# HazyResearch/flash-fft-conv

Hardware: AMD Instinct MI355X
Metric: FFT-conv fwd+bwd seq/s, B=16 H=768 L=16384 fft=32768 bf16 (higher is better)
Workload: dtype bf16; 1 GPU; FlashFFTConv(32768) B=16 H=768 L=16384 bf16, fwd+bwd incl. k->k_f and dk (BASELINE configs[1]); heads_per_rank=768, parallelism=head-shard x1 (no collective)

## Files before the change

flash-fft-conv_amd/csrc/ffc_body.h:

```cpp
#pragma once
#include <stdint.h>

#include "ffc_layout.h"
#include "ffc_plan.h"

#ifndef FFC_FN
#define FFC_FN inline __attribute__((always_inline))
#endif

namespace ffc {

struct ConvArgs {
  const void* u;
  const void* pregate;
  const void* postgate;
  void* y;
  const void* kf;
  const uint8_t* tab;
  PlanTabs t;
  int B, H, L;
  int npair;
  int nchunk, ppc;
  int conj_kf;
  int fast;
// ... 1045 lines not shown
        if (FWD && !NOTW) {
          if constexpr (CHAIN16_A) {
            i32 m = j * 4 + (w * 128 * GEO::S1 + 2 * tp + th);
            i32 k0 = hi * 4;
            if constexpr (RP) twiddle16(re, im, m * (k0 * ps.R + ps.k0), m * ps.R, -1.0f, s_fwd, GEO::N * ps.R - 1, 1.0f / (float)(GEO::N * ps.R));
            else twiddle16(re, im, m * k0, m, -1.0f, s_fwd);
          } else
#pragma unroll
          for (int half = 0; half < 2; half++) {
            const int s1 = (16 * half) / GEO::N1;
            i32 m = j * 4 + (s1 * 128 + w * 128 * GEO::S1 + 2 * tp + th);
            i32 k0 = hi * 4 + ((16 * half) % GEO::N1);
            F2 tr[4], ti[4];
            if constexpr (RP) chain8p(m * (k0 * ps.R + ps.k0), m * ps.R, -1.0f, s_fwd, tr, ti, GEO::N * ps.R - 1, 1.0f / (float)(GEO::N * ps.R));
            else chain8p(m * k0, m, -1.0f, s_fwd, tr, ti);
            apply8(re, im, half, tr, ti);
          }
        }
        if constexpr (!B::LEAN_OUTER) {
          if (th == 0) {
            re0 = re; im0 = im;
          } else {
#pragma unroll
            for (int r = 0; r < 16; r++) {
              if (!FWD && HALF && row_dead((r & 3) + 8 * (r >> 2))) continue;
              const int c = (r & 3) + 8 * (r >> 2);
              const int s1 = c / GEO::N1, rwc = c % GEO::N1;
              i32 off = colb[s1] + (rwc * (GEO::Mi * 2) + 4 * tp);
              B::lds_w32(off, B::template pack<DT>(re0[r], re[r]));
              B::lds_w32(off + GEO::PLANE, B::template pack<DT>(im0[r], im[r]));
            }
          }
        } else {
          if (th == 0) {
#pragma unroll
            for (int q = 0; q < 8; q++) {
              if (!FWD && HALF && row_dead(((2 * q) & 3) + 8 * ((2 * q) >> 2))) continue;
              s0r[q] = B::template pack<DT>(re[2 * q], re[2 * q + 1]);
              s0i[q] = B::template pack<DT>(im[2 * q], im[2 * q + 1]);
            }
          } else {
#pragma unroll
            for (int q = 0; q < 8; q++) {
              if (!FWD && HALF && row_dead(((2 * q) & 3) + 8 * ((2 * q) >> 2))) continue;
              u32 p1r = B::template pack<DT>(re[2 * q], re[2 * q + 1]), p1i = B::template pack<DT>(im[2 * q], im[2 * q + 1]);
#pragma unroll
              for (int o = 0; o < 2; o++) {
                const int r = 2 * q + o;
                const int c = (r & 3) + 8 * (r >> 2);
                const int s1 = c / GEO::N1, rwc = c % GEO::N1;
                i32 off = colb[s1] + (rwc * (GEO::Mi * 2) + 4 * tp);
                B::lds_w32(off, o ? B::merge_hi(s0r[q], p1r) : B::merge_lo(s0r[q], p1r));
                B::lds_w32(off + GEO::PLANE, o ? B::merge_hi(s0i[q], p1i) : B::merge_lo(s0i[q], p1i));
              }
            }
          }
        }
      }
    }
  }

#ifndef FFC_OUTER_QUAD
#define FFC_OUTER_QUAD 1
#endif
  template <bool FWD, bool HALF, bool RP = false, bool NOTW = false>
  static FFC_FN void outer_stage_quad(int L, Unit un, float s_fwd = 1.0f, Pass ps = Pass()) {
    const i32 lane = B::opaque(B::lane());
    const int w = un.wq;
    const i32 j = lane & 31, hi = lane >> 5;
    constexpr int ms_lim = (FWD && HALF && GEO::N1 == 32) ? 1 : 2;
    i32 colb[GEO::S1];
#pragma unroll
    for (int s = 0; s < GEO::S1; s++)
      colb[s] = e_off<GEO, i32>(hi * 4, j * 4 + (s * 128 + w * 128 * GEO::S1)) + un.eb;
    Mat F1;
    if constexpr (RP) load_mat(F1, FWD ? ps.mat_fwd : ps.mat_inv, lane);
    else lds_mat(F1, GEO::L_F1);
    U2 rawr[2][8], rawi[2][8];
#pragma unroll
    for (int ms = 0; ms < 2; ms++) {
      if (ms >= ms_lim) continue;
#pragma unroll
      for (int e = 0; e < 8; e++) {
        const int c = 16 * ms + 8 * (e >> 2) + (e & 3);
        const int s1 = c / GEO::N1, rwc = c % GEO::N1;
        i32 off = colb[s1] + rwc * (GEO::Mi * 2);
        if (FWD && HALF && row_dead(c)) { rawr[ms][e].x = B::uconst(0); rawr[ms][e].y = B::uconst(0); rawi[ms][e] = rawr[ms][e]; continue; }
        rawr[ms][e] = B::lds_r64(off); rawi[ms][e] = B::lds_r64(off + GEO::PLANE);
      }
    }
    u32 p0r[16], p0i[16];
#pragma unroll
    for (int tp = 0; tp < 2; tp++) {
      A16 re0, im0;
#pragma unroll
      for (int th = 0; th < 2; th++) {
        Op op;
#pragma unroll
        for (int ms = 0; ms < 2; ms++) {
          if (ms >= ms_lim) continue;
#pragma unroll
          for (int d = 0; d < 4; d++) {
            const u32 ar = tp ? rawr[ms][2 * d].y : rawr[ms][2 * d].x, br = tp ? rawr[ms][2 * d + 1].y : rawr[ms][2 * d + 1].x;
            const u32 ai = tp ? rawi[ms][2 * d].y : rawi[ms][2 * d].x, bi = tp ? rawi[ms][2 * d + 1].y : rawi[ms][2 * d + 1].x;
            op.r[ms][d] = th ? B::merge_hi(ar, br) : B::merge_lo(ar, br);
            op.i[ms][d] = th ? B::merge_hi(ai, bi) : B::merge_lo(ai, bi);
          }
        }
        A16 re, im;
        re = B::a16_zero(); im = B::a16_zero();
        cmm<!FWD, false>(re, im, op, F1, ms_lim);
        if (FWD && !NOTW) {
          if constexpr (CHAIN16_A) {
            i32 m = j * 4 + (w * 128 * GEO::S1 + 2 * tp + th);
            i32 k0 = hi * 4;
            if constexpr (RP) twiddle16(re, im, m * (k0 * ps.R + ps.k0), m * ps.R, -1.0f, s_fwd, GEO::N * ps.R - 1, 1.0f / (float)(GEO::N * ps.R));
            else twiddle16(re, im, m * k0, m, -1.0f, s_fwd);
          } else
#pragma unroll
          for (int half = 0; half < 2; half++) {
            const int s1 = (16 * half) / GEO::N1;
            i32 m = j * 4 + (s1 * 128 + w * 128 * GEO::S1 + 2 * tp + th);
            i32 k0 = hi * 4 + ((16 * half) % GEO::N1);
            F2 tr[4], ti[4];
            if constexpr (RP) chain8p(m * (k0 * ps.R + ps.k0), m * ps.R, -1.0f, s_fwd, tr, ti, GEO::N * ps.R - 1, 1.0f / (float)(GEO::N * ps.R));
            else chain8p(m * k0, m, -1.0f, s_fwd, tr, ti);
            apply8(re, im, half, tr, ti);
          }
        }
        if (th == 0) {
          re0 = re; im0 = im;
        } else {
#pragma unroll
          for (int r = 0; r < 16; r++) {
            if (!FWD && HALF && row_dead((r & 3) + 8 * (r >> 2))) continue;
            const u32 vr = B::template pack<DT>(re0[r], re[r]), vi = B::template pack<DT>(im0[r], im[r]);
            if (tp == 0) {
              p0r[r] = vr; p0i[r] = vi;
            } else {
              const int c = (r & 3) + 8 * (r >> 2);
              const int s1 = c / GEO::N1, rwc = c % GEO::N1;
              i32 off = colb[s1] + rwc * (GEO::Mi * 2);
              U2 wr, wi;
              wr.x = p0r[r]; wr.y = vr; wi.x = p0i[r]; wi.y = vi;
              B::lds_w64(off, wr);
              B::lds_w64(off + GEO::PLANE, wi);
            }
          }
        }
      }
    }
  }

  template <bool FWD, bool HALF, bool RP = false, bool DIN = false, bool NOTW = false>
  static FFC_FN void outer_stage(int L, Unit un, float s_fwd = 1.0f, Pass ps = Pass()) {
    if constexpr (DIN) { outer_stage_pair<FWD, HALF, RP, true, NOTW>(L, un, s_fwd, ps); return; }
    if constexpr (B::LEAN_OUTER && !(FWD && HALF && GEO::N1 == 32)) outer_stage_tile<FWD, HALF, RP, NOTW>(L, un, s_fwd, ps);
    else if constexpr (!B::LEAN_OUTER && FFC_OUTER_QUAD != 0 && HALF) outer_stage_quad<FWD, HALF, RP, NOTW>(L, un, s_fwd, ps);
    else outer_stage_pair<FWD, HALF, RP, false, NOTW>(L, un, s_fwd, ps);
  }

  struct InnerRegs { Mat F2; CT16 tw; i32 roff[2][2]; i32 woff[4]; };
  template <bool TWR = true>
  static FFC_FN void load_inner(InnerRegs& R, Unit un) {
    lds_mat(R.F2, GEO::L_F2);
    if constexpr (TWR) lds_ct16(R.tw, GEO::L_TW);
    const i32 lane = B::lane();
    const i32 c = lane & 31, hi = lane >> 5;
    const i32 i16 = lane & 15, g16 = (lane >> 4) & 1;
    const i32 n3b = (g16 * 16) % GEO::N3;
#pragma unroll
    for (int ms = 0; ms < 2; ms++)
#pragma unroll
      for (int rho = 0; rho < 2; rho++) {
        i32 U = hi * 4 + (16 * ms + 8 * rho) + (i16 >> 2);
        i32 sU = U / GEO::N2, n2 = U % GEO::N2;
        i32 row = sU * GEO::SV + ((g16 * 16) / GEO::N3);
        R.roff[ms][rho] = e_off<GEO, i32>(row, n2 * GEO::N3 + n3b + (i16 & 3) * 4) + un.eb;
      }
#pragma unroll
    for (int rq = 0; rq < 4; rq++) {
      i32 V = hi * 4 + 8 * rq;
      i32 row = (c / GEO::N2) * GEO::SV + V / GEO::N3;
      R.woff[rq] = e_off<GEO, i32>(row, (c % GEO::N2) * GEO::N3 + V % GEO::N3) + un.eb;
    }
  }

  static constexpr int IPASS_BYTES = 2 * 6144 + 2 * 8192;
  static constexpr int L_IPASS = GEO::LDS_BYTES;
  struct InnerPass { Mat Fa, Finv; CT16 tw; int tw2_off; int base; };
  static FFC_FN void load_inner_pass(InnerPass& ip, int k0) {
    const int base = L_IPASS + k0 * IPASS_BYTES;
    lds_mat(ip.Fa, base);
    lds_mat(ip.Finv, base + 6144);
    lds_ct16(ip.tw, base + 12288);
    ip.tw2_off = base + 12288 + 8192;
    ip.base = base;
  }
  static FFC_FN void load_inner_pass_lean(InnerPass& ip, int k0) {
    ip.base = L_IPASS + k0 * IPASS_BYTES;
    ip.tw2_off = ip.base + 12288 + 8192;
  }
  static FFC_FN void setup_tables_ipass(const uint8_t* tab, const PlanTabs& t, int R) {
    for (int k0 = 0; k0 < R; k0++) copy_tab(tab + t.ipass[k0], L_IPASS + k0 * IPASS_BYTES, IPASS_BYTES);
    B::barrier();
  }

  static FFC_FN void load_tile_op(int tau, Op& op, Unit un, const InnerRegs& R, int doff = 0) {
    const int trow = tau * (GEO::G * GEO::Mi * 2) + doff;
    if (B::HAS_TR) {
#pragma unroll
      for (int ms = 0; ms < 2; ms++)
#pragma unroll
        for (int rho = 0; rho < 2; rho++) {
          i32 off = R.roff[ms][rho] + trow;
          U2 vr = B::lds_r64_tr(off), vi = B::lds_r64_tr(off + GEO::PLANE);
          op.r[ms][2 * rho] = vr.x; op.r[ms][2 * rho + 1] = vr.y;
          op.i[ms][2 * rho] = vi.x; op.i[ms][2 * rho + 1] = vi.y;
        }
#pragma unroll
      for (int ms = 0; ms < 2; ms++) { B::pin(op.r[ms]); B::pin(op.i[ms]); }
    } else {
      const i32 lane = B::opaque(B::lane());
      const i32 c = lane & 31, hi = lane >> 5;
      const i32 sV = c / GEO::N3, n3 = c % GEO::N3;
#pragma unroll
      for (int ms = 0; ms < 2; ms++)
#pragma unroll
        for (int d = 0; d < 4; d++) {
          u32 wr[2], wi[2];
#pragma unroll
          for (int hf = 0; hf < 2; hf++) {
            int e = 2 * d + hf;
            i32 U = hi * 4 + (16 * ms + 8 * (e >> 2) + (e & 3));
            i32 sU = U / GEO::N2, n2 = U % GEO::N2;
            i32 row = sU * GEO::SV + sV + tau * GEO::G;
            i32 off = e_off<GEO, i32>(row, n2 * GEO::N3 + n3) + un.eb + doff;
            wr[hf] = B::lds_r16(off);
            wi[hf] = B::lds_r16(off + GEO::PLANE);
          }
          op.r[ms][d] = wr[0] | (wr[1] << 16);
          op.i[ms][d] = wi[0] | (wi[1] << 16);
        }
    }
  }

  static constexpr bool CAN_FOLD = ((FFC_FOLD_TW >= 1 && GEO::N1 == 16) || (FFC_FOLD_TW >= 2 && GEO::N1 == 32)) && GEO::N2 == 32 && GEO::N3 == 32;
  template <bool TWR = true, bool IP = false, bool FOLD = false, bool IPL = false>
  static FFC_FN void tile_fwd(int tau, const InnerRegs& R, Unit un, A16& re, A16& im, const InnerPass* ip = nullptr, const uint8_t* fold = nullptr,
                              const Mat2* fa_pre = nullptr) {
    if constexpr (FOLD) {
      const i32 lane = B::opaque(B::lane());
      Mat2 FA, FB;
      if (fa_pre) FA = *fa_pre;
      else load_mat2_issue(FA, fold + (0 * GEO::NT + tau) * 6144, lane);
      load_mat2_issue(FB, fold + (1 * GEO::NT + tau) * 6144, lane);
      Op op;
      load_tile_op(tau, op, un, R);
      re = B::a16_zero(); im = B::a16_zero();
      cmm2<true>(re, im, op, FA);
      if constexpr (TWR) cmul(re, im, R.tw);
      else cmul_lds<false>(re, im, GEO::L_TW);
      to_op(re, im, op);
      re = B::a16_zero(); im = B::a16_zero();
      cmm2<false>(re, im, op, FB);
      return;
    }
    Op op;
    load_tile_op(tau, op, un, R);
    re = B::a16_zero(); im = B::a16_zero();
    if constexpr (IP && IPL) {
      Mat Fa;
      lds_mat(Fa, ip->base);
      cmm<false, true>(re, im, op, Fa);
      cmul_lds<false>(re, im, ip->base + 12288);
    } else if constexpr (IP) {
      cmm<false, true>(re, im, op, ip->Fa);
      cmul(re, im, ip->tw);
    } else {
      cmm<false, true>(re, im, op, R.F2);
      if constexpr (TWR) {
        cmul(re, im, R.tw);
      } else {
        cmul_lds<false>(re, im, GEO::L_TW);
      }
    }
    to_op(re, im, op);
    re = B::a16_zero(); im = B::a16_zero();
    if constexpr (GEO::N3 != GEO::N2) {
      Mat F3;
      lds_mat(F3, GEO::L_F3);
      cmm<false, false>(re, im, op, F3);
    } else {
      cmm<false, false>(re, im, op, R.F2);
    }
  }
  template <bool TWR = true, bool RP = false, bool IP = false, bool FOLD = false, bool IPL = false>
  static FFC_FN void tile_inv(float s_inv, int tau, const InnerRegs& R, Unit un, A16& re, A16& im, int dbg = 0, Pass ps = Pass(),
                              const InnerPass* ip = nullptr, const uint8_t* fold = nullptr, const Mat2* g_pre = nullptr) {
    const i32 lane = B::opaque(B::lane());
    const i32 c = lane & 31, hi = lane >> 5;
    if constexpr (FOLD) {
      static_assert(!RP && !IP && CAN_FOLD, "folded outer twiddle: single-pass fft 16384 / 32768");
      Mat2 GB, GA;
      if (g_pre) { GB = g_pre[0]; GA = g_pre[1]; }
      else {
        load_mat2_issue(GB, fold + (2 * GEO::NT + tau) * 6144, lane);
        load_mat2_issue(GA, fold + (3 * GEO::NT + tau) * 6144, lane);
      }
// ... 425 lines not shown
    kf_mul<SZ>(a, kfB, reB, imB); to_op(reB, imB, opB);
    reB = B::a16_zero(); imB = B::a16_zero();
    cmm<true, true>(reB, imB, opB, R.F2);
    cmul_conj(reA, imA, R.tw); to_op(reA, imA, opA);
    reA = B::a16_zero(); imA = B::a16_zero();
    cmm<true, true>(reA, imA, opA, R.F2);
    cmul_conj(reB, imB, R.tw); to_op(reB, imB, opB);
    reB = B::a16_zero(); imB = B::a16_zero();
    cmm<true, true>(reB, imB, opB, R.F2);
    oi_twiddle<RP>(a.s_inv, tauA, reA, imA, ps);
    tile_store(tauA, R, reA, imA);
    oi_twiddle<RP>(a.s_inv, tauB, reB, imB, ps);
    tile_store(tauB, R, reB, imB);
  }

  template <bool SZ>
  static FFC_FN void inner_tile2x_fold(const ConvArgs& a, int h, int tau, const InnerRegs& R, Unit un, uint8_t* zsA, uint8_t* zsB) {
    static_assert(CAN_FOLD && GEO::UPW >= 2, "folded outer twiddle, two units per workgroup");
    constexpr int DB = GEO::EBYTES;
    const i32 lane = B::opaque(B::lane());
    const uint8_t* fold = a.tab + a.t.fold;
    Mat2 FA, FB, GB, GA;
    load_mat2_issue(FA, fold + (0 * GEO::NT + tau) * 6144, lane);
    KfRegs kf;
    load_kf(a, h, tau, kf);
    Op opA, opB;
    load_tile_op(tau, opA, un, R);
    load_tile_op(tau, opB, un, R, DB);
    load_mat2_issue(FB, fold + (1 * GEO::NT + tau) * 6144, lane);
    A16 reA, imA, reB, imB;
    reA = B::a16_zero(); imA = B::a16_zero();
    cmm2<true>(reA, imA, opA, FA);
    reB = B::a16_zero(); imB = B::a16_zero();
    cmm2<true>(reB, imB, opB, FA);
    load_mat2_issue(GB, fold + (2 * GEO::NT + tau) * 6144, lane);
    cmul(reA, imA, R.tw); to_op(reA, imA, opA);
    reA = B::a16_zero(); imA = B::a16_zero();
    cmm2<false>(reA, imA, opA, FB);
    cmul(reB, imB, R.tw); to_op(reB, imB, opB);
    reB = B::a16_zero(); imB = B::a16_zero();
    cmm2<false>(reB, imB, opB, FB);
    load_mat2_issue(GA, fold + (3 * GEO::NT + tau) * 6144, lane);
    if constexpr (SZ) { z_store(zsA, tau, reA, imA, Z_STREAM); z_store(zsB, tau, reB, imB, Z_STREAM); }
    {
      CT16 k;
#pragma unroll
      for (int rq = 0; rq < 4; rq++) {
        u32 wv[4] = {kf.v[rq].x, kf.v[rq].y, kf.v[rq].z, kf.v[rq].w};
#pragma unroll
        for (int q = 0; q < 4; q++) {
          k.re[4 * rq + q] = B::template unpack_lo<DT>(wv[q]);
          k.im[4 * rq + q] = B::template unpack_hi<DT>(wv[q]);
        }
      }
      if constexpr (!SZ) k.im = B::a16_scale(k.im, a.conj_kf ? -1.0f : 1.0f);
      cmul(reA, imA, k); to_op(reA, imA, opA);
      reA = B::a16_zero(); imA = B::a16_zero();
      cmm2<true>(reA, imA, opA, GB);
      cmul(reB, imB, k); to_op(reB, imB, opB);
      reB = B::a16_zero(); imB = B::a16_zero();
      cmm2<true>(reB, imB, opB, GB);
    }
    cmul_conj(reA, imA, R.tw); to_op(reA, imA, opA);
    reA = B::a16_zero(); imA = B::a16_zero();
    cmm2<true>(reA, imA, opA, GA);
    cmul_conj(reB, imB, R.tw); to_op(reB, imB, opB);
    reB = B::a16_zero(); imB = B::a16_zero();
    cmm2<true>(reB, imB, opB, GA);
    tile_store(tau, R, reA, imA);
    tile_store(tau, R, reB, imB, DB);
  }
  template <bool SZ = false>
  static FFC_FN void inner_tile2x(const ConvArgs& a, int h, int tau, const InnerRegs& R, Unit un, uint8_t* zsA = nullptr, uint8_t* zsB = nullptr) {
    static_assert(GEO::N3 == GEO::N2 && GEO::OUTER && GEO::UPW >= 2, "inner_tile2x: two units per workgroup");
    constexpr int DB = GEO::EBYTES;
    KfRegs kf;
    load_kf(a, h, tau, kf);
    Op opA, opB;
    load_tile_op(tau, opA, un, R);
    load_tile_op(tau, opB, un, R, DB);
    A16 reA, imA, reB, imB;
    reA = B::a16_zero(); imA = B::a16_zero();
    cmm<false, true>(reA, imA, opA, R.F2);
    reB = B::a16_zero(); imB = B::a16_zero();
    cmm<false, true>(reB, imB, opB, R.F2);
    cmul(reA, imA, R.tw); to_op(reA, imA, opA);
    reA = B::a16_zero(); imA = B::a16_zero();
    cmm<false, false>(reA, imA, opA, R.F2);
    cmul(reB, imB, R.tw); to_op(reB, imB, opB);
    reB = B::a16_zero(); imB = B::a16_zero();
    cmm<false, false>(reB, imB, opB, R.F2);
    if constexpr (SZ) { z_store(zsA, tau, reA, imA, Z_STREAM); z_store(zsB, tau, reB, imB, Z_STREAM); }
    {
      CT16 k;
#pragma unroll
      for (int rq = 0; rq < 4; rq++) {
        u32 wv[4] = {kf.v[rq].x, kf.v[rq].y, kf.v[rq].z, kf.v[rq].w};
#pragma unroll
        for (int q = 0; q < 4; q++) {
          k.re[4 * rq + q] = B::template unpack_lo<DT>(wv[q]);
          k.im[4 * rq + q] = B::template unpack_hi<DT>(wv[q]);
        }
      }
      if constexpr (!SZ) k.im = B::a16_scale(k.im, a.conj_kf ? -1.0f : 1.0f);
      cmul(reA, imA, k); to_op(reA, imA, opA);
      reA = B::a16_zero(); imA = B::a16_zero();
      cmm<true, true>(reA, imA, opA, R.F2);
      cmul(reB, imB, k); to_op(reB, imB, opB);
      reB = B::a16_zero(); imB = B::a16_zero();
      cmm<true, true>(reB, imB, opB, R.F2);
    }
    cmul_conj(reA, imA, R.tw); to_op(reA, imA, opA);
    reA = B::a16_zero(); imA = B::a16_zero();
    cmm<true, true>(reA, imA, opA, R.F2);
    cmul_conj(reB, imB, R.tw); to_op(reB, imB, opB);
    reB = B::a16_zero(); imB = B::a16_zero();
    cmm<true, true>(reB, imB, opB, R.F2);
    {
      const i32 lane = B::opaque(B::lane());
      const i32 c = lane & 31, hi = lane >> 5;
      const i32 sUl = c / GEO::N2, mlane = (c % GEO::N2) * GEO::N3;
      if constexpr (GEO::N3 == 32) {
        i32 k1 = sUl * GEO::SV + tau * GEO::G;
        F2 tr[4], ti[4];
        f32 c8, s8;
        chain8p(B::mul24(mlane + hi * 4, k1), k1, 1.0f, a.s_inv, tr, ti, GEO::N - 1, 1.0f / (float)GEO::N, &c8, &s8);
        apply8(reA, imA, 0, tr, ti);
        apply8(reB, imB, 0, tr, ti);
        const f32 c16 = c8 * c8 - s8 * s8, s16 = (c8 + c8) * s8;
#pragma unroll
        for (int i = 0; i < 4; i++) B::cmulp(tr[i], ti[i], c16, s16, tr[i], ti[i]);
        apply8(reA, imA, 1, tr, ti);
        apply8(reB, imB, 1, tr, ti);
      } else
#pragma unroll
      for (int half = 0; half < 2; half++) {
        const int sV = (16 * half) / GEO::N3;
        i32 k1 = sUl * GEO::SV + (sV + tau * GEO::G);
        i32 n30 = hi * 4 + ((16 * half) % GEO::N3);
        F2 tr[4], ti[4];
        chain8p(B::mul24(mlane + n30, k1), k1, 1.0f, a.s_inv, tr, ti);
        apply8(reA, imA, half, tr, ti);
        apply8(reB, imB, half, tr, ti);
      }
    }
    tile_store(tau, R, reA, imA);
    tile_store(tau, R, reB, imB, DB);
  }

  static FFC_FN void unit_barrier() {
    if constexpr (GEO::NW > 1) B::barrier();
    else B::lds_fence();
  }
  template <bool HALF, bool PROF = false, bool RP = false, bool SZ = false, bool SP = false>
  static FFC_FN void outer_jobs(const ConvArgs& a, int h, int p0, int p1, int u, Unit un, int wg_linear = 0) {
    constexpr int NC = HALF ? NCH / 2 : NCH;
    constexpr bool PREFETCH = HALF && !RP;
    constexpr bool FOLDF = CAN_FOLD && !RP && !SP && !PROF && !B::LEAN_OUTER;
    constexpr bool CROSS = !SP && !RP && !PROF && !B::LEAN_OUTER && GEO::N3 == GEO::N2 && GEO::NW > 1 && GEO::UPW >= 2;
    const int npass = RP ? a.R : 1;
    const int iters = ((p1 - p0 + GEO::UPW - 1) / GEO::UPW) * npass;
    RowRegsT<NC> X;
    if constexpr (PREFETCH) { if (p0 + u < p1) rows_load<NC>(a, h, p0 + u, un, X); }
    unsigned long long acc[8] = {0, 0, 0, 0, 0, 0, 0, 0}, t0 = 0, t1 = 0;
#define FFC_TICK(k) if (PROF) { t1 = B::clock(); acc[k] += t1 - t0; t0 = t1; }
    const bool second = B::wave() >= 4;
#define FFC_PRIO(x) if constexpr (GEO::NW > 1) B::template setprio<x>();
#pragma unroll 1
    for (int it = 0; it < iters; it++) {
      const int p = p0 + (RP ? it / npass : it) * GEO::UPW + u;
      const Pass ps = RP ? make_pass(a, it % npass) : Pass();
      const int hk = RP ? h * ps.R + ps.k0 : h;
      const bool act = p < p1;
      if (PROF) t0 = B::clock();
      FFC_PRIO(1)
      if (act) {
        if constexpr (RP) {
          rows_in_rp<NC>(a, h, p, un, ps);
        } else {
          if constexpr (!PREFETCH) rows_load<NC>(a, h, p, un, X);
          rows_store<NC>(a, h, p, un, X);
        }
        B::lds_fence();
        FFC_TICK(0)
        FFC_PRIO(0)
        outer_stage<true, HALF, RP, false, FOLDF>(a.L, un, a.s_fwd, ps);
        FFC_TICK(1)
      }
      unit_barrier();
      FFC_TICK(2)
      if constexpr (CROSS) {
        const int ug = u >> 1, wl = (u & 1) * GEO::NW + un.wq;
        const int pA = p0 + it * GEO::UPW + 2 * ug;
        if (pA < p1) {
          Unit ua;
          ua.eb = 2 * ug * GEO::EBYTES; ua.wq = wl;
          InnerRegs R;
          load_inner(R, ua);
          uint8_t* zA = SZ ? z_slot(a.zsave, h, a.npair, pA) : nullptr;
          if (pA + 1 < p1) {
#pragma unroll 1
            for (int tt = 0; tt < 2; tt++) {
              if (tt == 0) { FFC_PRIO(3) } else if (second) { FFC_PRIO(2) } else { FFC_PRIO(1) }
              if constexpr (FOLDF) inner_tile2x_fold<SZ>(a, hk, wl * 2 + tt, R, ua, zA, zA + (int64_t)GEO::N * 4);
              else inner_tile2x<SZ>(a, hk, wl * 2 + tt, R, ua, zA, zA + (int64_t)GEO::N * 4);
            }
          } else {
            inner_tile2<false, SZ, FOLDF, HALF>(a, hk, wl * 2, R, ua, Pass(), zA);
          }
        }
      } else if (act) {
        InnerRegs R;
        load_inner(R, un);
        if constexpr (SP) {
          Mat Fs;
          lds_mat_sp(Fs);
#pragma unroll 1
          for (int tt = 0; tt < GEO::TPW; tt += 2) inner_tile2_sp(a, hk, un.wq * GEO::TPW + tt, R, Fs, un);
        } else if constexpr (GEO::N3 == GEO::N2) {
#pragma unroll 1
          for (int tt = 0; tt < GEO::TPW; tt += 2) {
            if (tt == 0) { FFC_PRIO(3) } else if (second) { FFC_PRIO(2) } else { FFC_PRIO(1) }
            inner_tile2<RP, SZ, FOLDF, HALF>(a, hk, un.wq * GEO::TPW + tt, R, un, ps,
                                SZ ? (RP ? z_slot_rp(a.zsave, h, a.npair, p, ps.R, ps.k0) : z_slot(a.zsave, h, a.npair, p)) : nullptr);
          }
        } else {
          KfRegs kf0;
          load_kf(a, h, un.wq * GEO::TPW, kf0);
#pragma unroll 1
          for (int tt = 0; tt < GEO::TPW; tt++) {
            KfRegs kfn;
            if (tt + 1 < GEO::TPW) load_kf(a, h, un.wq * GEO::TPW + tt + 1, kfn);
            inner_tile(a, un.wq * GEO::TPW + tt, R, un, kf0);
            kf0 = kfn;
          }
        }
      }
      FFC_TICK(3)
      unit_barrier();
      FFC_TICK(4)
      FFC_PRIO(3)
      if constexpr (PREFETCH) { if (it + 1 < iters && p + GEO::UPW < p1) rows_load<NC>(a, h, p + GEO::UPW, un, X); }
      if (act) {
        outer_stage<false, HALF, RP>(a.L, un, 1.0f, ps);
        B::lds_fence();
        FFC_TICK(5)
        FFC_PRIO(2)
        if constexpr (SZ) {
          if (a.yraw) {
            ConvArgs ar = a;
            ar.y = a.yraw; ar.postgate = nullptr; ar.addend = nullptr; ar.sby = (int64_t)a.H * a.L;
            if constexpr (RP) rows_out_rp<NC, false>(ar, h, p, un, ps);
            else rows_out<NC, false>(ar, h, p, un);
          }
        }
        if constexpr (RP) rows_out_rp<NC>(a, h, p, un, ps);
        else rows_out<NC>(a, h, p, un);
        FFC_TICK(6)
      }
    }
#undef FFC_TICK
#undef FFC_PRIO
    if (PROF && a.prof) {
      const i32 lane = B::lane();
      unsigned long long* dst = a.prof + ((long long)wg_linear * GEO::WGW + B::wave()) * 8;
#pragma unroll
      for (int k = 0; k < 8; k++) B::g_w64(dst, lane * 0 + k, B::u2_from64(acc[k]), lane < 1);
    }
  }

  template <bool HALF = false, bool SZ = false, bool SP = false>
  static FFC_FN void conv(const ConvArgs& a, int h, int chunk) {
    setup_tables(a.tab, a.t);
    conv_job<HALF, false, SZ, SP>(a, h, chunk);
  }
  template <bool HALF = false, bool RP = false, bool SZ = false, bool SP = false>
  static FFC_FN void conv_job(const ConvArgs& a, int h, int chunk) {
    const int wv = B::wave();
    Unit un;
    un.wq = wv % GEO::NW;
    const int u = wv / GEO::NW;
    un.eb = u * GEO::EBYTES;
    const int p0 = chunk * a.ppc;
    int p1 = p0 + a.ppc;
    if (p1 > a.npair) p1 = a.npair;
    if constexpr (GEO::OUTER) {
      outer_jobs<HALF, false, RP, SZ, SP>(a, h, p0, p1, u, un);
    } else {
      const int q0 = p0 / GEO::G, q1 = (p1 + GEO::G - 1) / GEO::G;
      const int iters = (q1 - q0 + GEO::UPW - 1) / GEO::UPW;
      InnerRegs R;
      load_inner(R, un);
      if constexpr (RP) {
        static_assert(GEO::G == 1, "inner-only multi-pass: one pair per tile");
#ifndef FFC_IP_MERGE
#define FFC_IP_MERGE 1
#endif
        if (FFC_IP_MERGE != 0 && a.fast && a.L <= GEO::N && !a.aux_in) {
          const i32 lane = B::opaque(B::lane());
#pragma unroll 1
          for (int it = 0; it < iters; it++) {
            const int q = q0 + it * GEO::UPW + u;
            if (q >= q1) continue;
            RowRegs X, Y;
            rows_load<NCH>(a, h, q, un, X);
            if (a.pregate) {
              RowRegs G;
#pragma unroll
              for (int ii = 0; ii < NCH; ii++) {
                i32 idx = lane + ii * 64;
                i32 m = (idx % CPR) * 8;
#pragma unroll
                for (int pl = 0; pl < 2; pl++) {
                  i32 b = (idx / CPR + q * GEO::G) * 2 + pl;
                  G.v[ii][pl] = gload8_rows((const uint16_t*)a.pregate, b, h, a, a.sbg, m, 1, b < a.B);
                }
              }
#pragma unroll
              for (int ii = 0; ii < NCH; ii++)
#pragma unroll
                for (int pl = 0; pl < 2; pl++) X.v[ii][pl] = mul4(X.v[ii][pl], G.v[ii][pl]);
            }
#pragma unroll 1
            for (int k0 = 0; k0 < a.R; k0++) {
              InnerPass ip;
              load_inner_pass(ip, k0);
              KfRegs kf;
              load_kf(a, h * a.R + k0, 0, kf);
#pragma unroll
              for (int ii = 0; ii < NCH; ii++) {
                i32 idx = lane + ii * 64;
                pred sw;
                i32 off = pair_off(idx / CPR, (idx % CPR) * 8, &sw) + un.eb;
#pragma unroll
                for (int pl = 0; pl < 2; pl++) {
                  const U4& v = X.v[ii][pl];
                  U4 o;
                  o.x = B::sel(sw, v.z, v.x); o.y = B::sel(sw, v.w, v.y);
                  o.z = B::sel(sw, v.x, v.z); o.w = B::sel(sw, v.y, v.w);
                  B::lds_w128(off + pl * GEO::PLANE, o, B::ptrue());
                }
              }
              B::lds_fence();
              inner_tile<true, SZ>(a, 0, R, un, kf, &ip, (SZ && a.zsave) ? z_slot_small(a.zsave, h, a.npair, q, a.R, k0) : nullptr);
              B::lds_fence();
#pragma unroll
              for (int ii = 0; ii < NCH; ii++) {
                i32 idx = lane + ii * 64;
                pred sw;
                i32 off = pair_off(idx / CPR, (idx % CPR) * 8, &sw) + un.eb;
#pragma unroll
                for (int pl = 0; pl < 2; pl++) {
                  U4 o = B::lds_r128(off + pl * GEO::PLANE);
                  U4 v;
                  v.x = B::sel(sw, o.z, o.x); v.y = B::sel(sw, o.w, o.y);
                  v.z = B::sel(sw, o.x, o.z); v.w = B::sel(sw, o.y, o.w);
                  if (k0 == 0) Y.v[ii][pl] = v;
                  else Y.v[ii][pl] = add4(Y.v[ii][pl], v, 1.0f);
                }
              }
              B::lds_fence();
            }
#pragma unroll
            for (int ii = 0; ii < NCH; ii++) {
              i32 idx = lane + ii * 64;
              i32 m = (idx % CPR) * 8;
#pragma unroll
              for (int pl = 0; pl < 2; pl++) {
                i32 b = (idx / CPR + q * GEO::G) * 2 + pl;
                U4 v = Y.v[ii][pl];
                if constexpr (SZ) {
                  if (a.yraw) gstore8_rows((uint16_t*)a.yraw, b, h, a, (int64_t)a.H * a.L, m, 1, b < a.B, v);
                }
                if constexpr (B::HAS_ADD) {
                  U4 r = gload8_rows((const uint16_t*)a.addend, b, h, a, a.sba, m, 1, b < a.B);
                  if (a.postgate) v = fma4(v, gload8_rows((const uint16_t*)a.postgate, b, h, a, a.sbp, m, 1, b < a.B), r);
                  else v = sum4(v, r);
                } else {
                  if (a.postgate) v = mul4(v, gload8_rows((const uint16_t*)a.postgate, b, h, a, a.sbp, m, 1, b < a.B));
                }
                gstore8_rows((uint16_t*)a.y, b, h, a, a.sby, m, 1, b < a.B, v);
              }
            }
          }
          return;
        }
#pragma unroll 1
        for (int it = 0; it < iters * a.R; it++) {
          const int q = q0 + (it / a.R) * GEO::UPW + u;
          const int k0 = it % a.R;
          if (q < q1) {
            Pass ps; ps.k0 = k0; ps.R = a.R;
            InnerPass ip;
            load_inner_pass(ip, k0);
            KfRegs kf;
            load_kf(a, h * a.R + k0, 0, kf);
            rows_in_rp<NCH>(a, h, q, un, ps);
            B::lds_fence();
            inner_tile<true, SZ>(a, 0, R, un, kf, &ip, (SZ && a.zsave) ? z_slot_small(a.zsave, h, a.npair, q, a.R, k0) : nullptr);
            B::lds_fence();
            if constexpr (SZ) {
              if (a.yraw) {
                ConvArgs ar = a;
                ar.y = a.yraw; ar.postgate = nullptr; ar.addend = nullptr; ar.sby = (int64_t)a.H * a.L;
                rows_out_rp<NCH, false>(ar, h, q, un, ps);
              }
            }
            rows_out_rp<NCH>(a, h, q, un, ps);
            B::lds_fence();
          }
        }
        return;
      }
#pragma unroll 1
      for (int it = 0; it < iters; it++) {
        const int q = q0 + it * GEO::UPW + u;
        const bool act = q < q1;
        if (act) {
          KfRegs kf;
          load_kf(a, h, 0, kf);
          rows_in(a, h, q, un);
          B::lds_fence();
          inner_tile<false, SZ>(a, 0, R, un, kf, nullptr, (SZ && a.zsave) ? z_slot_small(a.zsave, h, a.npair, q, 1, 0) : nullptr);
          B::lds_fence();
          if constexpr (SZ) {
            if (a.yraw) {
              ConvArgs ar = a;
              ar.y = a.yraw; ar.postgate = nullptr; ar.addend = nullptr; ar.sby = (int64_t)a.H * a.L;
              rows_out<NCH, false>(ar, h, q, un);
            }
          }
          rows_out(a, h, q, un);
        }
      }
    }
  }
};

}
```

flash-fft-conv_amd/csrc/ffc_bwd_launch.h:

```cpp
#pragma once
#ifndef FFC_GATE_BATCH
#define FFC_GATE_BATCH 1
#define FFC_GATE_BATCH_OUT 2
#endif
#include "ffc_dev.h"
using namespace ffc;

template <class GEO, int DT, bool HALF, int ZM>
__global__ __launch_bounds__(GEO::WGW * 64, 2) __attribute__((amdgpu_num_vgpr(128))) void bwd_kernel(DkfArgs d) {
  if constexpr (GEO::NW == 1) {
    const int total = ((d.c.H + 7) & ~7) * d.c.nchunk;
    for (int id = blockIdx.x; id < total; id += gridDim.x) {
      int h, chunk;
      if (map_id(id, d.c.H, d.c.nchunk, &h, &chunk)) Modes<DevBO, GEO, DT>::template bwd<HALF, false, true, ZM>(d, h, chunk, blockIdx.x);
    }
  } else {
    int h, chunk;
    if (!map_block(d.c.H, d.c.nchunk, &h, &chunk)) return;
    stagger_start(d.c.flags);
    Modes<DevBO, GEO, DT>::template bwd<HALF, false, true, ZM>(d, h, chunk, blockIdx.x);
  }
}
template <class GEO, int DT>
__global__ __launch_bounds__(GEO::WGW * 64, 2) void bwd_kernel_small(DkfArgs d) {
  using M = Modes<DevB, GEO, DT>;
  M::BD::setup_tables(d.c.tab, d.c.t);
  if constexpr (GEO::N == 1024) { if (d.c.R > 1) M::BD::setup_tables_ipass(d.c.tab, d.c.t, d.c.R); }
  const int total = ((d.c.H + 7) & ~7) * d.c.nchunk;
  for (int id = blockIdx.x; id < total; id += gridDim.x) {
    int h, chunk;
    if (map_id(id, d.c.H, d.c.nchunk, &h, &chunk)) M::template bwd<false, false, false>(d, h, chunk, id);
  }
}
template <class GEO, int DT, bool HALF, int ZM, bool FASTK>
__global__ __launch_bounds__(GEO::WGW * 64, 2) __attribute__((amdgpu_num_vgpr(128))) void bwd_rp_kernel(DkfArgs d) {
  using BK = typename std::conditional<FASTK, DevBOF, DevBO>::type;
  int h, chunk;
  if (!map_block(d.c.H, d.c.nchunk, &h, &chunk)) return;
  Modes<BK, GEO, DT>::BD::setup_tables(d.c.tab, d.c.t);
  const int wv = DevBO::wave(), wg = blockIdx.x;
#pragma unroll 1
  for (int k0 = 0; k0 < d.c.R; k0++) Modes<BK, GEO, DT>::template bwd<HALF, true, true, ZM>(d, h, chunk, wg, k0, wv);
}

template <int ZM>
struct BwdLaunchZ {
template <class GEO, int DT>
struct T {
  static int run(const DkfArgs& d, hipStream_t st) {
    static_assert(Body<DevB, GEO, DT>::IPASS_BYTES == IPASS_BYTES, "ffc_route.h");
    const BwdRoute r = bwd_route<GEO>(d, false);
    if (r.err) return ffc_fail(r.err);
    constexpr int T_ = GEO::WGW * 64;
    if constexpr (!GEO::OUTER && ZM != 0) {
      return ffc_fail("single-tile sizes are launched by the recomputing unit (run-time spectrum switch)");
    } else if constexpr (!GEO::OUTER) {
      return ffc_launch(bwd_kernel_small<GEO, DT>, "bwd_kernel", r.grid, T_, r.lds_max, r.lds, st, d);
    } else {
      return pick([&](auto mp, auto half, auto fastk) -> int {
        constexpr bool MP = decltype(mp)::value, HALF = decltype(half)::value, FASTK = decltype(fastk)::value;
        if constexpr (MP && GEO::N == 32768)
          return ffc_launch(bwd_rp_kernel<GEO, DT, HALF, ZM, FASTK>, "bwd_rp_kernel", r.grid, T_, r.lds_max, r.lds, st, d);
        else if constexpr (!MP && !FASTK)
          return ffc_launch(bwd_kernel<GEO, DT, HALF, ZM>, "bwd_kernel", r.grid, T_, r.lds_max, r.lds, st, d);
        else
          return ffc_fail("internal: the backward route names a kernel that does not exist");
      }, r.multi_pass, r.half, r.fastk);
    }
  }
};
};
```

flash-fft-conv_amd/csrc/ffc_conv_launch.h:

```cpp
#pragma once
#include "ffc_dev.h"

template <class FAM>
struct ConvLaunch {
template <class GEO, int DT>
struct T {
  static int run(const ffc::ConvArgs& a, hipStream_t st) {
    using namespace ffc;
    static_assert(Body<DevB, GEO, DT>::IPASS_BYTES == IPASS_BYTES, "ffc_route.h");
    const FwdRoute r = fwd_route<GEO>(a);
    if (r.err) return ffc_fail(r.err);
    return pick([&](auto mp, auto half, auto sz, auto sp) -> int {
      constexpr bool MP = decltype(mp)::value, HALF = decltype(half)::value, SZ = decltype(sz)::value, SP = decltype(sp)::value;
      if constexpr (fwd_kernel_exists<GEO>(FAM::HAS_ADD, MP, HALF, SZ, SP))
        return ffc_launch(FAM::template kernel<GEO, DT, MP, HALF, SZ, SP>(), FAM::what(MP, SZ, SP, GEO::OUTER), r.grid, GEO::WGW * 64, r.lds_max, r.lds, st, a);
      else
        return ffc_fail("internal: the forward route names a kernel that does not exist");
    }, r.multi_pass, r.half, r.sz, r.sp);
  }
};
};
```

flash-fft-conv_amd/csrc/ffc_dev.h:

```cpp
#pragma once
#include <hip/hip_runtime.h>
#include <stdint.h>
#include <stdlib.h>
#include <string.h>

#include <string>
#include <type_traits>

#define FFC_FN __device__ __forceinline__
#include "../../include/flashfftconv_hip.h"
#include "ffc_body.h"
#include "ffc_modes.h"
#include "ffc_big.h"
#include "ffc_route.h"

namespace ffc {

typedef __bf16 bf16x8 __attribute__((ext_vector_type(8)));
typedef _Float16 f16x8 __attribute__((ext_vector_type(8)));
typedef __bf16 bf16x2 __attribute__((ext_vector_type(2)));
typedef _Float16 f16x2 __attribute__((ext_vector_type(2)));
typedef float f32x2 __attribute__((ext_vector_type(2)));
typedef float f32x16 __attribute__((ext_vector_type(16)));
typedef short s16x4 __attribute__((ext_vector_type(4)));
typedef uint32_t u32x4v __attribute__((ext_vector_type(4)));

extern __shared__ __attribute__((aligned(16))) uint8_t ffc_smem[];

struct DevB {
  using f32 = float;
  using i32 = int;
  using u32 = uint32_t;
  using pred = bool;
  struct U2 { u32 x, y; };
  struct U4 { u32 x, y, z, w; };
  static constexpr bool LEAN_OUTER = false;
  static constexpr bool FAST_ONLY = false;
  static constexpr bool HAS_ADD = false;
  using A16 = f32x16;
  using W4 = u32x4v;
  static constexpr bool HAS_TR = true;
  template <bool CONJ> static FFC_FN void cmul16(A16& re, A16& im, const A16& tr, const A16& ti) {
    const A16 a = re, b = im;
    if (!CONJ) { re = a * tr - b * ti; im = a * ti + b * tr; }
    else { re = a * tr + b * ti; im = b * tr - a * ti; }
  }
  using F2 = f32x2;
  static FFC_FN F2 f2(f32 a, f32 b) { F2 v = {a, b}; return v; }
  static FFC_FN f32 f2_lo(F2 v) { return v.x; }
  static FFC_FN f32 f2_hi(F2 v) { return v.y; }
  static FFC_FN void cmulp(F2 xr, F2 xi, f32 wr, f32 wi, F2& yr, F2& yi) {
    yr = xr * wr - xi * wi;
    yi = xr * wi + xi * wr;
  }
  template <bool CONJ>
  static FFC_FN void cmul2v(A16& re, A16& im, int r0, F2 tr, F2 ti) {
    const F2 a = {re[r0], re[r0 + 1]}, b = {im[r0], im[r0 + 1]};
    F2 x, y;
    if (!CONJ) { x = a * tr - b * ti; y = a * ti + b * tr; }
    else { x = a * tr + b * ti; y = b * tr - a * ti; }
    re[r0] = x.x; re[r0 + 1] = x.y; im[r0] = y.x; im[r0 + 1] = y.y;
  }
  static FFC_FN void cmac2_conj(F2& wr, F2& wi, const A16& a, const A16& b, int r0, F2 zr, F2 zi) {
    const F2 a2 = {a[r0], a[r0 + 1]}, b2 = {b[r0], b[r0 + 1]};
    wr = wr + (a2 * zr + b2 * zi);
    wi = wi + (b2 * zr - a2 * zi);
  }
#define FFC_A8(b) "a" #b "0", "a" #b "1", "a" #b "2", "a" #b "3", "a" #b "4", "a" #b "5", "a" #b "6", "a" #b "7", "a" #b "8", "a" #b "9"
  static FFC_FN void agpr_reserve() {
    asm volatile("; a0..a127 hold the dk_f partial sums"
                 ::: "a0", "a1", "a2", "a3", "a4", "a5", "a6", "a7", "a8", "a9", FFC_A8(1), FFC_A8(2), FFC_A8(3), FFC_A8(4),
                     FFC_A8(5), FFC_A8(6), FFC_A8(7), FFC_A8(8), FFC_A8(9), FFC_A8(10), FFC_A8(11), "a120", "a121", "a122",
                     "a123", "a124", "a125", "a126", "a127");
  }
#undef FFC_A8
  template <int I> static FFC_FN f32 agpr_get() {
    f32 x;
    asm volatile("v_accvgpr_read_b32 %0, a%c1" : "=v"(x) : "n"(I));
    return x;
  }
  template <int I> static FFC_FN void agpr_set(f32 x) { asm volatile("v_accvgpr_write_b32 a%c0, %1" ::"n"(I), "v"(x)); }
  static FFC_FN void pin(W4& x) { asm("" : "+v"(x)); }
  static FFC_FN void pin4(U4& x) { asm volatile("" : "+v"(x.x), "+v"(x.y), "+v"(x.z), "+v"(x.w)); }
  static FFC_FN void sched_fence() { __builtin_amdgcn_sched_barrier(0); }
  template <bool CONJ>
  static FFC_FN void cmul2(A16& re, A16& im, int r0, f32 tr0, f32 tr1, f32 ti0, f32 ti1) {
    cmul2v<CONJ>(re, im, r0, f2(tr0, tr1), f2(ti0, ti1));
  }
  static FFC_FN A16 a16_scale(const A16& a, float s) { return a * s; }
  static FFC_FN A16 a16_zero() { A16 z = {0.f, 0.f, 0.f, 0.f, 0.f, 0.f, 0.f, 0.f, 0.f, 0.f, 0.f, 0.f, 0.f, 0.f, 0.f, 0.f}; return z; }
  static FFC_FN W4 w4(u32 a, u32 b, u32 c, u32 e) { W4 v = {a, b, c, e}; return v; }

  static FFC_FN i32 lane() { return (int)(threadIdx.x & 63); }
  static FFC_FN int wave() { return __builtin_amdgcn_readfirstlane((int)(threadIdx.x >> 6)); }
  static FFC_FN void barrier() { __syncthreads(); }
  static FFC_FN f32 fconst(float c) { return c; }
  static FFC_FN pred ptrue() { return true; }
  static FFC_FN pred pfalse() { return false; }
  static FFC_FN f32 as_f32(u32 a) { return __builtin_bit_cast(float, a); }
  static FFC_FN u32 as_u32(f32 a) { return __builtin_bit_cast(uint32_t, a); }

  static FFC_FN U2 lds_r64(i32 off) { uint2 v = *(const uint2*)(ffc_smem + off); return U2{v.x, v.y}; }
  static FFC_FN void lds_w64(i32 off, U2 v) { *(uint2*)(ffc_smem + off) = make_uint2(v.x, v.y); }
  static FFC_FN void lds_w32(i32 off, u32 v) { *(uint32_t*)(ffc_smem + off) = v; }
  static FFC_FN void lds_w128(i32 off, U4 v, pred p) {
    if (p) *(uint4*)(ffc_smem + off) = make_uint4(v.x, v.y, v.z, v.w);
  }
  static FFC_FN U4 lds_r128(i32 off) { uint4 v = *(const uint4*)(ffc_smem + off); return U4{v.x, v.y, v.z, v.w}; }
  static FFC_FN void lds_w16(i32 off, u32 v) { *(uint16_t*)(ffc_smem + off) = (uint16_t)v; }
  static FFC_FN u32 lds_r32(i32 off) { return *(const uint32_t*)(ffc_smem + off); }
  static FFC_FN u32 lds_r16(i32 off) { return *(const uint16_t*)(ffc_smem + off); }
  static FFC_FN U2 lds_r64_tr(i32 off) {
    s16x4 t = __builtin_amdgcn_ds_read_tr16_b64_v4i16((__attribute__((address_space(3))) s16x4*)(ffc_smem + off));
    uint2 v = __builtin_bit_cast(uint2, t);
    return U2{v.x, v.y};
  }
  static FFC_FN void lds_fence() { __builtin_amdgcn_fence(__ATOMIC_ACQ_REL, "wavefront"); }
  template <bool NT>
  static FFC_FN void g2lds32(const void* base, i32 dw, int lds_off) {
    const __attribute__((address_space(1))) void* g = (const __attribute__((address_space(1))) void*)((const uint32_t*)base + dw);
    __attribute__((address_space(3))) void* l = (__attribute__((address_space(3))) void*)(ffc_smem + lds_off);
    if constexpr (NT) __builtin_amdgcn_global_load_lds(g, l, 4, 0, 2);
    else __builtin_amdgcn_global_load_lds(g, l, 4, 0, 0);
  }
  template <bool NT>
  static FFC_FN void g2lds128(const void* base, i32 o16, int lds_off) {
    const __attribute__((address_space(1))) void* g = (const __attribute__((address_space(1))) void*)((const uint4*)base + o16);
    __attribute__((address_space(3))) void* l = (__attribute__((address_space(3))) void*)(ffc_smem + lds_off);
    if constexpr (NT) __builtin_amdgcn_global_load_lds(g, l, 16, 0, 2);
    else __builtin_amdgcn_global_load_lds(g, l, 16, 0, 0);
  }
  static FFC_FN void vm_wait0() { __builtin_amdgcn_s_waitcnt(0x0F70); }
  static FFC_FN void lds_w32p(i32 off, u32 v, pred p) { if (p) *(uint32_t*)(ffc_smem + off) = v; }
  static FFC_FN pred pnot(pred p) { return !p; }
  static FFC_FN u32 uconst(uint32_t c) { return c; }
  static FFC_FN i32 mul24(i32 a, i32 b) { return __mul24(a, b); }
  static FFC_FN unsigned long long clock() { return __builtin_amdgcn_s_memtime(); }
  template <int P> static FFC_FN void setprio() { __builtin_amdgcn_s_setprio(P); }
  static FFC_FN U2 u2_from64(unsigned long long v) { return U2{(u32)v, (u32)(v >> 32)}; }
  static FFC_FN void settle(f32& a, f32& b) { asm volatile("s_nop 4" : "+v"(a), "+v"(b)); }
  static FFC_FN f32 i2f(i32 a) { return (float)a; }
  static FFC_FN f32 cos_rev(f32 x) { return __builtin_amdgcn_cosf(x); }
  static FFC_FN f32 sin_rev(f32 x) { return __builtin_amdgcn_sinf(x); }
  static FFC_FN i32 opaque(i32 x) { asm volatile("" : "+v"(x)); return x; }
  static FFC_FN u32 sel(pred p, u32 a, u32 b) { return p ? a : b; }
  static FFC_FN u32 merge_lo(u32 a, u32 b) { return __builtin_amdgcn_perm(b, a, 0x05040100u); }
  static FFC_FN u32 merge_hi(u32 a, u32 b) { return __builtin_amdgcn_perm(b, a, 0x07060302u); }
  static FFC_FN i32 imin(i32 a, int b) { return a < b ? a : b; }
  static FFC_FN u32 g_r16(const void* base, i32 e, pred p) {
    uint16_t v = 0;
    if (p) v = ((const uint16_t*)base)[e];
    return v;
  }
  static FFC_FN void g_w16(void* base, i32 e, u32 v, pred p) {
    if (p) ((uint16_t*)base)[e] = (uint16_t)v;
  }
  static FFC_FN u32 g_r32(const void* base, i32 e, pred p) {
    uint32_t v = 0;
    if (p) v = ((const uint32_t*)base)[e];
    return v;
  }
  static FFC_FN void g_w32(void* base, i32 e, u32 v, pred p) {
    if (p) ((uint32_t*)base)[e] = v;
  }
  static FFC_FN U2 g_r64(const void* base, i32 o8, pred p) {
    uint2 v = make_uint2(0, 0);
    if (p) v = ((const uint2*)base)[o8];
    return U2{v.x, v.y};
  }
  static FFC_FN void g_w64(void* base, i32 o8, U2 v, pred p) {
    if (p) ((uint2*)base)[o8] = make_uint2(v.x, v.y);
  }
  static FFC_FN U4 g_r128(const void* base, i32 o16) {
    uint4 v = ((const uint4*)base)[o16];
    return U4{v.x, v.y, v.z, v.w};
  }
  static FFC_FN U4 g_r128_nt(const void* base, i32 o16) {
    u32x4v v = __builtin_nontemporal_load(((const u32x4v*)base) + o16);
    return U4{v.x, v.y, v.z, v.w};
  }
  static FFC_FN void g_w128_nt(void* base, i32 o16, U4 v, pred p) {
    if (p) { u32x4v t = {v.x, v.y, v.z, v.w}; __builtin_nontemporal_store(t, ((u32x4v*)base) + o16); }
  }
  static FFC_FN U4 g_r128p(const void* base, i32 o16, pred p) {
    uint4 v = make_uint4(0, 0, 0, 0);
    if (p) v = ((const uint4*)base)[o16];
    return U4{v.x, v.y, v.z, v.w};
  }
  static FFC_FN void g_w128(void* base, i32 o16, U4 v, pred p) {
    if (p) ((uint4*)base)[o16] = make_uint4(v.x, v.y, v.z, v.w);
  }
  template <int DT>
  static FFC_FN void mfma(A16& acc, const W4& a, const W4& b) {
    if (DT == DT_BF16)
      acc = __builtin_amdgcn_mfma_f32_32x32x16_bf16(__builtin_bit_cast(bf16x8, a), __builtin_bit_cast(bf16x8, b), acc, 0, 0, 0);
    else
      acc = __builtin_amdgcn_mfma_f32_32x32x16_f16(__builtin_bit_cast(f16x8, a), __builtin_bit_cast(f16x8, b), acc, 0, 0, 0);
  }
  template <int DT>
  static FFC_FN u32 pack(f32 lo, f32 hi) {
    f32x2 v = {lo, hi};
    if (DT == DT_BF16) return __builtin_bit_cast(uint32_t, __builtin_convertvector(v, bf16x2));
    return __builtin_bit_cast(uint32_t, __builtin_convertvector(v, f16x2));
  }
  static FFC_FN u32 pk_mul_f16(u32 a, u32 b) {
    return __builtin_bit_cast(uint32_t, __builtin_bit_cast(f16x2, a) * __builtin_bit_cast(f16x2, b));
  }
  template <int DT>
  static FFC_FN f32 unpack_lo(u32 a) {
    if (DT == DT_BF16) return __builtin_bit_cast(float, a << 16);
    return (float)__builtin_bit_cast(_Float16, (uint16_t)(a & 0xffffu));
  }
  template <int DT>
  static FFC_FN f32 unpack_hi(u32 a) {
    if (DT == DT_BF16) return __builtin_bit_cast(float, a & 0xffff0000u);
    return (float)__builtin_bit_cast(_Float16, (uint16_t)(a >> 16));
  }
};

__device__ __forceinline__ bool map_id(int id, int H, int nchunk, int* h, int* chunk) {
  int xcd = id & 7, s = id >> 3;
  *h = xcd + 8 * (s / nchunk);
  *chunk = s % nchunk;
  return *h < H;
}
__device__ __forceinline__ void stagger_start(int flags) {
  const int s = (flags >> 4) & 15;
  if (s == 0) return;
  const int n = ((blockIdx.x >> 3) & 7) * s;
  for (int i = 0; i < n; i++) __builtin_amdgcn_s_sleep(8);
}
__device__ __forceinline__ bool map_block(int H, int nchunk, int* h, int* chunk) {
  int id = blockIdx.x;
  int xcd = id & 7, s = id >> 3;
  *h = xcd + 8 * (s / nchunk);
  *chunk = s % nchunk;
  return *h < H;
}

struct DevBA : DevB {
  static constexpr bool HAS_ADD = true;
};

struct DevBO : DevB {
  static constexpr bool LEAN_OUTER = true;
  static FFC_FN i32 lane() {
    int x = (int)__builtin_amdgcn_mbcnt_hi(~0u, __builtin_amdgcn_mbcnt_lo(~0u, 0u));
    asm volatile("" : "+v"(x));
    return x;
  }
};

struct DevBOF : DevBO {
  static constexpr bool FAST_ONLY = true;
};

}

struct ffc_plan {
  ffc::HostPlan hp;
  ffc::HostPlan hp_bf;
  uint8_t* d_blob = nullptr;
  uint8_t* d_blob_bf = nullptr;
  int32_t* d_freq = nullptr;
  int num_cu = 256;
  int env_flags = 0;
  int env_stream = -1;
  int env_persist = -1;
  int env_wg_mult = 0;
};
static inline int ffc_persist(const ffc_plan* p) {
  if (p->env_persist == -1) return p->num_cu & ~7;
  return p->env_persist > 0 ? (p->env_persist & ~7) : 1 << 30;
}

extern "C" void ffc_set_error_(const char* m);
static inline int ffc_fail(const std::string& m) { ffc_set_error_(m.c_str()); return 1; }
#define HIPCHK(x)                                                                     \
  do {                                                                                \
    hipError_t e_ = (x);                                                              \
    if (e_ != hipSuccess) return ffc_fail(std::string(#x) + ": " + hipGetErrorString(e_)); \
  } while (0)

int ffc_set_lds_once(const void* kernel, int bytes);
namespace ffc { struct DkfArgs; }
int ffc_conv_res_launch(int N, int dtype, const ffc::ConvArgs& a, hipStream_t st);
int ffc_bwdz_launch(int N, int dtype, const ffc::DkfArgs& d, hipStream_t st);
template <class K>
static int ffc_set_lds(K kernel, int bytes) { return ffc_set_lds_once((const void*)kernel, bytes); }

template <class K, class A>
static int ffc_launch(K kernel, const char* what, dim3 grid, dim3 block, int lds_max, int lds, hipStream_t st, const A& args) {
  if (int rc = ffc_set_lds(kernel, lds_max)) return rc;
  hipLaunchKernelGGL(kernel, grid, block, lds, st, args);
  const hipError_t e = hipGetLastError();
  return e == hipSuccess ? 0 : ffc_fail(std::string(what) + " launch: " + hipGetErrorString(e));
}

template <template <class, int> class FN, class... A>
static int ffc_dispatch(int N, int dtype, A&&... args) {
  int rc = 0;
  const bool found = ffc::with_geo(N, [&](auto geo) {
    using GEO = decltype(geo);
    rc = dtype == ffc::DT_BF16 ? FN<GEO, ffc::DT_BF16>::run(args...) : FN<GEO, ffc::DT_F16>::run(args...);
  });
  return found ? rc : ffc_fail("unsupported fft size");
}

static inline void ffc_choose_chunks(const ffc_plan* p, int H, int npair, int* nchunk, int* ppc, bool fwd_only = false) {
  const bool outer = p->hp.N1 > 1;
  int upw = 8 / p->hp.NW;
  int pairs_per_iter = outer ? upw : upw * p->hp.G;
  int wg_per_cu = outer ? 1 : 2;
  int iters_total = (npair + pairs_per_iter - 1) / pairs_per_iter;
  int ipc;
  const int e = p->env_wg_mult;
  if (e > 0 || !fwd_only) {
    int mult = e > 0 ? e : 2;
    int target = p->num_cu * wg_per_cu * mult;
    int nc = (target + H - 1) / H;
    if (nc > iters_total) nc = iters_total;
    if (nc < 1) nc = 1;
    ipc = (iters_total + nc - 1) / nc;
  } else {
    const long slots = (long)p->num_cu * wg_per_cu;
    long best = -1;
    ipc = iters_total;
    for (int c = 1; c <= iters_total; c++) {
      long nch = (iters_total + c - 1) / c;
      long rounds = ((long)H * nch + slots - 1) / slots;
      long cost = rounds * (10L * c + 6);
      if (best < 0 || cost <= best) { best = cost; ipc = c; }
    }
  }
  *ppc = ipc * pairs_per_iter;
  *nchunk = (npair + *ppc - 1) / *ppc;
}

static inline void* ffc_zscratch(const ffc_plan* p, void* ws, int H, int nchunk) {
  return (uint8_t*)ws + (int64_t)nchunk * H * p->hp.R * p->hp.NT * 2048 * 4;
}
```

flash-fft-conv_amd/csrc/ffc_k_conv.hip:

```cpp
#include "ffc_conv_launch.h"
using namespace ffc;

static constexpr int SMALL_WAVES = 2;
template <class GEO, int DT, bool HALF, bool SZ = false, bool SP = false>
__global__ __launch_bounds__(GEO::WGW * 64, GEO::OUTER ? 2 : SMALL_WAVES) void conv_kernel(ConvArgs a) {
  using BD = Body<DevB, GEO, DT>;
  if constexpr (GEO::OUTER && GEO::NW == 1) {
    BD::setup_tables(a.tab, a.t);
    const int total = ((a.H + 7) & ~7) * a.nchunk;
    for (int id = blockIdx.x; id < total; id += gridDim.x) {
      int h, chunk;
      if (map_id(id, a.H, a.nchunk, &h, &chunk)) BD::template conv_job<HALF, false, SZ>(a, h, chunk);
    }
  } else if constexpr (!GEO::OUTER) {
    BD::setup_tables(a.tab, a.t);
    const int total = ((a.H + 7) & ~7) * a.nchunk;
    for (int id = blockIdx.x; id < total; id += gridDim.x) {
      int h, chunk;
      if (map_id(id, a.H, a.nchunk, &h, &chunk)) BD::template conv_job<HALF, false, SZ>(a, h, chunk);
    }
  } else {
    int h, chunk;
    if (!map_block(a.H, a.nchunk, &h, &chunk)) return;
    stagger_start(a.flags);
    if constexpr (GEO::NW > 1 && !SP) {
      BD::setup_tables(a.tab, a.t);
      if (a.kfuse_k || a.kfuse_x) Modes<DevB, GEO, DT>::kfft_head(a, h);
      BD::template conv_job<HALF, false, SZ, SP>(a, h, chunk);
    } else {
      BD::template conv<HALF, SZ, SP>(a, h, chunk);
    }
  }
}

template <class GEO, int DT, bool HALF, bool SZ = false>
__global__ __launch_bounds__(GEO::WGW * 64, 2) void conv_rp_kernel(ConvArgs a) {
  using BD = Body<DevB, GEO, DT>;
  if constexpr (!GEO::OUTER) {
    BD::setup_tables(a.tab, a.t);
    BD::setup_tables_ipass(a.tab, a.t, a.R);
    const int total = ((a.H + 7) & ~7) * a.nchunk;
    for (int id = blockIdx.x; id < total; id += gridDim.x) {
      int h, chunk;
      if (map_id(id, a.H, a.nchunk, &h, &chunk)) BD::template conv_job<HALF, true, SZ>(a, h, chunk);
    }
  } else {
    int h, chunk;
    if (!map_block(a.H, a.nchunk, &h, &chunk)) return;
    BD::setup_tables(a.tab, a.t);
    BD::template conv_job<HALF, true, SZ>(a, h, chunk);
  }
}

struct ConvKernels {
  static constexpr bool HAS_ADD = false;
  template <class GEO, int DT, bool MP, bool HALF, bool SZ, bool SP>
  static constexpr auto kernel() {
    if constexpr (MP) return conv_rp_kernel<GEO, DT, HALF, SZ>;
    else return conv_kernel<GEO, DT, HALF, SZ, SP>;
  }
  static const char* what(bool mp, bool sz, bool sp, bool outer) {
    if (mp) return sz && outer ? "conv_rp_kernel (spectrum-saving)" : "conv_rp_kernel";
    if (sz) return outer ? "conv_kernel (spectrum-saving)" : "conv_kernel (spectrum-saving, single tile)";
    return sp ? "conv_kernel (frequency-sparse)" : "conv_kernel";
  }
};
template __global__ void conv_kernel<Geo<1, 16, 16>, DT_BF16, true>(ConvArgs);
template __global__ void conv_kernel<Geo<1, 16, 16>, DT_F16, true>(ConvArgs);
template __global__ void conv_kernel<Geo<1, 16, 32>, DT_BF16, true>(ConvArgs);
template __global__ void conv_kernel<Geo<1, 16, 32>, DT_F16, true>(ConvArgs);
template __global__ void conv_kernel<Geo<1, 32, 32>, DT_BF16, true>(ConvArgs);
template __global__ void conv_kernel<Geo<1, 32, 32>, DT_F16, true>(ConvArgs);

static inline bool ffc_stride_ok(int64_t* sb, int64_t B, int64_t H, int64_t L) {
  if (*sb == 0) *sb = H * L;
  return *sb >= H * L && (B - 1) * *sb + H * L < ((int64_t)1 << 31);
}

extern "C" int64_t ffc_spectrum_bytes(const ffc_plan* p, int64_t B, int64_t H) {
  if (!p || B <= 0 || H <= 0) return 0;
  if (p->hp.N1 <= 1) {
    const int64_t G = (32 / p->hp.N2) * (32 / p->hp.N3);
    return H * (((B + 1) / 2 + G - 1) / G) * p->hp.R * 4096;
  }
  return ((B + 1) / 2) * H * (int64_t)p->hp.N * 4;
}

struct FwdCall {
  const void *u, *kf, *pregate, *postgate;
  void* y;
  int64_t B, H, L;
  void* stream;
  int conj_kf;
  int64_t sb_u, sb_pre, sb_post, sb_y;
  void *zsave, *yraw;
  int sparse;
  const void* addend; int64_t sb_add;
  const float* kfuse_k; int64_t kfuse_Lk;
  const void* kfuse_x; float kfuse_xscale;
};
static FwdCall fwd_call(const void* u, const void* kf, const void* pregate, const void* postgate, void* y, int64_t B, int64_t H, int64_t L,
                        void* stream) {
  FwdCall c{};
  c.u = u; c.kf = kf; c.pregate = pregate; c.postgate = postgate; c.y = y; c.B = B; c.H = H; c.L = L; c.stream = stream;
  return c;
}
static bool kfft_in_launch(const ffc_plan* p, int64_t B, int64_t H) {
  int nchunk = 0, ppc = 0;
  if (B > 0 && H > 0) ffc_choose_chunks(p, (int)H, (int)((B + 1) / 2), &nchunk, &ppc, true);
  return fwd_takes_kfft(p->hp, nchunk, 0, p->env_flags);
}

static int conv_fwd_impl(const ffc_plan* p, const FwdCall& c) {
  const void *u = c.u, *kf = c.kf, *pregate = c.pregate, *postgate = c.postgate, *addend = c.addend;
  void *y = c.y, *zsave = c.zsave;
  const int64_t B = c.B, H = c.H, L = c.L;
  const int sparse = c.sparse;
  int64_t sb_u = c.sb_u, sb_pre = c.sb_pre, sb_post = c.sb_post, sb_y = c.sb_y, sb_add = c.sb_add;
  if (!p || !u || !kf || !y) return ffc_fail("null arg");
  if (B <= 0 || H <= 0) return ffc_fail("empty batch/heads");
  if (L <= 0 || L > p->hp.N) return ffc_fail("L must be in (0, fft_size]");
  if ((uintptr_t)kf & 15) return ffc_fail("k_f must be 16-byte aligned");
  if (!ffc_stride_ok(&sb_u, B, H, L) || !ffc_stride_ok(&sb_pre, B, H, L) || !ffc_stride_ok(&sb_post, B, H, L) ||
      !ffc_stride_ok(&sb_y, B, H, L) || !ffc_stride_ok(&sb_add, B, H, L))
    return ffc_fail("tensor too large (>= 2^31 elements) or batch stride smaller than H*L");
  ConvArgs a{};
  a.u = u; a.pregate = pregate; a.postgate = postgate; a.y = y; a.kf = kf;
  a.tab = p->d_blob; a.t = p->hp.tabs;
  a.B = (int)B; a.H = (int)H; a.L = (int)L; a.npair = (int)((B + 1) / 2);
  a.sbu = sb_u; a.sbg = sb_pre; a.sbp = sb_post; a.sby = sb_y;
  a.addend = addend; a.sba = sb_add;
  a.conj_kf = c.conj_kf;
  a.zsave = zsave; a.yraw = (zsave || p->hp.N1 <= 1) ? c.yraw : nullptr;
  a.sparse = sparse;
  if (sparse && (sparse < 0 || sparse > 4 || zsave || p->hp.R > 1 || p->hp.N2 != 32 || p->hp.N3 != 32 || p->hp.N1 <= 1))
    return ffc_fail("frequency-sparse forward: fft 16384 / 32768, 1 <= rows <= 4, no spectrum buffer");
  if (zsave && (ffc_spectrum_bytes(p, B, H) == 0 || ((uintptr_t)zsave & 15))) return ffc_fail("spectrum buffer: unsupported plan or misaligned");
  a.s_inv = (float)p->hp.s_inv; a.s_fwd = (float)p->hp.s_fwd;
  a.flags = p->env_flags;
  a.fast = (L % 8 == 0) && !(((uintptr_t)u | (uintptr_t)y | (uintptr_t)pregate | (uintptr_t)postgate | (uintptr_t)addend) & 15) &&
           !((sb_u | sb_pre | sb_post | sb_y | sb_add) & 7);
  ffc_choose_chunks(p, a.H, a.npair, &a.nchunk, &a.ppc, true);
  a.persist = ffc_persist(p);
  a.R = p->hp.R;
  if (c.kfuse_k) {
    a.kfuse_k = c.kfuse_k; a.kfuse_Lk = (int)c.kfuse_Lk;
    a.kfuse_scale = (float)(p->hp.s_k / p->hp.s_fwd) / (p->hp.dtype == DT_F16 ? 256.f : 1.f);
    a.kfuse_fast = (c.kfuse_Lk % 4 == 0) && !((uintptr_t)c.kfuse_k & 15);
  }
  if (c.kfuse_x) { a.kfuse_x = c.kfuse_x; a.kfuse_scale = c.kfuse_xscale; a.kfuse_Lk = p->hp.N; a.kfuse_fast = 1; }
  a.stream = p->env_stream >= 0 ? p->env_stream : (p->hp.R > 1 ? 0 : 1);
  if (addend) return ffc_conv_res_launch(p->hp.N, p->hp.dtype, a, (hipStream_t)c.stream);
  return ffc_dispatch<ConvLaunch<ConvKernels>::T>(p->hp.N, p->hp.dtype, a, (hipStream_t)c.stream);
}

extern "C" int ffc_conv_fwd_strided(const ffc_plan* p, const void* u, const void* kf, const void* pregate, const void* postgate,
                                    void* y, int64_t B, int64_t H, int64_t L, int conj_kf, int64_t sb_u, int64_t sb_pre,
                                    int64_t sb_post, int64_t sb_y, void* stream) {
  FwdCall c = fwd_call(u, kf, pregate, postgate, y, B, H, L, stream);
  c.conj_kf = conj_kf; c.sb_u = sb_u; c.sb_pre = sb_pre; c.sb_post = sb_post; c.sb_y = sb_y;
  return conv_fwd_impl(p, c);
}
extern "C" int ffc_conv_fwd_z(const ffc_plan* p, const void* u, const void* kf, const void* pregate, const void* postgate, void* y,
                              void* zsave, void* y_raw, int64_t B, int64_t H, int64_t L, int64_t sb_u, int64_t sb_pre, int64_t sb_post,
                              int64_t sb_y, void* stream) {
  if (!zsave && !(y_raw && p && p->hp.N1 <= 1)) return ffc_fail("null spectrum buffer (y_raw alone: single-tile sizes, fft <= 2048)");
  if (y_raw && ((uintptr_t)y_raw & 15)) return ffc_fail("y_raw must be 16-byte aligned");
  FwdCall c = fwd_call(u, kf, pregate, postgate, y, B, H, L, stream);
  c.zsave = zsave; c.yraw = y_raw; c.sb_u = sb_u; c.sb_pre = sb_pre; c.sb_post = sb_post; c.sb_y = sb_y;
  return conv_fwd_impl(p, c);
}

extern "C" int ffc_conv_fwd_res(const ffc_plan* p, const void* u, const void* kf, const void* pregate, const void* postgate,
                                const void* addend, void* y, void* zsave, void* y_raw, int64_t B, int64_t H, int64_t L, int conj_kf,
                                int64_t sb_u, int64_t sb_pre, int64_t sb_post, int64_t sb_add, int64_t sb_y, void* stream) {
  if (!p) return ffc_fail("null arg");
  if (y_raw && !zsave && p->hp.N1 > 1) return ffc_fail("y_raw without a spectrum buffer: single-tile sizes only (fft <= 2048)");
  if (y_raw && ((uintptr_t)y_raw & 15)) return ffc_fail("y_raw must be 16-byte aligned");
  if ((zsave || y_raw) && conj_kf) return ffc_fail("spectrum buffer / y_raw: forward pass only (conj_kf = 0)");
  if (addend && y && B > 0 && H > 0 && L > 0) {
    const int64_t sa = sb_add ? sb_add : H * L, sy = sb_y ? sb_y : H * L;
    const uintptr_t a0 = (uintptr_t)addend, a1 = a0 + (uintptr_t)(((B - 1) * sa + H * L) * 2);
    const uintptr_t y0 = (uintptr_t)y, y1 = y0 + (uintptr_t)(((B - 1) * sy + H * L) * 2);
    if (a0 < y1 && y0 < a1) return ffc_fail("addend overlaps y");
  }
  FwdCall c = fwd_call(u, kf, pregate, postgate, y, B, H, L, stream);
  c.conj_kf = conj_kf; c.zsave = zsave; c.yraw = y_raw; c.addend = addend;
  c.sb_u = sb_u; c.sb_pre = sb_pre; c.sb_post = sb_post; c.sb_y = sb_y; c.sb_add = sb_add;
  return conv_fwd_impl(p, c);
}

extern "C" int ffc_conv_fwd_sparse(const ffc_plan* p, const void* u, const void* kf, const void* pregate, const void* postgate,
                                   void* y, int64_t B, int64_t H, int64_t L, int conj_kf, int rows, void* stream) {
  if (rows < 1) return ffc_fail("frequency-sparse forward: rows must be >= 1");
  FwdCall c = fwd_call(u, kf, pregate, postgate, y, B, H, L, stream);
  c.conj_kf = conj_kf; c.sparse = rows;
  return conv_fwd_impl(p, c);
}

extern "C" int ffc_conv_fwd(const ffc_plan* p, const void* u, const void* kf, const void* pregate, const void* postgate, void* y,
                            int64_t B, int64_t H, int64_t L, int conj_kf, void* stream) {
  return ffc_conv_fwd_strided(p, u, kf, pregate, postgate, y, B, H, L, conj_kf, 0, 0, 0, 0, stream);
}

template <class GEO, int DT>
__global__ __launch_bounds__(GEO::WGW * 64, 2) void conv_prof_kernel(ConvArgs a) {
  int h, chunk;
  if (!map_block(a.H, a.nchunk, &h, &chunk)) return;
  using BD = Body<DevB, GEO, DT>;
  BD::setup_tables(a.tab, a.t);
  const int wv = DevB::wave();
  typename BD::Unit un;
  un.wq = wv % GEO::NW;
  const int u = wv / GEO::NW;
  un.eb = u * GEO::EBYTES;
  const int p0 = chunk * a.ppc;
  int p1 = p0 + a.ppc;
  if (p1 > a.npair) p1 = a.npair;
  if (16 * GEO::Mi >= a.L) BD::template outer_jobs<true, true>(a, h, p0, p1, u, un, blockIdx.x);
  else BD::template outer_jobs<false, true>(a, h, p0, p1, u, un, blockIdx.x);
}

extern "C" int ffc_conv_fwd_prof(const ffc_plan* p, const void* u, const void* kf, void* y, int64_t B, int64_t H, int64_t L,
                                 unsigned long long* prof, int* grid_out, void* stream) {
  if (!p || p->hp.N != 32768 || p->hp.dtype != DT_BF16) return ffc_fail("prof build: N=32768 bf16 only");
  using GEO = Geo<32, 32, 32>;
  ConvArgs a{};
  a.u = u; a.y = y; a.kf = kf; a.tab = p->d_blob; a.t = p->hp.tabs;
  a.B = (int)B; a.H = (int)H; a.L = (int)L; a.npair = (int)((B + 1) / 2); a.s_inv = (float)p->hp.s_inv; a.s_fwd = (float)p->hp.s_fwd;
  a.fast = (L % 8 == 0);
  a.sbu = a.sbg = a.sbp = a.sby = H * L;
  a.flags = p->env_flags;
  a.prof = prof;
  ffc_choose_chunks(p, a.H, a.npair, &a.nchunk, &a.ppc);
  const int grid = fwd_route<GEO>(a).grid;
  if (grid_out) *grid_out = grid;
  return ffc_launch(conv_prof_kernel<GEO, DT_BF16>, "conv_prof_kernel", grid, GEO::WGW * 64, GEO::LDS_BYTES, GEO::LDS_BYTES, (hipStream_t)stream, a);
}

extern "C" int ffc_conv_fwd_k(const ffc_plan* p, const float* k, int64_t Lk, void* kf_out, const void* u, const void* pregate,
                              const void* postgate, void* y, void* zsave, void* y_raw, int64_t B, int64_t H, int64_t L, void* stream) {
  if (!p || !k || !kf_out) return ffc_fail("null arg");
  if (y_raw && ((uintptr_t)y_raw & 15)) return ffc_fail("y_raw must be 16-byte aligned");
  const bool fuse = kfft_in_launch(p, B, H) && Lk > 0 && Lk <= p->hp.N && H * Lk < ((int64_t)1 << 31);
  if (!fuse) {
    int rc = ffc_kernel_fft(p, k, H, Lk, kf_out, stream);
    if (rc) return rc;
  }
  FwdCall c = fwd_call(u, kf_out, pregate, postgate, y, B, H, L, stream);
  c.zsave = zsave; c.yraw = y_raw;
  if (fuse) { c.kfuse_k = k; c.kfuse_Lk = Lk; }
  return conv_fwd_impl(p, c);
}

extern "C" int ffc_conv_fwd_kx(const ffc_plan* p, const void* xpair, float scale, void* kf_out, const void* u, void* y, void* zsave,
                               int64_t B, int64_t H, int64_t L, void* stream) {
  if (!p || !xpair || !kf_out) return ffc_fail("null arg");
  const bool fuse = kfft_in_launch(p, B, H) && !((uintptr_t)xpair & 15);
  if (!fuse) {
    int rc = ffc_kernel_fft_c(p, xpair, H, kf_out, scale, stream);
    if (rc) return rc;
  }
  FwdCall c = fwd_call(u, kf_out, nullptr, nullptr, y, B, H, L, stream);
  c.zsave = zsave;
  if (fuse) { c.kfuse_x = xpair; c.kfuse_xscale = scale; }
  return conv_fwd_impl(p, c);
}
```

flash-fft-conv_amd/csrc/ffc_modes.h:

```cpp
#pragma once
#include "ffc_body.h"

namespace ffc {

struct KfArgs {
  const float* k;
  void* kf;
  const uint8_t* tab;
  PlanTabs t;
  int H, Lk;
  float scale;
  float s_fwd;
  float prescale;
  const void* xpair;
  int fast;
  int R;
};

struct DkfArgs {
  ConvArgs c;
  const void* dout;
  float* ws;
  int64_t sbd, sbdu, sbdpre, sbdpost;
  void* du;
// ... 688 lines not shown
    ConvArgs av = a;
    ConvArgs ad = a;
    ad.u = d.dout; ad.pregate = a.postgate; ad.sbu = d.sbd; ad.sbg = a.sbp;
    float* slab = RP ? d.ws + (((int64_t)chunk * a.H + h) * a.R + k0) * (GEO::NT * 2048)
                     : d.ws + ((int64_t)chunk * a.H + h) * (GEO::NT * 2048);
    InnerRegs R;
    if constexpr (GEO::OUTER) {
      const int iters = (p1 - p0 + GEO::UPW - 1) / GEO::UPW;
      uint8_t* zs = (uint8_t*)d.zscratch + ((int64_t)(wg_linear * GEO::UPW + u)) * (GEO::N * 4);
      WAcc W;
      w_acc_zero(W);
#pragma unroll 1
      for (int it = 0; it < iters; it++) {
        const int p = p0 + it * GEO::UPW + u;
        const bool act = p < p1;
        if (act) {
          if constexpr (RP) BD::template rows_in_rp<NCX>(av, h, p, un, ps);
          else BD::template rows_in<NCX>(av, h, p, un);
          B::lds_fence();
          BD::template outer_stage<true, HALF, RP>(a.L, un, a.s_fwd, ps);
        }
        BD::unit_barrier();
        if (act) {
          BD::template load_inner<false>(R, un);
#pragma unroll 1
          for (int tt = 0; tt < GEO::TPW; tt++) {
            A16 re, im;
            BD::template tile_fwd<false>(un.wq * GEO::TPW + tt, R, un, re, im);
            z_store(zs, un.wq * GEO::TPW + tt, re, im, (a.flags & 4) != 0);
          }
        }
        BD::unit_barrier();
        if (act) {
          if constexpr (RP) BD::template rows_in_rp<NCX>(ad, h, p, un, ps);
          else BD::template rows_in<NCX>(ad, h, p, un);
          B::lds_fence();
          BD::template outer_stage<true, HALF, RP>(a.L, un, a.s_fwd, ps);
        }
        BD::unit_barrier();
        if (act) {
          BD::template load_inner<false>(R, un);
          bwd_tiles<false, RP>(a, h, un, R, zs, slab, it == 0, W, ps);
        } else if (it == 0) {
#pragma unroll 1
          for (int tt = GEO::TPW; tt < GEO::TPW; tt++) w_zero(slab, un.wq * GEO::TPW + tt);
        }
        BD::unit_barrier();
      }
      w_acc_finish(slab, u, un, W);
    } else if (a.R > 1) {
      if constexpr (GEO::N == 1024) {
        BD::setup_tables_ipass(a.tab, a.t, a.R);
        const int q0 = p0, q1 = p1;
        const int iters = (q1 - q0 + GEO::UPW - 1) / GEO::UPW;
        BD::template load_inner<false>(R, un);
#pragma unroll 1
        for (int k0 = 0; k0 < a.R; k0++) {
          Pass ps; ps.k0 = k0; ps.R = a.R;
          InnerPass ip;
          BD::load_inner_pass_lean(ip, k0);
          A16 wre = B::a16_zero(), wim = B::a16_zero();
#pragma unroll 1
          for (int it = 0; it < iters; it++) {
            const int q = q0 + it * GEO::UPW + u;
            if (q < q1) {
              ZReg zv;
              A16 re, im;
              BD::template rows_in_rp<BD::NCH>(av, h, q, un, ps);
              B::lds_fence();
              BD::template tile_fwd<true, true, false, true>(0, R, un, re, im, &ip);
              z_pack(re, im, zv);
              B::lds_fence();
              BD::template rows_in_rp<BD::NCH>(ad, h, q, un, ps);
              B::lds_fence();
              BD::template tile_fwd<true, true, false, true>(0, R, un, re, im, &ip);
              w_add(wre, wim, zv, re, im);
              B::lds_fence();
            }
          }
          reduce_store_w(d.ws + (((int64_t)chunk * a.H + h) * a.R + k0) * 2048, u, wre, wim);
        }
      }
    } else {
      const int q0 = p0 / GEO::G, q1 = (p1 + GEO::G - 1) / GEO::G;
      const int iters = (q1 - q0 + GEO::UPW - 1) / GEO::UPW;
      BD::load_inner(R, un);
      A16 wre, wim;
      wre = B::a16_zero(); wim = B::a16_zero();
#pragma unroll 1
      for (int it = 0; it < iters; it++) {
        const int q = q0 + it * GEO::UPW + u;
        if (q < q1) {
          ZReg zv;
          A16 re, im;
          BD::rows_in(av, h, q, un);
          B::lds_fence();
          BD::tile_fwd(0, R, un, re, im);
          z_pack(re, im, zv);
          B::lds_fence();
          BD::rows_in(ad, h, q, un);
          B::lds_fence();
          BD::tile_fwd(0, R, un, re, im);
#pragma unroll
          for (int r = 0; r < 16; r++) {
            u32 pr = zv.r[r >> 1], pi = zv.i[r >> 1];
            f32 ur = (r & 1) ? B::template unpack_hi<DT>(pr) : B::template unpack_lo<DT>(pr);
            f32 ui = (r & 1) ? B::template unpack_hi<DT>(pi) : B::template unpack_lo<DT>(pi);
            wre[r] = wre[r] + (re[r] * ur + im[r] * ui);
            wim[r] = wim[r] + (im[r] * ur - re[r] * ui);
          }
          B::lds_fence();
        }
      }
      reduce_store_w(slab, u, wre, wim);
    }
  }
  static FFC_FN void z_unpack(const typename BD::KfRegs& z, A16& re, A16& im) {
#pragma unroll
    for (int rq = 0; rq < 4; rq++) {
      u32 wv[4] = {z.v[rq].x, z.v[rq].y, z.v[rq].z, z.v[rq].w};
#pragma unroll
      for (int q = 0; q < 4; q++) {
        re[4 * rq + q] = B::template unpack_lo<DT>(wv[q]);
        im[4 * rq + q] = B::template unpack_hi<DT>(wv[q]);
      }
    }
  }
  static FFC_FN void kf_plain_mul(const typename BD::KfRegs& kf, A16& re, A16& im) {
    typename BD::CT16 k;
#pragma unroll
    for (int rq = 0; rq < 4; rq++) {
      u32 wv[4] = {kf.v[rq].x, kf.v[rq].y, kf.v[rq].z, kf.v[rq].w};
#pragma unroll
      for (int q = 0; q < 4; q++) {
        k.re[4 * rq + q] = B::template unpack_lo<DT>(wv[q]);
        k.im[4 * rq + q] = B::template unpack_hi<DT>(wv[q]);
      }
    }
    BD::cmul(re, im, k);
  }
  static FFC_FN void kf_conj_mul(const typename BD::KfRegs& kf, A16& re, A16& im) {
    typename BD::CT16 k;
#pragma unroll
    for (int rq = 0; rq < 4; rq++) {
      u32 wv[4] = {kf.v[rq].x, kf.v[rq].y, kf.v[rq].z, kf.v[rq].w};
#pragma unroll
      for (int q = 0; q < 4; q++) {
        k.re[4 * rq + q] = B::template unpack_lo<DT>(wv[q]);
        k.im[4 * rq + q] = B::template unpack_hi<DT>(wv[q]);
      }
    }
    BD::cmul_conj(re, im, k);
  }
  template <bool HALF = false, bool RP = false, bool SETUP = true, int ZM = -1>
  static FFC_FN void bwd(const DkfArgs& d, int h, int chunk, int wg_linear, int k0 = 0, int wv_in = 0) {
    const ConvArgs& a = d.c;
    const Pass ps = RP ? make_pass(a.tab, a.t, a.R, k0) : Pass();
    const int hk = RP ? h * a.R + k0 : h;
    constexpr int NCX = HALF ? BD::NCH / 2 : BD::NCH;
    if constexpr (!RP && SETUP) BD::setup_tables(a.tab, a.t);
    const int wv = RP ? wv_in : B::wave();
    Unit un;
    un.wq = wv % GEO::NW;
    const int u = wv / GEO::NW;
    un.eb = u * GEO::EBYTES;
    const int p0 = chunk * a.ppc;
    int p1 = p0 + a.ppc;
    if (p1 > a.npair) p1 = a.npair;
    ConvArgs av = a;
    ConvArgs ad = a;
    ad.u = d.dout; ad.pregate = a.postgate; ad.sbu = d.sbd; ad.sbg = a.sbp;
    ConvArgs ao = a;
    ao.y = d.du; ao.postgate = a.pregate; ao.sby = d.sbdu; ao.sbp = a.sbg;
    ConvArgs ap = a;
    ap.y = d.dpre; ap.postgate = a.u; ap.sby = d.sbdpre; ap.sbp = a.sbu;
    ConvArgs aq = a;
    aq.y = d.dpost; aq.postgate = d.dout; aq.sby = d.sbdpost; aq.sbp = d.sbd;
    const bool dpost_tf = d.dpost != nullptr && d.yraw == nullptr;
    if constexpr (!(RP && GEO::OUTER)) {
      if (d.dpost && d.yraw) { ad.aux_in = d.yraw; ad.aux_out = d.dpost; ad.sbai = (int64_t)a.H * a.L; ad.sbao = d.sbdpost; }
    }
    float* slab = RP ? d.ws + (((int64_t)chunk * a.H + h) * a.R + k0) * (GEO::NT * 2048)
                     : d.ws + ((int64_t)chunk * a.H + h) * (GEO::NT * 2048);
    InnerRegs R;
    if constexpr (GEO::OUTER) {
      const int iters = (p1 - p0 + GEO::UPW - 1) / GEO::UPW;
      uint8_t* zs = (uint8_t*)d.zscratch + ((int64_t)(wg_linear * GEO::UPW + u)) * (GEO::N * 4);
      WAcc W;
      w_acc_zero(W);
      const bool have_z = ZM < 0 ? d.zin != nullptr : ZM == 1;
      constexpr bool FOLDZ = BD::CAN_FOLD && GEO::N1 == 32 && ZM == 1 && !RP;
      constexpr bool DMA_OK = BD::HAS_DMA && HALF && !RP && ZM != 0;
      const bool dma = DMA_OK && have_z && a.fast && !ad.pregate && !ad.aux_in && !dpost_tf && !(a.flags & 8);
      if constexpr (DMA_OK) { if (dma && p0 + u < p1) BD::rows_dma(ad, h, p0 + u, un); }
      const bool second = wv >= 4;
#define FFC_BPRIO(x) if constexpr (GEO::NW > 1) B::template setprio<x>();
#pragma unroll 1
      for (int it = 0; it < iters; it++) {
        const int p = p0 + it * GEO::UPW + u;
        const bool act = p < p1;
        FFC_BPRIO(1)
        const void* zp = !have_z ? (const void*)zs
                         : RP ? (const void*)BD::z_slot_rp(const_cast<void*>(d.zin), h, a.npair, act ? p : p0, a.R, k0)
                              : (const void*)BD::z_slot(const_cast<void*>(d.zin), h, a.npair, act ? p : p0);
        if (have_z) {
          if (dpost_tf) {
            BD::unit_barrier();
            if (act) {
              BD::template load_inner<false>(R, un);
#pragma unroll 1
              for (int tt = 0; tt < GEO::TPW; tt++) {
                const int tau = un.wq * GEO::TPW + tt;
                typename BD::KfRegs zv, kf;
                z_load(zp, tau, zv, BD::Z_STREAM);
                BD::load_kf(a, hk, tau, kf);
                A16 re, im;
                z_unpack(zv, re, im);
                kf_plain_mul(kf, re, im);
                BD::template tile_inv<false, RP>(a.s_inv, tau, R, un, re, im, 0, ps);
              }
            }
            BD::unit_barrier();
            if (act) {
              BD::template outer_stage<false, HALF, RP>(a.L, un, 1.0f, ps);
              B::lds_fence();
              if constexpr (RP) BD::template rows_out_rp<NCX>(aq, h, p, un, ps);
              else BD::template rows_out<NCX>(aq, h, p, un);
            }
          }
          if (act) {
            bool done = false;
            if constexpr (DMA_OK) {
              if (dma) {
                BD::rows_dma_finish(ad, p, un);
                FFC_BPRIO(0)
                BD::template outer_stage<true, HALF, RP, true, FOLDZ>(a.L, un, a.s_fwd, ps);
                done = true;
              }
            }
            if (!done) {
              if constexpr (RP) BD::template rows_in_rp<NCX>(ad, h, p, un, ps);
              else BD::template rows_in<NCX>(ad, h, p, un);
              B::lds_fence();
              FFC_BPRIO(0)
              BD::template outer_stage<true, HALF, RP, false, FOLDZ>(a.L, un, a.s_fwd, ps);
            }
          }
        } else {
          if (act) {
            if constexpr (RP) BD::template rows_in_rp<NCX>(av, h, p, un, ps);
            else BD::template rows_in<NCX>(av, h, p, un);
            B::lds_fence();
            FFC_BPRIO(0)
            BD::template outer_stage<true, HALF, RP>(a.L, un, a.s_fwd, ps);
          }
          BD::unit_barrier();
          FFC_BPRIO(3)
          if (act) {
            BD::template load_inner<false>(R, un);
#pragma unroll 1
            for (int tt = 0; tt < GEO::TPW; tt++) {
              const int tau = un.wq * GEO::TPW + tt;
              A16 re, im;
              BD::template tile_fwd<false>(tau, R, un, re, im);
              z_store(zs, tau, re, im, (a.flags & 4) != 0);
              if (dpost_tf) {
                typename BD::KfRegs kf;
                BD::load_kf(a, hk, tau, kf);
                kf_plain_mul(kf, re, im);
                BD::template tile_inv<false, RP>(a.s_inv, tau, R, un, re, im, 0, ps);
              }
            }
          }
          BD::unit_barrier();
          FFC_BPRIO(1)
          if (dpost_tf) {
            if (act) {
              BD::template outer_stage<false, HALF, RP>(a.L, un, 1.0f, ps);
              B::lds_fence();
              if constexpr (RP) BD::template rows_out_rp<NCX>(aq, h, p, un, ps);
              else BD::template rows_out<NCX>(aq, h, p, un);
            }
          }
          if (act) {
            if constexpr (RP) BD::template rows_in_rp<NCX>(ad, h, p, un, ps);
            else BD::template rows_in<NCX>(ad, h, p, un);
            B::lds_fence();
            FFC_BPRIO(0)
            BD::template outer_stage<true, HALF, RP>(a.L, un, a.s_fwd, ps);
          }
        }
        BD::unit_barrier();
        FFC_BPRIO(3)
        if (act) {
          BD::template load_inner<false>(R, un);
          bwd_tiles<true, RP, ZM == 1>(a, hk, un, R, zp, slab, it == 0, W, ps, have_z && BD::Z_STREAM, second);
        } else if (it == 0) {
#pragma unroll 1
          for (int tt = GEO::TPW; tt < GEO::TPW; tt++) w_zero(slab, un.wq * GEO::TPW + tt);
        }
        BD::unit_barrier();
        FFC_BPRIO(3)
        if (act) {
          BD::template outer_stage<false, HALF, RP>(a.L, un, 1.0f, ps);
          B::lds_fence();
          if constexpr (DMA_OK) { if (dma && p + GEO::UPW < p1) BD::rows_dma(ad, h, p + GEO::UPW, un); }
          FFC_BPRIO(2)
          if constexpr (RP) {
            BD::template rows_out_rp<NCX>(ao, h, p, un, ps);
            if (d.dpre) BD::template rows_out_rp<NCX>(ap, h, p, un, ps);
          } else {
            BD::template rows_out<NCX>(ao, h, p, un);
            if (d.dpre) BD::template rows_out<NCX>(ap, h, p, un);
          }
        }
      }
#undef FFC_BPRIO
      if constexpr (!RP && GEO::NW > 1) {
        if (d.dk_out || d.dk_pair) {
          using MB = Modes<B, GEO, DT_BF16>;
          if constexpr (DT != DT_BF16) {
            B::barrier();
            MB::BD::setup_tables(d.tab_bf, d.t_bf);
          }
          if constexpr (GEO::UPW == 1) MB::dk_tail(d, h, un.wq);
          else MB::dk_tail_multi(d, h, u, un.wq);
          return;
        }
      }
      if constexpr (RP && GEO::NW > 1 && GEO::UPW == 1 && DT == DT_BF16) {
        if (d.dk_out) { dk_tail_rp(d, h, un.wq, ps); return; }
      }
      w_acc_finish(slab, u, un, W);
    } else if (a.R > 1) {
      if constexpr (GEO::N == 1024) {
        if constexpr (SETUP) BD::setup_tables_ipass(a.tab, a.t, a.R);
        const int q0 = p0, q1 = p1;
        const int iters = (q1 - q0 + GEO::UPW - 1) / GEO::UPW;
        BD::template load_inner<false>(R, un);
#pragma unroll 1
        for (int k0 = 0; k0 < a.R; k0++) {
          Pass ps; ps.k0 = k0; ps.R = a.R;
          InnerPass ip;
          BD::load_inner_pass_lean(ip, k0);
          A16 wre = B::a16_zero(), wim = B::a16_zero();
#pragma unroll 1
          for (int it = 0; it < iters; it++) {
            const int q = q0 + it * GEO::UPW + u;
            if (q < q1) {
              ZReg zv;
              A16 re, im;
              typename BD::KfRegs kf;
              BD::load_kf(a, h * a.R + k0, 0, kf);
              typename BD::KfRegs zk;
              if (d.zin) {
                z_load(BD::z_slot_small(const_cast<void*>(d.zin), h, a.npair, q, a.R, k0), 0, zk, BD::Z_STREAM);
              } else {
                BD::template rows_in_rp<BD::NCH>(av, h, q, un, ps);
                B::lds_fence();
                BD::template tile_fwd<true, true, false, true>(0, R, un, re, im, &ip);
                z_pack(re, im, zv);
                B::lds_fence();
              }
              if (ad.aux_in && k0 == 0) BD::template rows_aux_rp<BD::NCH>(ad, h, q, un);
              BD::template rows_in_rp<BD::NCH>(ad, h, q, un, ps);
              B::lds_fence();
              BD::template tile_fwd<true, true, false, true>(0, R, un, re, im, &ip);
              if (d.zin) w_add_k(wre, wim, zk, re, im);
              else w_add(wre, wim, zv, re, im);
              kf_conj_mul(kf, re, im);
              B::lds_fence();
              BD::template tile_inv<true, false, true, false, true>(a.s_inv, 0, R, un, re, im, 0, Pass(), &ip);
              B::lds_fence();
              BD::template rows_out_rp<BD::NCH>(ao, h, q, un, ps);
              if (d.dpre) BD::template rows_out_rp<BD::NCH>(ap, h, q, un, ps);
              B::lds_fence();
            }
          }
          reduce_store_w(d.ws + (((int64_t)chunk * a.H + h) * a.R + k0) * 2048, u, wre, wim);
        }
      }
    } else {
      const int q0 = p0 / GEO::G, q1 = (p1 + GEO::G - 1) / GEO::G;
      const int iters = (q1 - q0 + GEO::UPW - 1) / GEO::UPW;
      BD::load_inner(R, un);
      A16 wre = B::a16_zero(), wim = B::a16_zero();
#pragma unroll 1
      for (int it = 0; it < iters; it++) {
        const int q = q0 + it * GEO::UPW + u;
        if (q < q1) {
          ZReg zv;
          A16 re, im;
          typename BD::KfRegs kf;
          BD::load_kf(a, h, 0, kf);
          typename BD::KfRegs zk;
          if (d.zin) {
            z_load(BD::z_slot_small(const_cast<void*>(d.zin), h, a.npair, q, 1, 0), 0, zk, BD::Z_STREAM);
          } else {
            BD::rows_in(av, h, q, un);
            B::lds_fence();
            BD::tile_fwd(0, R, un, re, im);
            z_pack(re, im, zv);
            B::lds_fence();
          }
          BD::rows_in(ad, h, q, un);
          B::lds_fence();
          BD::tile_fwd(0, R, un, re, im);
          if (d.zin) w_add_k(wre, wim, zk, re, im);
          else w_add(wre, wim, zv, re, im);
          kf_conj_mul(kf, re, im);
          B::lds_fence();
          BD::tile_inv(a.s_inv, 0, R, un, re, im);
          B::lds_fence();
          BD::rows_out(ao, h, q, un);
          if (d.dpre) BD::rows_out(ap, h, q, un);
          B::lds_fence();
        }
      }
      reduce_store_w(slab, u, wre, wim);
    }
  }

  static FFC_FN void w_add(A16& wre, A16& wim, const ZReg& zv, const A16& re, const A16& im) {
#pragma unroll
    for (int r = 0; r < 16; r++) {
      u32 pr = zv.r[r >> 1], pi = zv.i[r >> 1];
      f32 ur = (r & 1) ? B::template unpack_hi<DT>(pr) : B::template unpack_lo<DT>(pr);
      f32 ui = (r & 1) ? B::template unpack_hi<DT>(pi) : B::template unpack_lo<DT>(pi);
      wre[r] = wre[r] + (re[r] * ur + im[r] * ui);
      wim[r] = wim[r] + (im[r] * ur - re[r] * ui);
    }
  }
  static FFC_FN void w_add_k(A16& wre, A16& wim, const typename BD::KfRegs& z, const A16& re, const A16& im) {
#pragma unroll
    for (int rq = 0; rq < 4; rq++) {
      u32 wv[4] = {z.v[rq].x, z.v[rq].y, z.v[rq].z, z.v[rq].w};
#pragma unroll
      for (int q = 0; q < 4; q++) {
        const int r = 4 * rq + q;
        f32 ur = B::template unpack_lo<DT>(wv[q]), ui = B::template unpack_hi<DT>(wv[q]);
        wre[r] = wre[r] + (re[r] * ur + im[r] * ui);
        wim[r] = wim[r] + (im[r] * ur - re[r] * ui);
      }
    }
  }
  static FFC_FN void reduce_store_w(float* slab, int u, const A16& wre, const A16& wim) {
    static_assert(!GEO::OUTER, "single-tile geometries");
    if constexpr (GEO::UPW == 1) {
      store_w(slab, wre, wim);
    } else {
      static_assert(GEO::UPW == 8 && GEO::UPW * GEO::EBYTES >= 8 * 4096, "one wave per unit, 4 KB of exchange buffer each");
      const i32 lane = B::opaque(B::lane());
      f32 sr[2], si[2];
#pragma unroll
      for (int plane = 0; plane < 2; plane++) {
        B::barrier();
#pragma unroll
// ... 246 lines not shown
```

flash-fft-conv_amd/csrc/ffc_route.h:

```cpp
#pragma once
#include <stdint.h>
#include <type_traits>
#include "ffc_body.h"
#include "ffc_modes.h"
#include "ffc_big.h"

namespace ffc {

template <class F>
inline int pick(F&& f) { return f(); }
template <class F, class... Bs>
inline int pick(F&& f, bool b, Bs... bs) {
  return b ? pick([&](auto... r) { return f(std::true_type{}, r...); }, bs...)
           : pick([&](auto... r) { return f(std::false_type{}, r...); }, bs...);
}
template <class F>
inline int level_dispatch(int n0, bool f16, bool fwd, F&& f) {
  return pick([&](auto n32, auto h, auto fw) -> int {
    return f(std::integral_constant<int, decltype(n32)::value ? 32 : 16>{}, std::integral_constant<int, decltype(h)::value ? DT_F16 : DT_BF16>{}, fw);
  }, n0 == 32, f16, fwd);
}

template <class F>
inline bool with_geo(int N, F&& f) {
  switch (N) {
    case 256: f(Geo<1, 16, 16>{}); return true;
    case 512: f(Geo<1, 16, 32>{}); return true;
    case 1024: case 2048: f(Geo<1, 32, 32>{}); return true;
    case 4096: f(Geo<16, 16, 16>{}); return true;
    case 8192: f(Geo<32, 16, 16>{}); return true;
    case 16384: f(Geo<16, 32, 32>{}); return true;
    case 32768: case 65536: case 131072: f(Geo<32, 32, 32>{}); return true;
  }
  return false;
}

static constexpr int IPASS_BYTES = 2 * 6144 + 2 * 8192;
static constexpr const char* NO_MULTI_PASS = "multi-pass plan on a geometry without multi-pass kernels";

inline int cap_two_per_cu(int grid, int persist) {
  const int cap = (persist > 0 && persist < (1 << 29)) ? 2 * persist : (1 << 30);
  return grid > cap ? cap : grid;
}

struct FwdRoute {
  bool multi_pass;
  bool half;
  bool sz;
  bool sp;
  int grid, lds_max, lds;
  const char* err;
};
template <class GEO>
inline FwdRoute fwd_route(const ConvArgs& a) {
  FwdRoute r{};
  r.grid = ((a.H + 7) & ~7) * a.nchunk;
  r.lds_max = r.lds = GEO::LDS_BYTES;
  if (a.R > 1) {
    r.multi_pass = true;
    if (GEO::N == 32768) {
      r.half = 16 * GEO::Mi >= a.L;
      r.sz = a.zsave != nullptr;
    } else if (GEO::N == 1024) {
      r.sz = a.zsave || a.yraw;
      r.grid = cap_two_per_cu(r.grid, a.persist);
      r.lds_max = GEO::LDS_BYTES + 2 * IPASS_BYTES;
      r.lds = GEO::LDS_BYTES + a.R * IPASS_BYTES;
    } else {
      r.err = NO_MULTI_PASS;
    }
    return r;
  }
  if (GEO::OUTER && GEO::NW == 1 && r.grid > a.persist) r.grid = a.persist;
  if (!GEO::OUTER && a.persist > 0 && a.persist < (1 << 29) && r.grid > 2 * a.persist) r.grid = 2 * a.persist;
  r.half = GEO::OUTER && (GEO::N1 / 2) * GEO::Mi >= a.L;
  if (a.sparse) {
    if (GEO::HAS_SP) r.sp = true;
    else r.err = "frequency-sparse kernel: fft 16384 / 32768 only";
    return r;
  }
  r.sz = a.zsave || (!GEO::OUTER && a.yraw);
  return r;
}
template <class GEO>
constexpr bool fwd_kernel_exists(bool add, bool multi_pass, bool half, bool sz, bool sp) {
  if (multi_pass) return !sp && (GEO::N == 32768 || (GEO::N == 1024 && !half));
  if (sp) return GEO::HAS_SP && !add && !sz;
  return GEO::OUTER || !half;
}

struct BwdRoute {
  bool multi_pass;
  bool half;
  bool fastk;
  bool small;
  int grid, lds_max, lds;
  const char* err;
};
template <class GEO>
inline BwdRoute bwd_route(const DkfArgs& d, bool dkf) {
  const ConvArgs& c = d.c;
  BwdRoute r{};
  r.grid = ((c.H + 7) & ~7) * c.nchunk;
  r.lds_max = r.lds = GEO::LDS_BYTES;
  if (c.R > 1 && GEO::OUTER) {
    if (GEO::N != 32768) { r.err = NO_MULTI_PASS; return r; }
    r.multi_pass = true;
    r.half = 16 * GEO::Mi >= c.L;
    r.fastk = !dkf && c.fast && (FFC_RP_FASTK != 0);
    return r;
  }
  if (GEO::OUTER) {
    if (GEO::NW == 1 && c.persist > 0 && r.grid > c.persist) r.grid = c.persist;
    r.half = (GEO::N1 / 2) * GEO::Mi >= c.L;
    return r;
  }
  r.small = true;
  if (c.R > 1 && GEO::N != 1024) { r.err = NO_MULTI_PASS; return r; }
  r.lds_max = GEO::LDS_BYTES + 2 * IPASS_BYTES;
  r.lds = GEO::LDS_BYTES + (c.R > 1 ? c.R * IPASS_BYTES : 0);
  if (!dkf) r.grid = cap_two_per_cu(r.grid, c.persist);
  return r;
}

inline bool fwd_takes_kfft(const HostPlan& hp, int nchunk, int sparse, int flags) {
  return nchunk == 1 && hp.N >= 8192 && hp.N <= 32768 && hp.R == 1 && !sparse && !(flags & 64);
}
enum { DK_SEPARATE = 0, DK_TAIL = 1, DK_TAIL_MULTI = 2 };
inline bool bwd_takes_dk(const HostPlan& hp, int nchunk, int flags) {
  return nchunk == 1 && hp.N >= ((flags & 128) ? 8192 : 16384) && hp.N <= 32768 && hp.R == 1 && !(flags & 32);
}
inline bool bwd_takes_dk_multi(const HostPlan& hp, int nchunk, int flags) {
  return nchunk == 1 && hp.R > 1 && hp.N1 > 1 && hp.dtype == DT_BF16 && !(flags & 32);
}
inline int bwd_dk_form(const HostPlan& hp, int nchunk, int flags, bool complex_rows) {
  if (bwd_takes_dk(hp, nchunk, flags)) return DK_TAIL;
  return (!complex_rows && bwd_takes_dk_multi(hp, nchunk, flags)) ? DK_TAIL_MULTI : DK_SEPARATE;
}
inline void set_dk_tail(DkfArgs* d, float* dk, void* pair, int Lk, float scale, int fast, const uint8_t* tab_bf, const PlanTabs& t_bf) {
  d->dk_out = dk; d->dk_pair = pair; d->Lk = Lk; d->dk_scale = scale; d->dk_fast = fast;
  d->tab_bf = tab_bf; d->t_bf = t_bf;
}

inline int decode_dtype(int dtype, int dir, BigArgs* a) {
  a->lf32 = (dtype & 16) ? 1 : 0;
  a->half = (dtype & 32) ? 1 : 0;
  const int e = (dtype >> 8) & 0xff;
  if (e > 30 || (e && !(a->lf32 && dir))) return -1;
  a->lpre = (float)(1u << e);
  return dtype & 15;
}
inline const char* set_long_side(BigArgs* a, int dir, int64_t Hin, int64_t Llong, int64_t pitch_in, int64_t pitch_out, int64_t pitch_gate) {
  const int64_t hl = Hin * Llong;
  if ((dir ? pitch_out : pitch_in) != 0) return "outer pass: the short side (pair-plane tensor) is contiguous, its pitch must be 0";
  int64_t pl = dir ? pitch_in : pitch_out, pg = a->gate ? pitch_gate : 0;
  if (!pl) pl = hl;
  if (!pg) pg = hl;
  if (pl < hl || pg < hl) return "outer pass: a batch pitch is smaller than Hin * Llong";
  if (a->lf32 && pl != hl) return "outer pass: the fp32 long side is contiguous";
  a->pin = dir ? pl : 0; a->pout = dir ? 0 : pl; a->pgate = pg;
  a->strided = (pl != hl || pg != hl) ? 1 : 0;
  a->fast = (Llong % 8 == 0) && !(((uintptr_t)a->in | (uintptr_t)a->out | (uintptr_t)a->gate) & 15) && !((pl | pg) & 7);
  return nullptr;
}
inline bool half_rows_ok(const BigArgs& a, int64_t Bv, int64_t npair) { return !a.half || (Bv == 1 && npair == 1); }
inline const char* set_level(BigArgs* a, int dir, int64_t Bv, int64_t npair, int64_t Hin, int64_t Mi, int64_t Llong, float scale,
                             int64_t pitch_in, int64_t pitch_out, int64_t pitch_gate) {
  a->Bp_valid = (int)Bv; a->npair = (int)npair; a->Hin = (int)Hin; a->Mi = (int)Mi; a->Llong = (int)Llong; a->scale = scale;
  return set_long_side(a, dir, Hin, Llong, pitch_in, pitch_out, pitch_gate);
}
inline bool level_pipe(const BigArgs& a, bool fwd, bool opt_in) {
  return opt_in && a.R == 1 && a.fast && !a.lf32 && !a.half && !a.strided && !(fwd && a.gate);
}
inline bool level_wide(const BigArgs& a) { return a.Llong > 32 * a.Mi; }
inline const char* level_wide_check(const BigArgs& a) {
  if (a.strided) return "outer pass (R passes), wide form: contiguous long side only";
  if (a.lf32 || a.half) return "outer pass (R passes), long side beyond the first 32 rows: 16-bit rows and all short-side rows only";
  if (GeoBig<32>::WGW % a.R) return "outer pass (R passes), wide form: R must divide the workgroup's waves";
  return nullptr;
}
inline int level_wide_cols(int R) { return 128 * (GeoBig<32>::WGW / R); }
inline int64_t level_blocks(const BigArgs& a, int cols) { return (int64_t)a.npair * a.Hin * (a.Mi / cols); }

}
```

flash-fft-conv_amd/csrc/ffc_sim.cpp:

```cpp
#include <math.h>
#include <pthread.h>
#include <stdint.h>
#include <stdlib.h>
#include <string.h>

#include <atomic>
#include <thread>
#include <vector>

#define FFC_FN inline __attribute__((always_inline))
#include "ffc_body.h"
#include "ffc_modes.h"
#include "ffc_big.h"
#include "ffc_route.h"

namespace ffc {

template <class T>
struct Vec {
  T v[64];
  Vec() {}
  Vec(T s) { for (int i = 0; i < 64; i++) v[i] = s; }
};
#define VOP(op)                                                                           \
  template <class T> inline Vec<T> operator op(const Vec<T>& a, const Vec<T>& b) {        \
    Vec<T> r; for (int i = 0; i < 64; i++) r.v[i] = a.v[i] op b.v[i]; return r; }         \
  template <class T> inline Vec<T> operator op(const Vec<T>& a, T b) {                    \
    Vec<T> r; for (int i = 0; i < 64; i++) r.v[i] = a.v[i] op b; return r; }              \
  template <class T> inline Vec<T> operator op(T a, const Vec<T>& b) {                    \
    Vec<T> r; for (int i = 0; i < 64; i++) r.v[i] = a op b.v[i]; return r; }
VOP(+) VOP(-) VOP(*) VOP(/) VOP(%) VOP(&) VOP(|) VOP(^)
#undef VOP
template <class T> inline Vec<T> operator<<(const Vec<T>& a, int s) { Vec<T> r; for (int i = 0; i < 64; i++) r.v[i] = a.v[i] << s; return r; }
template <class T> inline Vec<T> operator>>(const Vec<T>& a, int s) { Vec<T> r; for (int i = 0; i < 64; i++) r.v[i] = a.v[i] >> s; return r; }
inline Vec<uint32_t> operator&(const Vec<uint32_t>& a, unsigned b) { Vec<uint32_t> r; for (int i = 0; i < 64; i++) r.v[i] = a.v[i] & b; return r; }
inline Vec<int> operator*(const Vec<int>& a, long b) { return a * (int)b; }
inline Vec<bool> operator<(const Vec<int>& a, int b) { Vec<bool> r; for (int i = 0; i < 64; i++) r.v[i] = a.v[i] < b; return r; }
inline Vec<bool> operator<(const Vec<int>& a, const Vec<int>& b) { Vec<bool> r; for (int i = 0; i < 64; i++) r.v[i] = a.v[i] < b.v[i]; return r; }
inline Vec<bool> operator>=(const Vec<int>& a, int b) { Vec<bool> r; for (int i = 0; i < 64; i++) r.v[i] = a.v[i] >= b; return r; }
inline Vec<bool> operator&&(const Vec<bool>& a, const Vec<bool>& b) { Vec<bool> r; for (int i = 0; i < 64; i++) r.v[i] = a.v[i] && b.v[i]; return r; }
inline Vec<bool> operator&&(const Vec<bool>& a, bool b) { Vec<bool> r; for (int i = 0; i < 64; i++) r.v[i] = a.v[i] && b; return r; }

struct WgCtx {
  std::vector<uint8_t> lds;
  pthread_barrier_t bar;
  int nwaves;
};
static thread_local WgCtx* g_wg = nullptr;
static thread_local int g_wave = 0;
static thread_local Vec<float> g_agpr[128];
static std::atomic<long> g_dma_count{0};

static inline float dt_to_f32(int DT, uint16_t h) { return DT == DT_BF16 ? bf16_to_f32(h) : f16_to_f32(h); }
static inline uint16_t f32_to_dt(int DT, float f) { return DT == DT_BF16 ? f32_to_bf16(f) : f32_to_f16(f); }

struct SimB {
  static constexpr bool LEAN_OUTER = false;
  static constexpr bool FAST_ONLY = false;
  static constexpr bool HAS_ADD = false;
  using f32 = Vec<float>;
  using i32 = Vec<int>;
  using u32 = Vec<uint32_t>;
  using pred = Vec<bool>;
  struct U2 { u32 x, y; };
  struct U4 { u32 x, y, z, w; };
  struct A16 { f32 v[16]; f32& operator[](int i) { return v[i]; } const f32& operator[](int i) const { return v[i]; } };
  struct W4 { u32 v[4]; u32& operator[](int i) { return v[i]; } const u32& operator[](int i) const { return v[i]; } };
  template <bool CONJ> static void cmul16(A16& re, A16& im, const A16& tr, const A16& ti) {
    for (int r = 0; r < 16; r++) {
      f32 a = re[r], b = im[r];
      if (!CONJ) { re[r] = a * tr[r] - b * ti[r]; im[r] = a * ti[r] + b * tr[r]; }
      else { re[r] = a * tr[r] + b * ti[r]; im[r] = b * tr[r] - a * ti[r]; }
    }
  }
  struct F2 { f32 x, y; };
  static F2 f2(const f32& a, const f32& b) { F2 v; v.x = a; v.y = b; return v; }
  static f32 f2_lo(const F2& v) { return v.x; }
  static f32 f2_hi(const F2& v) { return v.y; }
  static void cmulp(const F2& xr, const F2& xi, const f32& wr, const f32& wi, F2& yr, F2& yi) {
    F2 r, i;
    r.x = xr.x * wr - xi.x * wi; r.y = xr.y * wr - xi.y * wi;
    i.x = xr.x * wi + xi.x * wr; i.y = xr.y * wi + xi.y * wr;
    yr = r; yi = i;
  }
  template <bool CONJ>
  static void cmul2v(A16& re, A16& im, int r0, const F2& tr, const F2& ti) { cmul2<CONJ>(re, im, r0, tr.x, tr.y, ti.x, ti.y); }
  static void cmac2_conj(F2& wr, F2& wi, const A16& a, const A16& b, int r0, const F2& zr, const F2& zi) {
    wr.x = wr.x + (a[r0] * zr.x + b[r0] * zi.x);
    wr.y = wr.y + (a[r0 + 1] * zr.y + b[r0 + 1] * zi.y);
    wi.x = wi.x + (b[r0] * zr.x - a[r0] * zi.x);
    wi.y = wi.y + (b[r0 + 1] * zr.y - a[r0 + 1] * zi.y);
  }
  static void agpr_reserve() {}
  template <int I> static f32 agpr_get() { return g_agpr[I]; }
  template <int I> static void agpr_set(const f32& x) { g_agpr[I] = x; }
  static void pin(W4&) {}
  static void pin4(U4&) {}
  static void sched_fence() {}
  template <bool CONJ>
  static void cmul2(A16& re, A16& im, int r0, const f32& tr0, const f32& tr1, const f32& ti0, const f32& ti1) {
    const f32* tr[2] = {&tr0, &tr1}; const f32* ti[2] = {&ti0, &ti1};
    for (int q = 0; q < 2; q++) {
      f32 a = re[r0 + q], b = im[r0 + q];
      if (!CONJ) { re[r0 + q] = a * *tr[q] - b * *ti[q]; im[r0 + q] = a * *ti[q] + b * *tr[q]; }
      else { re[r0 + q] = a * *tr[q] + b * *ti[q]; im[r0 + q] = b * *tr[q] - a * *ti[q]; }
    }
  }
  static A16 a16_scale(const A16& a, float s) { A16 r; for (int i = 0; i < 16; i++) r[i] = a[i] * f32(s); return r; }
  static A16 a16_zero() { A16 z; for (int i = 0; i < 16; i++) z.v[i] = f32(0.f); return z; }
  static W4 w4(const u32& a, const u32& b, const u32& c, const u32& e) { W4 v; v.v[0] = a; v.v[1] = b; v.v[2] = c; v.v[3] = e; return v; }
  static bool HAS_TR;

  static i32 lane() { i32 r; for (int i = 0; i < 64; i++) r.v[i] = i; return r; }
  static int wave() { return g_wave; }
  static void barrier() { if (g_wg->nwaves > 1) pthread_barrier_wait(&g_wg->bar); }
  static f32 fconst(float c) { return f32(c); }
  static pred ptrue() { return pred(true); }
  static pred pfalse() { return pred(false); }
  static f32 as_f32(const u32& a) { f32 r; for (int i = 0; i < 64; i++) memcpy(&r.v[i], &a.v[i], 4); return r; }
  static u32 as_u32(const f32& a) { u32 r; for (int i = 0; i < 64; i++) memcpy(&r.v[i], &a.v[i], 4); return r; }

  static uint8_t* L() { return g_wg->lds.data(); }
  static void chk(int off, int n) { if (off < 0 || off + n > (int)g_wg->lds.size() || (off & (n - 1))) abort(); }
  static U2 lds_r64(const i32& off) {
    U2 r;
    for (int i = 0; i < 64; i++) { chk(off.v[i], 8); memcpy(&r.x.v[i], L() + off.v[i], 4); memcpy(&r.y.v[i], L() + off.v[i] + 4, 4); }
    return r;
  }
  static void lds_w64(const i32& off, const U2& v) {
    for (int i = 0; i < 64; i++) { chk(off.v[i], 8); memcpy(L() + off.v[i], &v.x.v[i], 4); memcpy(L() + off.v[i] + 4, &v.y.v[i], 4); }
  }
  static void lds_w32(const i32& off, const u32& v) {
    for (int i = 0; i < 64; i++) { chk(off.v[i], 4); memcpy(L() + off.v[i], &v.v[i], 4); }
  }
  static void lds_w128(const i32& off, const U4& v, const pred& p) {
    for (int i = 0; i < 64; i++)
      if (p.v[i]) {
        chk(off.v[i], 16);
        memcpy(L() + off.v[i], &v.x.v[i], 4); memcpy(L() + off.v[i] + 4, &v.y.v[i], 4);
        memcpy(L() + off.v[i] + 8, &v.z.v[i], 4); memcpy(L() + off.v[i] + 12, &v.w.v[i], 4);
      }
  }
  static U4 lds_r128(const i32& off) {
    U4 r;
    for (int i = 0; i < 64; i++) {
      chk(off.v[i], 16);
      memcpy(&r.x.v[i], L() + off.v[i], 4); memcpy(&r.y.v[i], L() + off.v[i] + 4, 4);
      memcpy(&r.z.v[i], L() + off.v[i] + 8, 4); memcpy(&r.w.v[i], L() + off.v[i] + 12, 4);
    }
    return r;
  }
  static void lds_w16(const i32& off, const u32& v) {
    for (int i = 0; i < 64; i++) { chk(off.v[i], 2); uint16_t h = (uint16_t)v.v[i]; memcpy(L() + off.v[i], &h, 2); }
  }
  static u32 lds_r32(const i32& off) {
    u32 r;
    for (int i = 0; i < 64; i++) { chk(off.v[i], 4); memcpy(&r.v[i], L() + off.v[i], 4); }
    return r;
  }
  static u32 lds_r16(const i32& off) {
    u32 r;
    for (int i = 0; i < 64; i++) { chk(off.v[i], 2); uint16_t h; memcpy(&h, L() + off.v[i], 2); r.v[i] = h; }
    return r;
  }
  static U2 lds_r64_tr(const i32& off) {
    U2 r;
    for (int g = 0; g < 4; g++) {
      uint16_t M[16][4];
      for (int i = 0; i < 16; i++) { chk(off.v[g * 16 + i], 8); memcpy(M[i], L() + off.v[g * 16 + i], 8); }
      for (int i = 0; i < 16; i++) {
        uint16_t e[4];
        for (int j = 0; j < 4; j++) e[j] = M[4 * j + (i >> 2)][i & 3];
        r.x.v[g * 16 + i] = e[0] | ((uint32_t)e[1] << 16);
        r.y.v[g * 16 + i] = e[2] | ((uint32_t)e[3] << 16);
      }
    }
    return r;
  }
  static void lds_fence() {}
  template <bool NT>
  static void g2lds32(const void* base, const i32& dw, int lds_off) {
    g_dma_count++;
    for (int i = 0; i < 64; i++) { chk(lds_off + 4 * i, 4); memcpy(L() + lds_off + 4 * i, (const uint32_t*)base + dw.v[i], 4); }
  }
  template <bool NT>
  static void g2lds128(const void* base, const i32& o16, int lds_off) {
    g_dma_count++;
    for (int i = 0; i < 64; i++) { chk(lds_off + 16 * i, 16); memcpy(L() + lds_off + 16 * i, (const uint8_t*)base + 16 * (int64_t)o16.v[i], 16); }
  }
  static void vm_wait0() {}
  static void lds_w32p(const i32& off, const u32& v, const pred& p) {
    for (int i = 0; i < 64; i++) if (p.v[i]) { chk(off.v[i], 4); memcpy(L() + off.v[i], &v.v[i], 4); }
  }
  static pred pnot(const pred& p) { pred r; for (int i = 0; i < 64; i++) r.v[i] = !p.v[i]; return r; }
  static i32 mul24(const i32& a, const i32& b) { return a * b; }
  static unsigned long long clock() { return 0; }
  template <int P> static void setprio() {}
  static U2 u2_from64(unsigned long long v) { U2 r; r.x = u32((uint32_t)v); r.y = u32((uint32_t)(v >> 32)); return r; }
  static void settle(f32&, f32&) {}
  static f32 i2f(const i32& a) { f32 r; for (int i = 0; i < 64; i++) r.v[i] = (float)a.v[i]; return r; }
  static f32 cos_rev(const f32& a) { f32 r; for (int i = 0; i < 64; i++) r.v[i] = (float)cos(6.283185307179586 * (double)a.v[i]); return r; }
  static f32 sin_rev(const f32& a) { f32 r; for (int i = 0; i < 64; i++) r.v[i] = (float)sin(6.283185307179586 * (double)a.v[i]); return r; }
  static i32 opaque(const i32& x) { return x; }
  static u32 uconst(uint32_t c) { return u32(c); }
  static i32 imin(const i32& a, int b) { i32 r; for (int i = 0; i < 64; i++) r.v[i] = a.v[i] < b ? a.v[i] : b; return r; }
  static u32 merge_lo(const u32& a, const u32& b) { u32 r; for (int i = 0; i < 64; i++) r.v[i] = (a.v[i] & 0xffffu) | (b.v[i] << 16); return r; }
  static u32 merge_hi(const u32& a, const u32& b) { u32 r; for (int i = 0; i < 64; i++) r.v[i] = (a.v[i] >> 16) | (b.v[i] & 0xffff0000u); return r; }
  static u32 sel(const pred& p, const u32& a, const u32& b) { u32 r; for (int i = 0; i < 64; i++) r.v[i] = p.v[i] ? a.v[i] : b.v[i]; return r; }
  static u32 g_r16(const void* base, const i32& e, const pred& p) {
    u32 r;
    for (int i = 0; i < 64; i++) { uint16_t h = 0; if (p.v[i]) memcpy(&h, (const uint8_t*)base + (int64_t)e.v[i] * 2, 2); r.v[i] = h; }
    return r;
  }
  static void g_w16(void* base, const i32& e, const u32& v, const pred& p) {
    for (int i = 0; i < 64; i++) if (p.v[i]) { uint16_t h = (uint16_t)v.v[i]; memcpy((uint8_t*)base + (int64_t)e.v[i] * 2, &h, 2); }
  }
  static u32 g_r32(const void* base, const i32& e, const pred& p) {
    u32 r;
    for (int i = 0; i < 64; i++) { uint32_t h = 0; if (p.v[i]) memcpy(&h, (const uint8_t*)base + (int64_t)e.v[i] * 4, 4); r.v[i] = h; }
    return r;
  }
  static void g_w32(void* base, const i32& e, const u32& v, const pred& p) {
    for (int i = 0; i < 64; i++) if (p.v[i]) memcpy((uint8_t*)base + (int64_t)e.v[i] * 4, &v.v[i], 4);
  }
  static U2 g_r64(const void* base, const i32& o8, const pred& p) {
    U2 r;
    for (int i = 0; i < 64; i++) {
      if (p.v[i]) { const uint8_t* q = (const uint8_t*)base + (int64_t)o8.v[i] * 8; memcpy(&r.x.v[i], q, 4); memcpy(&r.y.v[i], q + 4, 4); }
      else { r.x.v[i] = 0; r.y.v[i] = 0; }
    }
    return r;
  }
  static void g_w64(void* base, const i32& o8, const U2& v, const pred& p) {
    for (int i = 0; i < 64; i++)
      if (p.v[i]) { uint8_t* q = (uint8_t*)base + (int64_t)o8.v[i] * 8; memcpy(q, &v.x.v[i], 4); memcpy(q + 4, &v.y.v[i], 4); }
  }
  static U4 g_r128(const void* base, const i32& o16) {
    U4 r;
    for (int i = 0; i < 64; i++) {
      const uint8_t* q = (const uint8_t*)base + (int64_t)o16.v[i] * 16;
      memcpy(&r.x.v[i], q, 4); memcpy(&r.y.v[i], q + 4, 4); memcpy(&r.z.v[i], q + 8, 4); memcpy(&r.w.v[i], q + 12, 4);
    }
    return r;
  }
  static U4 g_r128_nt(const void* base, const i32& o16) { return g_r128(base, o16); }
  static U4 g_r128p(const void* base, const i32& o16, const pred& p) {
    U4 r;
    for (int i = 0; i < 64; i++) {
      if (p.v[i]) {
        const uint8_t* q = (const uint8_t*)base + (int64_t)o16.v[i] * 16;
        memcpy(&r.x.v[i], q, 4); memcpy(&r.y.v[i], q + 4, 4); memcpy(&r.z.v[i], q + 8, 4); memcpy(&r.w.v[i], q + 12, 4);
      } else { r.x.v[i] = r.y.v[i] = r.z.v[i] = r.w.v[i] = 0; }
    }
    return r;
  }
  static void g_w128(void* base, const i32& o16, const U4& v, const pred& p) {
    for (int i = 0; i < 64; i++)
      if (p.v[i]) {
        uint8_t* q = (uint8_t*)base + (int64_t)o16.v[i] * 16;
        memcpy(q, &v.x.v[i], 4); memcpy(q + 4, &v.y.v[i], 4); memcpy(q + 8, &v.z.v[i], 4); memcpy(q + 12, &v.w.v[i], 4);
      }
  }
  static void g_w128_nt(void* base, const i32& o16, const U4& v, const pred& p) { g_w128(base, o16, v, p); }
  template <int DT>
  static void mfma(A16& acc, const W4& a, const W4& b) {
    float A[32][16], Bm[16][32];
    for (int l = 0; l < 64; l++)
      for (int e = 0; e < 8; e++) {
        uint16_t ha = (uint16_t)(a[e >> 1].v[l] >> (16 * (e & 1)));
        uint16_t hb = (uint16_t)(b[e >> 1].v[l] >> (16 * (e & 1)));
        A[l & 31][8 * (l >> 5) + e] = dt_to_f32(DT, ha);
        Bm[8 * (l >> 5) + e][l & 31] = dt_to_f32(DT, hb);
      }
    for (int l = 0; l < 64; l++)
      for (int r = 0; r < 16; r++) {
        int i = acc_row(r, l >> 5), j = l & 31;
        float s = 0;
        for (int k = 0; k < 16; k++) s += A[i][k] * Bm[k][j];
        acc[r].v[l] += s;
      }
  }
  template <int DT> static u32 pack(const f32& lo, const f32& hi) {
    u32 r;
    for (int i = 0; i < 64; i++) r.v[i] = f32_to_dt(DT, lo.v[i]) | ((uint32_t)f32_to_dt(DT, hi.v[i]) << 16);
    return r;
  }
  static u32 pk_mul_f16(const u32& a, const u32& b) {
    u32 r;
    for (int i = 0; i < 64; i++) {
      float lo = f16_to_f32((uint16_t)a.v[i]) * f16_to_f32((uint16_t)b.v[i]);
      float hi = f16_to_f32((uint16_t)(a.v[i] >> 16)) * f16_to_f32((uint16_t)(b.v[i] >> 16));
      r.v[i] = f32_to_f16(lo) | ((uint32_t)f32_to_f16(hi) << 16);
    }
    return r;
  }
  template <int DT> static f32 unpack_lo(const u32& a) { f32 r; for (int i = 0; i < 64; i++) r.v[i] = dt_to_f32(DT, (uint16_t)a.v[i]); return r; }
  template <int DT> static f32 unpack_hi(const u32& a) { f32 r; for (int i = 0; i < 64; i++) r.v[i] = dt_to_f32(DT, (uint16_t)(a.v[i] >> 16)); return r; }
};
bool SimB::HAS_TR = true;
struct SimBO : SimB { static constexpr bool LEAN_OUTER = true; };
struct SimBA : SimB { static constexpr bool HAS_ADD = true; };
struct SimBOF : SimBO { static constexpr bool FAST_ONLY = true; };
static bool g_force_slow = false;

template <class F>
static void run_wg(int nwaves, int lds_bytes, F fn) {
  WgCtx ctx;
  ctx.lds.assign(lds_bytes, 0xCD);
  ctx.nwaves = nwaves;
  pthread_barrier_init(&ctx.bar, nullptr, nwaves);
  std::vector<std::thread> th;
  for (int w = 0; w < nwaves; w++)
    th.emplace_back([&, w]() { g_wg = &ctx; g_wave = w; fn(); });
  for (auto& t : th) t.join();
  pthread_barrier_destroy(&ctx.bar);
}

static constexpr int NO_KERNEL = -8;
template <class GEO> constexpr int sim_lds() { return GEO::LDS_BYTES + (GEO::OUTER ? 0 : 4 * IPASS_BYTES); }
template <class F>
static int sim_jobs(int H, int nchunk, int lds, F job) {
  for (int h = 0; h < H; h++)
    for (int c = 0; c < nchunk; c++) run_wg(8, lds, [&]() { job(h, c); });
  return 0;
}

template <class GEO, int DT, class SB = SimB>
static int sim_conv_t(const ConvArgs& a) {
  using BD = Body<SB, GEO, DT>;
  static_assert(BD::IPASS_BYTES == IPASS_BYTES && GEO::WGW == 8, "ffc_route.h");
  const FwdRoute r = fwd_route<GEO>(a);
  if (r.err) return NO_KERNEL;
  return pick([&](auto mp, auto half, auto sz, auto sp) -> int {
    constexpr bool MP = decltype(mp)::value, HALF = decltype(half)::value, SZ = decltype(sz)::value, SP = decltype(sp)::value;
    if constexpr (!fwd_kernel_exists<GEO>(SB::HAS_ADD, MP, HALF, SZ, SP)) {
      return NO_KERNEL;
    } else if constexpr (MP) {
      return sim_jobs(a.H, a.nchunk, r.lds, [&](int h, int c) {
        BD::setup_tables(a.tab, a.t);
        if constexpr (!GEO::OUTER) BD::setup_tables_ipass(a.tab, a.t, a.R);
        BD::template conv_job<HALF, true, SZ>(a, h, c);
      });
    } else {
      return sim_jobs(a.H, a.nchunk, r.lds, [&](int h, int c) {
        if constexpr (GEO::OUTER && GEO::NW > 1 && !SP && !SB::HAS_ADD) {
          if (a.kfuse_k || a.kfuse_x) {
            BD::setup_tables(a.tab, a.t);
            Modes<SB, GEO, DT>::kfft_head(a, h);
            BD::template conv_job<HALF, false, SZ>(a, h, c);
            return;
          }
        }
        BD::template conv<HALF, SZ, SP>(a, h, c);
      });
    }
  }, r.multi_pass, r.half, r.sz, r.sp);
}

template <template <class, int> class FN, class... A>
static int dispatch(int N, int dtype, A&&... args) {
  int rc = 0;
  const bool found = with_geo(N, [&](auto geo) {
    using GEO = decltype(geo);
    rc = dtype == DT_BF16 ? FN<GEO, DT_BF16>::run(args...) : FN<GEO, DT_F16>::run(args...);
  });
  return found ? rc : -1;
}
template <class GEO, int DT> struct ConvRun { static int run(const ConvArgs& a) { return sim_conv_t<GEO, DT>(a); } };
template <class GEO, int DT> struct ConvResRun { static int run(const ConvArgs& a) { return sim_conv_t<GEO, DT, SimBA>(a); } };
template <class GEO, int DT> struct KfRun {
  static int run(const KfArgs& a) {
    const int nunits = GEO::OUTER ? a.H : (a.H + GEO::G - 1) / GEO::G;
    for (int wg = 0; wg < (nunits + GEO::UPW - 1) / GEO::UPW; wg++)
      run_wg(GEO::WGW, sim_lds<GEO>(), [&]() { Modes<SimB, GEO, DT>::kfft(a, wg); });
    return 0;
  }
};
template <class GEO, int DT, bool DKF>
static int sim_bwd_t(const DkfArgs& d) {
  using MO = Modes<SimBO, GEO, DT>;
  const BwdRoute r = bwd_route<GEO>(d, DKF);
  if (r.err) return NO_KERNEL;
  const int H = d.c.H, nchunk = d.c.nchunk, lds = sim_lds<GEO>();
  return pick([&](auto mp, auto half, auto fastk, auto zm) -> int {
    constexpr bool MP = decltype(mp)::value, HALF = decltype(half)::value, FASTK = decltype(fastk)::value, ZM = decltype(zm)::value;
    if constexpr (!GEO::OUTER) {
      if constexpr (MP || HALF || FASTK || ZM) return NO_KERNEL;
      else if constexpr (DKF) return sim_jobs(H, nchunk, lds, [&](int h, int c) { MO::dkf(d, h, c, h * nchunk + c); });
      else return sim_jobs(H, nchunk, lds, [&](int h, int c) { MO::bwd(d, h, c, h * nchunk + c); });
    } else if constexpr (MP) {
      if constexpr (GEO::N != 32768 || (DKF && (FASTK || ZM))) {
        return NO_KERNEL;
      } else {
        using MK = Modes<typename std::conditional<FASTK, SimBOF, SimBO>::type, GEO, DT>;
        return sim_jobs(H, nchunk, lds, [&](int h, int c) {
          MK::BD::setup_tables(d.c.tab, d.c.t);
          for (int k0 = 0; k0 < d.c.R; k0++) {
            if constexpr (DKF) MK::template dkf<HALF, true>(d, h, c, h * nchunk + c, k0, SimBO::wave());
            else MK::template bwd<HALF, true>(d, h, c, h * nchunk + c, k0, SimBO::wave());
          }
        });
      }
    } else if constexpr (FASTK || (DKF && ZM)) {
      return NO_KERNEL;
    } else if constexpr (DKF) {
      return sim_jobs(H, nchunk, lds, [&](int h, int c) { MO::template dkf<HALF>(d, h, c, h * nchunk + c); });
    } else if constexpr (ZM) {
      return sim_jobs(H, nchunk, lds, [&](int h, int c) { MO::template bwd<HALF, false, true, 1>(d, h, c, h * nchunk + c); });
    } else {
      return sim_jobs(H, nchunk, lds, [&](int h, int c) { MO::template bwd<HALF>(d, h, c, h * nchunk + c); });
    }
  }, r.multi_pass, r.half, r.fastk, !DKF && GEO::OUTER && !r.multi_pass && d.zin != nullptr);
}
template <class GEO, int DT> struct DkfRun { static int run(const DkfArgs& d) { return sim_bwd_t<GEO, DT, true>(d); } };
template <class GEO, int DT> struct BwdRun { static int run(const DkfArgs& d) { return sim_bwd_t<GEO, DT, false>(d); } };
template <class GEO, int DT> struct DkRun {
  static int run(const DkArgs& a) {
    const int nunits = GEO::OUTER ? a.H : (a.H + GEO::G - 1) / GEO::G;
    for (int wg = 0; wg < (nunits + GEO::UPW - 1) / GEO::UPW; wg++)
      run_wg(GEO::WGW, sim_lds<GEO>(), [&]() { Modes<SimB, GEO, DT>::dkifft(a, wg); });
    return 0;
  }
};
template <class GEO, int DT> struct UpwGet { static int run(int* out) { *out = GEO::UPW; return 0; } };

}

using namespace ffc;

extern "C" {

void ffcsim_set_tr(int on) { SimB::HAS_TR = on != 0; }
void ffcsim_force_slow_io(int on) { g_force_slow = on != 0; }

int ffcsim_selftest_primitives(const uint32_t* in, uint32_t* out) {
  run_wg(1, 1024, [&]() {
    using Bk = SimB;
    Bk::W4 a, b;
    for (int i = 0; i < 4; i++) for (int l = 0; l < 64; l++) { a[i].v[l] = in[l * 8 + i]; b[i].v[l] = in[l * 8 + 4 + i]; }
    Bk::A16 acc = Bk::a16_zero(), acc2 = Bk::a16_zero();
    Bk::mfma<DT_BF16>(acc, a, b);
    Bk::mfma<DT_F16>(acc2, a, b);
    Bk::i32 lane = Bk::lane();
    Bk::U2 w; w.x = a[0]; w.y = a[1];
    Bk::lds_w64(lane * 8, w);
    Bk::U2 t = Bk::lds_r64_tr(((lane * 5 + 3) & 63) * 8);
    Bk::u32 p0 = Bk::pack<DT_BF16>(acc[0], acc[1]), p1 = Bk::pack<DT_F16>(acc[0], acc[1]);
    Bk::f32 u0 = Bk::unpack_lo<DT_F16>(a[2]), u1 = Bk::unpack_hi<DT_F16>(a[2]);
    Bk::f32 u2 = Bk::unpack_lo<DT_BF16>(a[2]), u3 = Bk::unpack_hi<DT_BF16>(a[2]);
    for (int l = 0; l < 64; l++) {
      for (int i = 0; i < 16; i++) { memcpy(&out[l * 40 + i], &acc[i].v[l], 4); memcpy(&out[l * 40 + 16 + i], &acc2[i].v[l], 4); }
      out[l * 40 + 32] = t.x.v[l]; out[l * 40 + 33] = t.y.v[l];
      out[l * 40 + 34] = p0.v[l]; out[l * 40 + 35] = p1.v[l];
      memcpy(&out[l * 40 + 36], &u0.v[l], 4); memcpy(&out[l * 40 + 37], &u1.v[l], 4);
      memcpy(&out[l * 40 + 38], &u2.v[l], 4); memcpy(&out[l * 40 + 39], &u3.v[l], 4);
    }
  });
  return 0;
}

int ffcsim_plan_info(int N, int dtype, int* nt, double* s_fwd, double* s_k, int32_t* kf_freq ) {
  HostPlan p;
  if (!build_plan(N, dtype, &p)) return -1;
  *nt = p.NT * p.R; *s_fwd = p.s_fwd; *s_k = p.s_k;
  if (kf_freq) memcpy(kf_freq, p.kf_freq.data(), p.kf_freq.size() * 4);
  return 0;
}

static int g_sparse_rows = 0;
void ffcsim_set_sparse(int rows) { g_sparse_rows = rows; }
static void* g_z = nullptr; static void* g_yraw = nullptr; static int g_flags = 0;
void ffcsim_set_z(void* z, void* yraw, int flags) { g_z = z; g_yraw = yraw; g_flags = flags; }
long ffcsim_dma_count() { return g_dma_count.exchange(0); }
static float* g_dk_out = nullptr; static int g_dk_lk = 0;
void ffcsim_set_fused_dk(float* dk, int Lk) { g_dk_out = dk; g_dk_lk = Lk; }
static const float* g_kfuse_k = nullptr; static int g_kfuse_lk = 0;
void ffcsim_set_fused_k(const float* k, int Lk) { g_kfuse_k = k; g_kfuse_lk = Lk; }
static const void* g_kfuse_x = nullptr; static float g_kfuse_xscale = 1.f;
void ffcsim_set_fused_kx(const void* xpair, float scale) { g_kfuse_x = xpair; g_kfuse_xscale = scale; }
static void* g_dk_pair = nullptr; static float g_dk_pair_scale = 1.f;
void ffcsim_set_fused_dkpair(void* outpair, float scale) { g_dk_pair = outpair; g_dk_pair_scale = scale; }
static int g_big_pipe = 0;
void ffcsim_set_big_pipe(int on) { g_big_pipe = on; }
int ffcsim_conv_fwd(int N, int dtype, const void* u, const void* kf, const void* pregate, const void* postgate,
                    void* y, int B, int H, int L, int conj_kf) {
  HostPlan p;
  if (!build_plan(N, dtype, &p)) return -1;
  if (L > N || L <= 0) return -2;
  ConvArgs a{};
  a.u = u; a.pregate = pregate; a.postgate = postgate; a.y = y; a.kf = kf;
  a.tab = p.blob.data(); a.t = p.tabs;
  a.B = B; a.H = H; a.L = L; a.npair = (B + 1) / 2;
  a.sbu = a.sbg = a.sbp = a.sby = (int64_t)H * L;
  a.nchunk = 1; a.ppc = a.npair; a.conj_kf = conj_kf; a.s_inv = (float)p.s_inv; a.s_fwd = (float)p.s_fwd;
  a.fast = (L % 8 == 0) && !g_force_slow;
  a.R = p.R;
  a.sparse = g_sparse_rows;
  if (p.N1 > 1 && p.R == 1) { a.zsave = g_z; a.yraw = g_z ? g_yraw : nullptr; }
  if (p.N1 <= 1) { a.zsave = g_z; a.yraw = g_yraw; }
  const bool kfuse = fwd_takes_kfft(p, a.nchunk, a.sparse, 0);
  if (g_kfuse_x && kfuse) {
    a.kfuse_x = g_kfuse_x; a.kfuse_scale = g_kfuse_xscale; a.kfuse_Lk = N; a.kfuse_fast = 1;
  }
  if (g_kfuse_k && kfuse) {
    a.kfuse_k = g_kfuse_k; a.kfuse_Lk = g_kfuse_lk; a.kfuse_scale = (float)(p.s_k / p.s_fwd) / (dtype == DT_F16 ? 256.f : 1.f); a.kfuse_fast = (g_kfuse_lk % 4 == 0) && !g_force_slow;
  }
  return dispatch<ConvRun>(N, dtype, a);
}

int ffcsim_conv_fwd_res(int N, int dtype, const void* u, const void* kf, const void* pregate, const void* postgate, const void* addend,
                        void* y, void* zsave, void* y_raw, int B, int H, int L, int conj_kf, int64_t sb_u, int64_t sb_pre, int64_t sb_post,
                        int64_t sb_add, int64_t sb_y) {
  HostPlan p;
  if (!build_plan(N, dtype, &p)) return -1;
  if (L > N || L <= 0 || B <= 0 || H <= 0) return -2;
  if (y_raw && !zsave && p.N1 > 1) return -3;
  const int64_t hl = (int64_t)H * L;
  if (!sb_u) sb_u = hl; if (!sb_pre) sb_pre = hl; if (!sb_post) sb_post = hl; if (!sb_add) sb_add = hl; if (!sb_y) sb_y = hl;
  if (sb_u < hl || sb_pre < hl || sb_post < hl || sb_add < hl || sb_y < hl) return -2;
  if (addend) {
    const uintptr_t a0 = (uintptr_t)addend, a1 = a0 + (uintptr_t)(((B - 1) * sb_add + hl) * 2);
    const uintptr_t y0 = (uintptr_t)y, y1 = y0 + (uintptr_t)(((B - 1) * sb_y + hl) * 2);
    if (a0 < y1 && y0 < a1) return -4;
  }
  ConvArgs a{};
  a.u = u; a.pregate = pregate; a.postgate = postgate; a.y = y; a.kf = kf; a.addend = addend;
  a.tab = p.blob.data(); a.t = p.tabs;
  a.B = B; a.H = H; a.L = L; a.npair = (B + 1) / 2;
  a.sbu = sb_u; a.sbg = sb_pre; a.sbp = sb_post; a.sby = sb_y; a.sba = sb_add;
  a.nchunk = 1; a.ppc = a.npair; a.conj_kf = conj_kf; a.s_inv = (float)p.s_inv; a.s_fwd = (float)p.s_fwd;
  a.fast = (L % 8 == 0) && !((sb_u | sb_pre | sb_post | sb_y | sb_add) & 7) && !g_force_slow;
  a.R = p.R;
  a.zsave = zsave; a.yraw = y_raw;
  if (!addend) return dispatch<ConvRun>(N, dtype, a);
  return dispatch<ConvResRun>(N, dtype, a);
}



static int sim_level_args(BigArgs* a, int* dtype, int fwd, const void* in, void* out, const void* gate, int Bp_valid, int npair, int Hin, int Mi,
                          int Llong, float scale, int64_t pitch_in, int64_t pitch_out, int64_t pitch_gate) {
  *dtype = decode_dtype(*dtype, fwd, a);
  if (*dtype < 0) return -1;
  if (!half_rows_ok(*a, Bp_valid, npair)) return -4;
  if (Llong <= 0) return -5;
  if (pitch_in || pitch_out || (gate && pitch_gate)) { a->in = in; a->out = out; a->gate = gate; }
  const bool bad = set_level(a, fwd, Bp_valid, npair, Hin, Mi, Llong, scale, pitch_in, pitch_out, pitch_gate) != nullptr;
  a->in = in; a->out = out; a->gate = gate;
  if (bad) return -7;
  if (g_force_slow) a->fast = 0;
  return 0;
}
int ffcsim_big_outer_r_strided(int N0, int R, int c, int dtype, int fwd, const void* in, void* out, const void* gate, int Bp_valid, int npair,
                               int Hin, int Mi, int Llong, float scale, int64_t pitch_in, int64_t pitch_out, int64_t pitch_gate) {
  HostPlan p;
  if (R > 1 && N0 != 32) return -3;
  BigArgs a{};
  a.R = R; a.c = c;
  const int rc = sim_level_args(&a, &dtype, fwd, in, out, gate, Bp_valid, npair, Hin, Mi, Llong, scale, pitch_in, pitch_out, pitch_gate);
  if (!build_plan(R > 1 ? 32768 * R : (N0 == 16 ? 16384 : 32768), dtype, &p)) return -1;
  if (rc) return rc;
  a.fmat = p.blob.data() + (R > 1 ? p.tabs.matk[c][fwd ? 0 : 1] : p.tabs.mat[0]);
  if (Mi % (N0 == 16 ? GeoBig<16>::Mi : GeoBig<32>::Mi)) return -2;
  const bool pipe = level_pipe(a, fwd != 0, g_big_pipe != 0);
  return level_dispatch(N0, dtype == DT_F16, fwd != 0, [&](auto n0, auto dt, auto fw) -> int {
    constexpr int NN = decltype(n0)::value, DD = decltype(dt)::value;
    constexpr bool FF = decltype(fw)::value;
    const int nblk = (int)level_blocks(a, GeoBig<NN>::Mi), npw = pipe ? (nblk < 3 ? nblk : 3) : nblk;
    for (int wg = 0; wg < npw; wg++)
      run_wg(GeoBig<NN>::WGW + (pipe ? 1 : 0), pipe ? BigBody<SimB, NN, DD>::PIPE_LDS : GeoBig<NN>::LDS_BYTES, [&]() {
        if (pipe) BigBody<SimB, NN, DD>::template run_pipe<FF>(a, wg, npw);
        else if (a.strided) BigBody<SimB, NN, DD, true>::template run<FF>(a, wg);
        else BigBody<SimB, NN, DD>::template run<FF>(a, wg);
      });
    return 0;
  });
}
int ffcsim_big_outer_r(int N0, int R, int c, int dtype, int fwd, const void* in, void* out, const void* gate, int Bp_valid, int npair,
                       int Hin, int Mi, int Llong, float scale) {
  return ffcsim_big_outer_r_strided(N0, R, c, dtype, fwd, in, out, gate, Bp_valid, npair, Hin, Mi, Llong, scale, 0, 0, 0);
}
int ffcsim_big_outer(int N0, int dtype, int fwd, const void* in, void* out, const void* gate, int Bp_valid, int npair,
                     int Hin, int Mi, int Llong, float scale) {
  return ffcsim_big_outer_r(N0, 1, 0, dtype, fwd, in, out, gate, Bp_valid, npair, Hin, Mi, Llong, scale);
}
int ffcsim_big_outer_strided(int N0, int dtype, int fwd, const void* in, void* out, const void* gate, int Bp_valid, int npair,
                             int Hin, int Mi, int Llong, float scale, int64_t pitch_in, int64_t pitch_out, int64_t pitch_gate) {
  return ffcsim_big_outer_r_strided(N0, 1, 0, dtype, fwd, in, out, gate, Bp_valid, npair, Hin, Mi, Llong, scale, pitch_in, pitch_out, pitch_gate);
}

int ffcsim_big_outer_all_strided(int R, int dtype, int fwd, const void* in, void* out, const void* gate, int Bp_valid, int npair,
                                 int Hin, int Mi, int Llong, float scale, int64_t pitch_in, int64_t pitch_out, int64_t pitch_gate) {
  HostPlan p;
  BigArgs a{};
  a.R = R; a.c = 0;
  const int rc = sim_level_args(&a, &dtype, fwd, in, out, gate, Bp_valid, npair, Hin, Mi, Llong, scale, pitch_in, pitch_out, pitch_gate);
  if (R < 2 || R > 4 || !build_plan(32768 * R, dtype, &p)) return -1;
  if (rc) return rc;
  for (int c = 0; c < R; c++) a.fmats[c] = p.blob.data() + p.tabs.matk[c][fwd ? 0 : 1];
  a.fmat = a.fmats[0];
  if (Mi % GeoBig<32>::Mi) return -2;
  if (Llong > R * 32 * Mi) return -5;
  if (level_wide(a)) {
    BigArgs w = a;
    w.strided = 0;
    if (level_wide_check(w)) return -6;
    if (pitch_in || pitch_out || pitch_gate) return -7;
    a.wide = 1;
  }
  return level_dispatch(32, dtype == DT_F16, fwd != 0, [&](auto n0, auto dt, auto fw) -> int {
    constexpr int DD = decltype(dt)::value;
    constexpr bool FF = decltype(fw)::value;
    if constexpr (decltype(n0)::value != 32) return -3;
    const int nblk = (int)level_blocks(a, a.wide ? level_wide_cols(a.R) : GeoBig<32>::Mi);
    for (int wg = 0; wg < nblk; wg++)
      run_wg(GeoBig<32>::WGW, GeoBig<32>::LDS_BYTES, [&]() {
        if (a.wide) BigBody<SimB, 32, DD>::template run_wide<FF>(a, wg);
        else if (a.strided) BigBody<SimB, 32, DD, true>::template run_all<FF>(a, wg);
        else BigBody<SimB, 32, DD>::template run_all<FF>(a, wg);
      });
    return 0;
  });
}
int ffcsim_big_outer_all(int R, int dtype, int fwd, const void* in, void* out, const void* gate, int Bp_valid, int npair,
                         int Hin, int Mi, int Llong, float scale) {
  return ffcsim_big_outer_all_strided(R, dtype, fwd, in, out, gate, Bp_valid, npair, Hin, Mi, Llong, scale, 0, 0, 0);
}

int ffcsim_upw(int N) { int u = 0; dispatch<UpwGet>(N, 0, &u); return u; }

int ffcsim_launch_route(int N, int dtype, int B, int H, int L, int nchunk, int persist, int flags, int* out) {
  HostPlan p;
  if (!build_plan(N, dtype, &p)) return -1;
  static char buf[16];
  DkfArgs d{};
  ConvArgs& a = d.c;
  a.B = B; a.H = H; a.L = L; a.npair = (B + 1) / 2; a.nchunk = nchunk; a.persist = persist; a.R = p.R;
  a.zsave = (flags & (1 << 16)) ? buf : nullptr; a.yraw = (flags & (1 << 17)) ? buf : nullptr;
  a.sparse = (flags & (1 << 18)) ? 2 : 0; a.fast = (flags & (1 << 19)) ? 1 : 0;
  with_geo(N, [&](auto geo) {
    using GEO = decltype(geo);
    const FwdRoute f = fwd_route<GEO>(a);
    const int fo[8] = {f.multi_pass, f.half, f.sz, f.sp, f.grid, f.lds_max, f.lds, f.err != nullptr};
    memcpy(out, fo, sizeof fo);
    for (int dkf = 0; dkf < 2; dkf++) {
      const BwdRoute b = bwd_route<GEO>(d, dkf != 0);
      const int bo[8] = {b.multi_pass, b.half, b.fastk, b.small, b.grid, b.lds_max, b.lds, b.err != nullptr};
      memcpy(out + 8 + 8 * dkf, bo, sizeof bo);
    }
  });
  out[24] = fwd_takes_kfft(p, nchunk, a.sparse, flags & 0xffff);
  out[25] = bwd_dk_form(p, nchunk, flags & 0xffff, false);
  out[26] = bwd_dk_form(p, nchunk, flags & 0xffff, true);
  return 0;
}

int ffcsim_kernel_fft_c(int N, int dtype, const void* xpair, int H, void* kf, float scale) {
  HostPlan p;
  if (!build_plan(N, dtype, &p)) return -1;
  KfArgs a{};
  a.xpair = xpair; a.kf = kf; a.tab = p.blob.data(); a.t = p.tabs; a.H = H; a.Lk = N; a.scale = scale; a.prescale = 1.f; a.s_fwd = (float)p.s_fwd; a.fast = 1;
  a.R = p.R;
  return dispatch<KfRun>(N, dtype, a);
}

int ffcsim_kernel_fft(int N, int dtype, const float* k, int H, int Lk, void* kf) {
  HostPlan p;
  if (!build_plan(N, dtype, &p)) return -1;
  KfArgs a{};
  a.k = k; a.kf = kf; a.tab = p.blob.data(); a.t = p.tabs; a.H = H; a.Lk = Lk;
  a.s_fwd = (float)p.s_fwd;
  a.prescale = dtype == DT_F16 ? 256.f : 1.f;
  a.scale = (float)(p.s_k / p.s_fwd) / a.prescale; a.fast = (Lk % 4 == 0) && !g_force_slow;
  a.R = p.R;
  return dispatch<KfRun>(N, dtype, a);
}

int ffcsim_conv_bwd_dkf(int N, int dtype, const void* dout, const void* u, const void* pregate, const void* postgate,
                        float* ws, int B, int H, int L, int nchunk) {
  HostPlan p;
  if (!build_plan(N, dtype, &p)) return -1;
  DkfArgs d{};
  ConvArgs& a = d.c;
  a.u = u; a.pregate = pregate; a.postgate = postgate; a.tab = p.blob.data(); a.t = p.tabs;
  a.B = B; a.H = H; a.L = L; a.npair = (B + 1) / 2; a.s_fwd = (float)p.s_fwd;
  a.sbu = a.sbg = a.sbp = a.sby = (int64_t)H * L; d.sbd = d.sbdu = d.sbdpre = d.sbdpost = (int64_t)H * L;
  int upw = ffcsim_upw(N);
  int per_iter = p.N1 > 1 ? upw : upw * p.G;
  int iters_total = (a.npair + per_iter - 1) / per_iter;
  if (nchunk > iters_total) nchunk = iters_total;
  int ipc = (iters_total + nchunk - 1) / nchunk;
  a.ppc = ipc * per_iter; a.nchunk = (a.npair + a.ppc - 1) / a.ppc;
  a.fast = (L % 8 == 0) && !g_force_slow;
  a.R = p.R;
  d.dout = dout; d.ws = ws;
  std::vector<uint8_t> zs((size_t)H * a.nchunk * upw * N * 4 + 16);
  d.zscratch = zs.data();
  int rc = dispatch<DkfRun>(N, dtype, d);
  return rc < 0 ? rc : a.nchunk;
}

int ffcsim_conv_bwd(int N, int dtype, const void* dout, const void* u, const void* kf, const void* pregate, const void* postgate,
                    void* du, void* dpre, void* dpost, float* ws, int B, int H, int L, int nchunk) {
  HostPlan p;
  if (!build_plan(N, dtype, &p)) return -1;
  DkfArgs d{};
  ConvArgs& a = d.c;
  a.u = u; a.kf = kf; a.pregate = pregate; a.postgate = postgate; a.tab = p.blob.data(); a.t = p.tabs;
  a.B = B; a.H = H; a.L = L; a.npair = (B + 1) / 2; a.s_inv = (float)p.s_inv; a.s_fwd = (float)p.s_fwd;
  a.sbu = a.sbg = a.sbp = a.sby = (int64_t)H * L; d.sbd = d.sbdu = d.sbdpre = d.sbdpost = (int64_t)H * L;
  int upw = ffcsim_upw(N);
  int per_iter = p.N1 > 1 ? upw : upw * p.G;
  int iters_total = (a.npair + per_iter - 1) / per_iter;
  if (nchunk > iters_total) nchunk = iters_total;
  int ipc = (iters_total + nchunk - 1) / nchunk;
  a.ppc = ipc * per_iter; a.nchunk = (a.npair + a.ppc - 1) / a.ppc;
  a.fast = (L % 8 == 0) && !g_force_slow;
  a.R = p.R;
  d.dout = dout; d.ws = ws; d.du = du; d.dpre = dpre; d.dpost = (p.N1 > 1 || g_yraw) ? dpost : nullptr;
  if (p.N1 > 1 && p.R == 1 && g_z) { d.zin = g_z; d.yraw = g_yraw; a.flags = g_flags; a.stream = 1; }
  if (p.N1 <= 1) { d.zin = g_z; d.yraw = dpost ? g_yraw : nullptr; }
  HostPlan pbf;
  if (g_dk_pair && bwd_dk_form(p, a.nchunk, 128, true) != DK_SEPARATE) {
    if (!build_plan(N, DT_BF16, &pbf)) return -1;
    set_dk_tail(&d, nullptr, g_dk_pair, N, g_dk_pair_scale, 1, pbf.blob.data(), pbf.tabs);
  } else if (g_dk_out && bwd_dk_form(p, a.nchunk, 128, false) != DK_SEPARATE) {
    if (!build_plan(N, DT_BF16, &pbf)) return -1;
    set_dk_tail(&d, g_dk_out, nullptr, g_dk_lk, (float)(1.0 / p.s_fwd), (g_dk_lk % 4 == 0) && !g_force_slow, pbf.blob.data(), pbf.tabs);
  }
  std::vector<uint8_t> zs((size_t)H * a.nchunk * upw * N * 4 + 16);
  d.zscratch = zs.data();
  int rc = dispatch<BwdRun>(N, dtype, d);
  return rc < 0 ? rc : a.nchunk;
}

int ffcsim_kernel_ifft_grad_c(int N, const float* ws, int nslab, int H, void* outpair, float scale) {
  HostPlan p;
  if (!build_plan(N, DT_BF16, &p)) return -1;
  DkArgs a{};
  a.ws = ws; a.outpair = outpair; a.tab = p.blob.data(); a.t = p.tabs; a.H = H; a.Lk = N; a.nslab = nslab; a.scale = scale; a.s_inv = (float)p.s_inv; a.fast = 1;
  a.R = p.R;
  return dispatch<DkRun>(N, DT_BF16, a);
}

int ffcsim_kernel_ifft_grad(int N, int dtype, const float* ws, int nslab, int H, int Lk, float* dk) {
  HostPlan p;
  (void)dtype;
  dtype = DT_BF16;
  if (!build_plan(N, dtype, &p)) return -1;
  DkArgs a{};
  a.ws = ws; a.dk = dk; a.tab = p.blob.data(); a.t = p.tabs; a.H = H; a.Lk = Lk; a.nslab = nslab;
  a.scale = (float)(1.0 / p.s_fwd); a.s_inv = (float)p.s_inv;
  a.fast = (Lk % 4 == 0) && !g_force_slow;
  a.R = p.R;
  return dispatch<DkRun>(N, dtype, a);
}

}
```

Before: 10.58 million seq/s.

## Use half-height 16x16 MFMA inverse outer stage with direct global store for fft 32768

Adds a specialised inverse outer FFT stage for the 32x32x32 geometry that computes only the half of the output rows needed when L <= N/2. It uses 16x16x32 MFMA tiles with a register-pinned DFT matrix. A new direct-store route writes the result straight from registers to global memory, with optional nontemporal stores, and skips the LDS round trip and the separate rows_out pass. It is wired into the forward and backward kernel launch routes. The cost is more kernel variants and register pressure, and the route-selection logic (r.gs) is only partly shown.

```diff
diff --git a/flash-fft-conv_amd/csrc/ffc_body.h b/flash-fft-conv_amd/csrc/ffc_body.h
--- a/flash-fft-conv_amd/csrc/ffc_body.h
+++ b/flash-fft-conv_amd/csrc/ffc_body.h
@@ -1221,9 +1221,98 @@
     }
   }
 
+  static constexpr bool HALF_C = GEO::N1 == 32 && GEO::N2 == 32 && GEO::N3 == 32;
+  using A4 = typename B::A4;
+  struct NoMid { FFC_FN void operator()() const {} };
+  template <bool GS, class MID>
+  static FFC_FN void outer_inv_half_cols(int hc, Unit un, const W4& Cr, const W4& Ci, const W4& Cn, const ConvArgs* a, int h, int pq, MID mid) {
+    const i32 lane = B::opaque(B::lane());
+    const i32 c = lane & 15, g = lane >> 4;
+    const i32 m0 = c * 4 + (hc * 64 + un.wq * 128);
+    const i32 colr = e_off<GEO, i32>((g >> 1) * 16 + (g & 1) * 4, m0) + un.eb;
+    U2 rawr[8], rawi[8];
+#pragma unroll
+    for (int e = 0; e < 8; e++) {
+      i32 off = colr + kslot_row(0, 0, e) * (GEO::Mi * 2);
+      rawr[e] = B::lds_r64(off); rawi[e] = B::lds_r64(off + GEO::PLANE);
+    }
+    A4 re[4], im[4];
+#pragma unroll
+    for (int t = 0; t < 4; t++) {
+      W4 dr, di;
+#pragma unroll
+      for (int d = 0; d < 4; d++) {
+        const u32 ar = (t & 2) ? rawr[2 * d].y : rawr[2 * d].x, br = (t & 2) ? rawr[2 * d + 1].y : rawr[2 * d + 1].x;
+        const u32 ai = (t & 2) ? rawi[2 * d].y : rawi[2 * d].x, bi = (t & 2) ? rawi[2 * d + 1].y : rawi[2 * d + 1].x;
+        dr[d] = (t & 1) ? B::merge_hi(ar, br) : B::merge_lo(ar, br);
+        di[d] = (t & 1) ? B::merge_hi(ai, bi) : B::merge_lo(ai, bi);
+      }
+      re[t] = B::a4_zero(); im[t] = B::a4_zero();
+      B::template mfma16<DT>(re[t], Cr, dr);
+      B::template mfma16<DT>(im[t], Ci, dr);
+      B::template mfma16<DT>(re[t], Cn, di);
+      B::template mfma16<DT>(im[t], Cr, di);
+      if (t == 0) mid();
+    }
+    U2 wr[4], wi[4];
+#pragma unroll
+    for (int r = 0; r < 4; r++) {
+      wr[r].x = B::template pack<DT>(re[0][r], re[1][r]); wr[r].y = B::template pack<DT>(re[2][r], re[3][r]);
+      wi[r].x = B::template pack<DT>(im[0][r], im[1][r]); wi[r].y = B::template pack<DT>(im[2][r], im[3][r]);
+    }
+    if constexpr (!GS) {
+      const i32 colw = e_off<GEO, i32>(g * 4, m0) + un.eb;
+#pragma unroll
+      for (int r = 0; r < 4; r++) {
+        B::lds_w64(colw + r * (GEO::Mi * 2), wr[r]);
+        B::lds_w64(colw + (r * (GEO::Mi * 2) + GEO::PLANE), wi[r]);
+      }
+    } else {
+      const i32 n = g * (4 * GEO::Mi) + m0;
+#pragma unroll
+      for (int pl = 0; pl < 2; pl++) {
+        const int b = 2 * pq + pl;
+        const bool ok = b < a->B;
+        uint16_t* base = (uint16_t*)a->y + row_off(b, ok, a->sby, h, a->L);
+        if (a->stream) {
+#pragma unroll
+          for (int r = 0; r < 4; r++) B::g_w64_nt(base, (n + r * GEO::Mi) >> 2, pl ? wi[r] : wr[r], ((n + r * GEO::Mi) < a->L) && ok);
+        } else {
+#pragma unroll
+          for (int r = 0; r < 4; r++) B::g_w64(base, (n + r * GEO::Mi) >> 2, pl ? wi[r] : wr[r], ((n + r * GEO::Mi) < a->L) && ok);
+        }
+      }
+    }
+  }
+  template <bool GS>
+  static FFC_FN void outer_inv_half(Unit un, const ConvArgs* a = nullptr, int h = 0, int pq = 0) { outer_inv_half<GS>(un, a, h, pq, NoMid()); }
+  template <bool GS, class LAST>
+  static FFC_FN void outer_inv_half(Unit un, const ConvArgs* a, int h, int pq, LAST last) {
+    static_assert(HALF_C && GEO::S1 == 1 && GEO::NW == 8, "half-height phase C: fft 32768");
+    static_assert(!GS || !B::HAS_ADD, "the direct store has no addend");
+    const i32 lane = B::opaque(B::lane());
+    const i32 toff = ((lane & 15) + ((lane >> 4) & 1) * 32) * 16 + (lane >> 5) * 3072 + GEO::L_F1;
+    U4 v0 = B::lds_r128(toff), v1 = B::lds_r128(toff + 1024), v2 = B::lds_r128(toff + 2048);
+    W4 Cr = B::w4(v0.x, v0.y, v0.z, v0.w);
+    W4 Ci = B::w4(v2.x, v2.y, v2.z, v2.w);
+    W4 Cn = B::w4(v1.x, v1.y, v1.z, v1.w);
+    B::pin(Cr); B::pin(Ci); B::pin(Cn);
+    if constexpr (B::LEAN_OUTER) {
+#pragma unroll 1
+      for (int hc = 0; hc < 2; hc++)
+        outer_inv_half_cols<GS>(hc, un, Cr, Ci, Cn, a, h, pq, [&]() { if (hc == 1) last(); });
+    } else {
+      outer_inv_half_cols<GS>(0, un, Cr, Ci, Cn, a, h, pq, NoMid());
+      outer_inv_half_cols<GS>(1, un, Cr, Ci, Cn, a, h, pq, last);
+    }
+  }
+
   template <bool FWD, bool HALF, bool RP = false, bool DIN = false, bool NOTW = false>
-  static FFC_FN void outer_stage(int L, Unit un, float s_fwd = 1.0f, Pass ps = Pass()) {
+  static FFC_FN void outer_stage(int L, Unit un, float s_fwd = 1.0f, Pass ps = Pass(), int flags = 0) {
     if constexpr (DIN) { outer_stage_pair<FWD, HALF, RP, true, NOTW>(L, un, s_fwd, ps); return; }
+    if constexpr (!FWD && HALF && !RP && HALF_C) {
+      if (!(flags & 256)) { outer_inv_half<false>(un); return; }
+    }
     if constexpr (B::LEAN_OUTER && !(FWD && HALF && GEO::N1 == 32)) outer_stage_tile<FWD, HALF, RP, NOTW>(L, un, s_fwd, ps);
     else if constexpr (!B::LEAN_OUTER && FFC_OUTER_QUAD != 0 && HALF) outer_stage_quad<FWD, HALF, RP, NOTW>(L, un, s_fwd, ps);
     else outer_stage_pair<FWD, HALF, RP, false, NOTW>(L, un, s_fwd, ps);
@@ -1955,8 +2044,9 @@
     if constexpr (GEO::NW > 1) B::barrier();
     else B::lds_fence();
   }
-  template <bool HALF, bool PROF = false, bool RP = false, bool SZ = false, bool SP = false>
+  template <bool HALF, bool PROF = false, bool RP = false, bool SZ = false, bool SP = false, bool GS = false>
   static FFC_FN void outer_jobs(const ConvArgs& a, int h, int p0, int p1, int u, Unit un, int wg_linear = 0) {
+    static_assert(!GS || (HALF && !RP && !SP && HALF_C), "direct-store phase C: single-pass fft 32768, L <= N/2");
     constexpr int NC = HALF ? NCH / 2 : NCH;
     constexpr bool PREFETCH = HALF && !RP;
     constexpr bool FOLDF = CAN_FOLD && !RP && !SP && !PROF && !B::LEAN_OUTER;
@@ -2044,8 +2134,13 @@
       FFC_TICK(4)
       FFC_PRIO(3)
       if constexpr (PREFETCH) { if (it + 1 < iters && p + GEO::UPW < p1) rows_load<NC>(a, h, p + GEO::UPW, un, X); }
-      if (act) {
-        outer_stage<false, HALF, RP>(a.L, un, 1.0f, ps);
+      if constexpr (GS) {
+        if (act) {
+          outer_inv_half<true>(un, &a, h, p);
+          FFC_TICK(5)
+        }
+      } else if (act) {
+        outer_stage<false, HALF, RP>(a.L, un, 1.0f, ps, a.flags);
         B::lds_fence();
         FFC_TICK(5)
         FFC_PRIO(2)
@@ -2072,12 +2167,12 @@
     }
   }
 
-  template <bool HALF = false, bool SZ = false, bool SP = false>
+  template <bool HALF = false, bool SZ = false, bool SP = false, bool GS = false>
   static FFC_FN void conv(const ConvArgs& a, int h, int chunk) {
     setup_tables(a.tab, a.t);
-    conv_job<HALF, false, SZ, SP>(a, h, chunk);
-  }
-  template <bool HALF = false, bool RP = false, bool SZ = false, bool SP = false>
+    conv_job<HALF, false, SZ, SP, GS>(a, h, chunk);
+  }
+  template <bool HALF = false, bool RP = false, bool SZ = false, bool SP = false, bool GS = false>
   static FFC_FN void conv_job(const ConvArgs& a, int h, int chunk) {
     const int wv = B::wave();
     Unit un;
@@ -2088,7 +2183,7 @@
     int p1 = p0 + a.ppc;
     if (p1 > a.npair) p1 = a.npair;
     if constexpr (GEO::OUTER) {
-      outer_jobs<HALF, false, RP, SZ, SP>(a, h, p0, p1, u, un);
+      outer_jobs<HALF, false, RP, SZ, SP, GS>(a, h, p0, p1, u, un);
     } else {
       const int q0 = p0 / GEO::G, q1 = (p1 + GEO::G - 1) / GEO::G;
       const int iters = (q1 - q0 + GEO::UPW - 1) / GEO::UPW;
diff --git a/flash-fft-conv_amd/csrc/ffc_bwd_launch.h b/flash-fft-conv_amd/csrc/ffc_bwd_launch.h
--- a/flash-fft-conv_amd/csrc/ffc_bwd_launch.h
+++ b/flash-fft-conv_amd/csrc/ffc_bwd_launch.h
@@ -6,7 +6,7 @@
 #include "ffc_dev.h"
 using namespace ffc;
 
-template <class GEO, int DT, bool HALF, int ZM>
+template <class GEO, int DT, bool HALF, int ZM, bool GS = false>
 __global__ __launch_bounds__(GEO::WGW * 64, 2) __attribute__((amdgpu_num_vgpr(128))) void bwd_kernel(DkfArgs d) {
   if constexpr (GEO::NW == 1) {
     const int total = ((d.c.H + 7) & ~7) * d.c.nchunk;
@@ -18,7 +18,7 @@
     int h, chunk;
     if (!map_block(d.c.H, d.c.nchunk, &h, &chunk)) return;
     stagger_start(d.c.flags);
-    Modes<DevBO, GEO, DT>::template bwd<HALF, false, true, ZM>(d, h, chunk, blockIdx.x);
+    Modes<DevBO, GEO, DT>::template bwd<HALF, false, true, ZM, GS>(d, h, chunk, blockIdx.x);
   }
 }
 template <class GEO, int DT>
@@ -56,6 +56,11 @@
       return ffc_fail("single-tile sizes are launched by the recomputing unit (run-time spectrum switch)");
     } else if constexpr (!GEO::OUTER) {
       return ffc_launch(bwd_kernel_small<GEO, DT>, "bwd_kernel", r.grid, T_, r.lds_max, r.lds, st, d);
+    } else if (r.gs) {
+      if constexpr (GEO::N == 32768)
+        return ffc_launch(bwd_kernel<GEO, DT, true, ZM, true>, "bwd_kernel (direct store)", r.grid, T_, r.lds_max, r.lds, st, d);
+      else
+        return ffc_fail("internal: the backward route names a kernel that does not exist");
     } else {
       return pick([&](auto mp, auto half, auto fastk) -> int {
         constexpr bool MP = decltype(mp)::value, HALF = decltype(half)::value, FASTK = decltype(fastk)::value;
diff --git a/flash-fft-conv_amd/csrc/ffc_conv_launch.h b/flash-fft-conv_amd/csrc/ffc_conv_launch.h
--- a/flash-fft-conv_amd/csrc/ffc_conv_launch.h
+++ b/flash-fft-conv_amd/csrc/ffc_conv_launch.h
@@ -10,6 +10,14 @@
     static_assert(Body<DevB, GEO, DT>::IPASS_BYTES == IPASS_BYTES, "ffc_route.h");
     const FwdRoute r = fwd_route<GEO>(a);
     if (r.err) return ffc_fail(r.err);
+    if (r.gs) {
+      if constexpr (!FAM::HAS_ADD && GEO::N == 32768)
+        return pick([&](auto sz) -> int {
+          return ffc_launch(FAM::template kernel_gs<GEO, DT, decltype(sz)::value>(), FAM::what(false, decltype(sz)::value, false, true), r.grid, GEO::WGW * 64, r.lds_max, r.lds, st, a);
+        }, r.sz);
+      else
+        return ffc_fail("internal: the forward route names a kernel that does not exist");
+    }
     return pick([&](auto mp, auto half, auto sz, auto sp) -> int {
       constexpr bool MP = decltype(mp)::value, HALF = decltype(half)::value, SZ = decltype(sz)::value, SP = decltype(sp)::value;
       if constexpr (fwd_kernel_exists<GEO>(FAM::HAS_ADD, MP, HALF, SZ, SP))
diff --git a/flash-fft-conv_amd/csrc/ffc_dev.h b/flash-fft-conv_amd/csrc/ffc_dev.h
--- a/flash-fft-conv_amd/csrc/ffc_dev.h
+++ b/flash-fft-conv_amd/csrc/ffc_dev.h
@@ -24,6 +24,8 @@
 typedef float f32x16 __attribute__((ext_vector_type(16)));
 typedef short s16x4 __attribute__((ext_vector_type(4)));
 typedef uint32_t u32x4v __attribute__((ext_vector_type(4)));
+typedef uint32_t u32x2v __attribute__((ext_vector_type(2)));
+typedef float f32x4 __attribute__((ext_vector_type(4)));
 
 extern __shared__ __attribute__((aligned(16))) uint8_t ffc_smem[];
 
@@ -39,6 +41,7 @@
   static constexpr bool HAS_ADD = false;
   using A16 = f32x16;
   using W4 = u32x4v;
+  using A4 = f32x4;
   static constexpr bool HAS_TR = true;
   template <bool CONJ> static FFC_FN void cmul16(A16& re, A16& im, const A16& tr, const A16& ti) {
     const A16 a = re, b = im;
@@ -89,6 +92,7 @@
   }
   static FFC_FN A16 a16_scale(const A16& a, float s) { return a * s; }
   static FFC_FN A16 a16_zero() { A16 z = {0.f, 0.f, 0.f, 0.f, 0.f, 0.f, 0.f, 0.f, 0.f, 0.f, 0.f, 0.f, 0.f, 0.f, 0.f, 0.f}; return z; }
+  static FFC_FN A4 a4_zero() { A4 z = {0.f, 0.f, 0.f, 0.f}; return z; }
   static FFC_FN W4 w4(u32 a, u32 b, u32 c, u32 e) { W4 v = {a, b, c, e}; return v; }
 
   static FFC_FN i32 lane() { return (int)(threadIdx.x & 63); }
@@ -131,6 +135,7 @@
     else __builtin_amdgcn_global_load_lds(g, l, 16, 0, 0);
   }
   static FFC_FN void vm_wait0() { __builtin_amdgcn_s_waitcnt(0x0F70); }
+  static FFC_FN void lds_wait0() { __builtin_amdgcn_s_waitcnt(0xC07F); __builtin_amdgcn_sched_barrier(0); }
   static FFC_FN void lds_w32p(i32 off, u32 v, pred p) { if (p) *(uint32_t*)(ffc_smem + off) = v; }
   static FFC_FN pred pnot(pred p) { return !p; }
   static FFC_FN u32 uconst(uint32_t c) { return c; }
@@ -171,6 +176,9 @@
   static FFC_FN void g_w64(void* base, i32 o8, U2 v, pred p) {
     if (p) ((uint2*)base)[o8] = make_uint2(v.x, v.y);
   }
+  static FFC_FN void g_w64_nt(void* base, i32 o8, U2 v, pred p) {
+    if (p) { u32x2v t = {v.x, v.y}; __builtin_nontemporal_store(t, ((u32x2v*)base) + o8); }
+  }
   static FFC_FN U4 g_r128(const void* base, i32 o16) {
     uint4 v = ((const uint4*)base)[o16];
     return U4{v.x, v.y, v.z, v.w};
@@ -196,6 +204,13 @@
       acc = __builtin_amdgcn_mfma_f32_32x32x16_bf16(__builtin_bit_cast(bf16x8, a), __builtin_bit_cast(bf16x8, b), acc, 0, 0, 0);
     else
       acc = __builtin_amdgcn_mfma_f32_32x32x16_f16(__builtin_bit_cast(f16x8, a), __builtin_bit_cast(f16x8, b), acc, 0, 0, 0);
+  }
+  template <int DT>
+  static FFC_FN void mfma16(A4& acc, const W4& a, const W4& b) {
+    if (DT == DT_BF16)
+      acc = __builtin_amdgcn_mfma_f32_16x16x32_bf16(__builtin_bit_cast(bf16x8, a), __builtin_bit_cast(bf16x8, b), acc, 0, 0, 0);
+    else
+      acc = __builtin_amdgcn_mfma_f32_16x16x32_f16(__builtin_bit_cast(f16x8, a), __builtin_bit_cast(f16x8, b), acc, 0, 0, 0);
   }
   template <int DT>
   static FFC_FN u32 pack(f32 lo, f32 hi) {
diff --git a/flash-fft-conv_amd/csrc/ffc_k_conv.hip b/flash-fft-conv_amd/csrc/ffc_k_conv.hip
--- a/flash-fft-conv_amd/csrc/ffc_k_conv.hip
+++ b/flash-fft-conv_amd/csrc/ffc_k_conv.hip
@@ -2,7 +2,7 @@
 using namespace ffc;
 
 static constexpr int SMALL_WAVES = 2;
-template <class GEO, int DT, bool HALF, bool SZ = false, bool SP = false>
+template <class GEO, int DT, bool HALF, bool SZ = false, bool SP = false, bool GS = false>
 __global__ __launch_bounds__(GEO::WGW * 64, GEO::OUTER ? 2 : SMALL_WAVES) void conv_kernel(ConvArgs a) {
   using BD = Body<DevB, GEO, DT>;
   if constexpr (GEO::OUTER && GEO::NW == 1) {
@@ -26,9 +26,9 @@
     if constexpr (GEO::NW > 1 && !SP) {
       BD::setup_tables(a.tab, a.t);
       if (a.kfuse_k || a.kfuse_x) Modes<DevB, GEO, DT>::kfft_head(a, h);
-      BD::template conv_job<HALF, false, SZ, SP>(a, h, chunk);
+      BD::template conv_job<HALF, false, SZ, SP, GS>(a, h, chunk);
     } else {
-      BD::template conv<HALF, SZ, SP>(a, h, chunk);
+      BD::template conv<HALF, SZ, SP, GS>(a, h, chunk);
     }
   }
 }
@@ -59,6 +59,8 @@
     if constexpr (MP) return conv_rp_kernel<GEO, DT, HALF, SZ>;
     else return conv_kernel<GEO, DT, HALF, SZ, SP>;
   }
+  template <class GEO, int DT, bool SZ>
+  static constexpr auto kernel_gs() { return conv_kernel<GEO, DT, true, SZ, false, true>; }
   static const char* what(bool mp, bool sz, bool sp, bool outer) {
     if (mp) return sz && outer ? "conv_rp_kernel (spectrum-saving)" : "conv_rp_kernel";
     if (sz) return outer ? "conv_kernel (spectrum-saving)" : "conv_kernel (spectrum-saving, single tile)";
@@ -203,7 +205,7 @@
   return ffc_conv_fwd_strided(p, u, kf, pregate, postgate, y, B, H, L, conj_kf, 0, 0, 0, 0, stream);
 }
 
-template <class GEO, int DT>
+template <class GEO, int DT, bool GS = false>
 __global__ __launch_bounds__(GEO::WGW * 64, 2) void conv_prof_kernel(ConvArgs a) {
   int h, chunk;
   if (!map_block(a.H, a.nchunk, &h, &chunk)) return;
@@ -217,7 +219,8 @@
   const int p0 = chunk * a.ppc;
   int p1 = p0 + a.ppc;
   if (p1 > a.npair) p1 = a.npair;
-  if (16 * GEO::Mi >= a.L) BD::template outer_jobs<true, true>(a, h, p0, p1, u, un, blockIdx.x);
+  if constexpr (GS) BD::template outer_jobs<true, true, false, false, false, true>(a, h, p0, p1, u, un, blockIdx.x);
+  else if (16 * GEO::Mi >= a.L) BD::template outer_jobs<true, true>(a, h, p0, p1, u, un, blockIdx.x);
   else BD::template outer_jobs<false, true>(a, h, p0, p1, u, un, blockIdx.x);
 }
 
@@ -228,13 +231,15 @@
   ConvArgs a{};
   a.u = u; a.y = y; a.kf = kf; a.tab = p->d_blob; a.t = p->hp.tabs;
   a.B = (int)B; a.H = (int)H; a.L = (int)L; a.npair = (int)((B + 1) / 2); a.s_inv = (float)p->hp.s_inv; a.s_fwd = (float)p->hp.s_fwd;
-  a.fast = (L % 8 == 0);
+  a.fast = (L % 8 == 0) && !(((uintptr_t)u | (uintptr_t)y) & 15);
   a.sbu = a.sbg = a.sbp = a.sby = H * L;
   a.flags = p->env_flags;
   a.prof = prof;
   ffc_choose_chunks(p, a.H, a.npair, &a.nchunk, &a.ppc);
-  const int grid = fwd_route<GEO>(a).grid;
+  const FwdRoute r = fwd_route<GEO>(a);
+  const int grid = r.grid;
   if (grid_out) *grid_out = grid;
+  if (r.gs) return ffc_launch(conv_prof_kernel<GEO, DT_BF16, true>, "conv_prof_kernel", grid, GEO::WGW * 64, GEO::LDS_BYTES, GEO::LDS_BYTES, (hipStream_t)stream, a);
   return ffc_launch(conv_prof_kernel<GEO, DT_BF16>, "conv_prof_kernel", grid, GEO::WGW * 64, GEO::LDS_BYTES, GEO::LDS_BYTES, (hipStream_t)stream, a);
 }
 
diff --git a/flash-fft-conv_amd/csrc/ffc_modes.h b/flash-fft-conv_amd/csrc/ffc_modes.h
--- a/flash-fft-conv_amd/csrc/ffc_modes.h
+++ b/flash-fft-conv_amd/csrc/ffc_modes.h
@@ -864,8 +864,9 @@
     }
     BD::cmul_conj(re, im, k);
   }
-  template <bool HALF = false, bool RP = false, bool SETUP = true, int ZM = -1>
+  template <bool HALF = false, bool RP = false, bool SETUP = true, int ZM = -1, bool GS = false>
   static FFC_FN void bwd(const DkfArgs& d, int h, int chunk, int wg_linear, int k0 = 0, int wv_in = 0) {
+    static_assert(!GS || (HALF && !RP && BD::HALF_C), "direct-store phase C: single-pass fft 32768, L <= N/2");
     const ConvArgs& a = d.c;
     const Pass ps = RP ? make_pass(a.tab, a.t, a.R, k0) : Pass();
     const int hk = RP ? h * a.R + k0 : h;
@@ -934,7 +935,7 @@
             }
             BD::unit_barrier();
             if (act) {
-              BD::template outer_stage<false, HALF, RP>(a.L, un, 1.0f, ps);
+              BD::template outer_stage<false, HALF, RP>(a.L, un, 1.0f, ps, a.flags);
               B::lds_fence();
               if constexpr (RP) BD::template rows_out_rp<NCX>(aq, h, p, un, ps);
               else BD::template rows_out<NCX>(aq, h, p, un);
@@ -988,7 +989,7 @@
           FFC_BPRIO(1)
           if (dpost_tf) {
             if (act) {
-              BD::template outer_stage<false, HALF, RP>(a.L, un, 1.0f, ps);
+              BD::template outer_stage<false, HALF, RP>(a.L, un, 1.0f, ps, a.flags);
               B::lds_fence();
               if constexpr (RP) BD::template rows_out_rp<NCX>(aq, h, p, un, ps);
               else BD::template rows_out<NCX>(aq, h, p, un);
@@ -1013,8 +1014,16 @@
         }
         BD::unit_barrier();
         FFC_BPRIO(3)
-        if (act) {
-          BD::template outer_stage<false, HALF, RP>(a.L, un, 1.0f, ps);
+        if constexpr (GS) {
+          if (act) {
+            BD::template outer_inv_half<true>(un, &ao, h, p, [&]() {
+              if constexpr (DMA_OK) {
+                if (dma && p + GEO::UPW < p1) { B::lds_wait0(); BD::rows_dma(ad, h, p + GEO::UPW, un); }
+              }
+            });
+          }
+        } else if (act) {
+          BD::template outer_stage<false, HALF, RP>(a.L, un, 1.0f, ps, a.flags);
           B::lds_fence();
           if constexpr (DMA_OK) { if (dma && p + GEO::UPW < p1) BD::rows_dma(ad, h, p + GEO::UPW, un); }
           FFC_BPRIO(2)
diff --git a/flash-fft-conv_amd/csrc/ffc_route.h b/flash-fft-conv_amd/csrc/ffc_route.h
--- a/flash-fft-conv_amd/csrc/ffc_route.h
+++ b/flash-fft-conv_amd/csrc/ffc_route.h
@@ -50,7 +50,12 @@
   bool sp;
   int grid, lds_max, lds;
   const char* err;
+  bool gs;
 };
+template <class GEO>
+inline bool direct_store_ok(bool half, bool multi_pass, int fast, bool plain, int flags) {
+  return GEO::N == 32768 && half && !multi_pass && fast && plain && !(flags & 256);
+}
 template <class GEO>
 inline FwdRoute fwd_route(const ConvArgs& a) {
   FwdRoute r{};
@@ -80,6 +85,7 @@
     return r;
   }
   r.sz = a.zsave || (!GEO::OUTER && a.yraw);
+  r.gs = direct_store_ok<GEO>(r.half, false, a.fast, !a.postgate && !a.addend && !a.yraw, a.flags);
   return r;
 }
 template <class GEO>
@@ -96,6 +102,7 @@
   bool small;
   int grid, lds_max, lds;
   const char* err;
+  bool gs;
 };
 template <class GEO>
 inline BwdRoute bwd_route(const DkfArgs& d, bool dkf) {
@@ -113,6 +120,7 @@
   if (GEO::OUTER) {
     if (GEO::NW == 1 && c.persist > 0 && r.grid > c.persist) r.grid = c.persist;
     r.half = (GEO::N1 / 2) * GEO::Mi >= c.L;
+    r.gs = !dkf && direct_store_ok<GEO>(r.half, false, c.fast, !c.pregate && !d.dpre, c.flags);
     return r;
   }
   r.small = true;
diff --git a/flash-fft-conv_amd/csrc/ffc_sim.cpp b/flash-fft-conv_amd/csrc/ffc_sim.cpp
--- a/flash-fft-conv_amd/csrc/ffc_sim.cpp
+++ b/flash-fft-conv_amd/csrc/ffc_sim.cpp
@@ -50,6 +50,8 @@
 static thread_local int g_wave = 0;
 static thread_local Vec<float> g_agpr[128];
 static std::atomic<long> g_dma_count{0};
+static std::atomic<long> g_gs_count{0};
+static int g_sim_flags = 0;
 
 static inline float dt_to_f32(int DT, uint16_t h) { return DT == DT_BF16 ? bf16_to_f32(h) : f16_to_f32(h); }
 static inline uint16_t f32_to_dt(int DT, float f) { return DT == DT_BF16 ? f32_to_bf16(f) : f32_to_f16(f); }
@@ -66,6 +68,8 @@
   struct U4 { u32 x, y, z, w; };
   struct A16 { f32 v[16]; f32& operator[](int i) { return v[i]; } const f32& operator[](int i) const { return v[i]; } };
   struct W4 { u32 v[4]; u32& operator[](int i) { return v[i]; } const u32& operator[](int i) const { return v[i]; } };
+  struct A4 { f32 v[4]; f32& operator[](int i) { return v[i]; } const f32& operator[](int i) const { return v[i]; } };
+  static A4 a4_zero() { A4 z; for (int i = 0; i < 4; i++) z.v[i] = f32(0.f); return z; }
   template <bool CONJ> static void cmul16(A16& re, A16& im, const A16& tr, const A16& ti) {
     for (int r = 0; r < 16; r++) {
       f32 a = re[r], b = im[r];
@@ -189,6 +193,7 @@
     for (int i = 0; i < 64; i++) { chk(lds_off + 16 * i, 16); memcpy(L() + lds_off + 16 * i, (const uint8_t*)base + 16 * (int64_t)o16.v[i], 16); }
   }
   static void vm_wait0() {}
+  static void lds_wait0() {}
   static void lds_w32p(const i32& off, const u32& v, const pred& p) {
     for (int i = 0; i < 64; i++) if (p.v[i]) { chk(off.v[i], 4); memcpy(L() + off.v[i], &v.v[i], 4); }
   }
@@ -235,6 +240,7 @@
     for (int i = 0; i < 64; i++)
       if (p.v[i]) { uint8_t* q = (uint8_t*)base + (int64_t)o8.v[i] * 8; memcpy(q, &v.x.v[i], 4); memcpy(q + 4, &v.y.v[i], 4); }
   }
+  static void g_w64_nt(void* base, const i32& o8, const U2& v, const pred& p) { g_w64(base, o8, v, p); }
   static U4 g_r128(const void* base, const i32& o16) {
     U4 r;
     for (int i = 0; i < 64; i++) {
@@ -280,6 +286,24 @@
         acc[r].v[l] += s;
       }
   }
+  template <int DT>
+  static void mfma16(A4& acc, const W4& a, const W4& b) {
+    float A[16][32], Bm[32][16];
+    for (int l = 0; l < 64; l++)
+      for (int e = 0; e < 8; e++) {
+        uint16_t ha = (uint16_t)(a[e >> 1].v[l] >> (16 * (e & 1)));
+        uint16_t hb = (uint16_t)(b[e >> 1].v[l] >> (16 * (e & 1)));
+        A[l & 15][8 * (l >> 4) + e] = dt_to_f32(DT, ha);
+        Bm[8 * (l >> 4) + e][l & 15] = dt_to_f32(DT, hb);
+      }
+    for (int l = 0; l < 64; l++)
+      for (int r = 0; r < 4; r++) {
+        int i = 4 * (l >> 4) + r, j = l & 15;
+        float s = 0;
+        for (int k = 0; k < 32; k++) s += A[i][k] * Bm[k][j];
+        acc[r].v[l] += s;
+      }
+  }
   template <int DT> static u32 pack(const f32& lo, const f32& hi) {
     u32 r;
     for (int i = 0; i < 64; i++) r.v[i] = f32_to_dt(DT, lo.v[i]) | ((uint32_t)f32_to_dt(DT, hi.v[i]) << 16);
@@ -331,6 +355,20 @@
   static_assert(BD::IPASS_BYTES == IPASS_BYTES && GEO::WGW == 8, "ffc_route.h");
   const FwdRoute r = fwd_route<GEO>(a);
   if (r.err) return NO_KERNEL;
+  if (r.gs) {
+    if constexpr (!SB::HAS_ADD && GEO::N == 32768) {
+      g_gs_count++;
+      return pick([&](auto sz) -> int {
+        return sim_jobs(a.H, a.nchunk, r.lds, [&](int h, int c) {
+          BD::setup_tables(a.tab, a.t);
+          if (a.kfuse_k || a.kfuse_x) Modes<SB, GEO, DT>::kfft_head(a, h);
+          BD::template conv_job<true, false, decltype(sz)::value, false, true>(a, h, c);
+        });
+      }, r.sz);
+    } else {
+      return NO_KERNEL;
+    }
+  }
   return pick([&](auto mp, auto half, auto sz, auto sp) -> int {
     constexpr bool MP = decltype(mp)::value, HALF = decltype(half)::value, SZ = decltype(sz)::value, SP = decltype(sp)::value;
     if constexpr (!fwd_kernel_exists<GEO>(SB::HAS_ADD, MP, HALF, SZ, SP)) {
@@ -382,6 +420,15 @@
   const BwdRoute r = bwd_route<GEO>(d, DKF);
   if (r.err) return NO_KERNEL;
   const int H = d.c.H, nchunk = d.c.nchunk, lds = sim_lds<GEO>();
+  if (r.gs) {
+    if constexpr (GEO::N == 32768) {
+      g_gs_count++;
+      if (d.zin) return sim_jobs(H, nchunk, lds, [&](int h, int c) { MO::template bwd<true, false, true, 1, true>(d, h, c, h * nchunk + c); });
+      return sim_jobs(H, nchunk, lds, [&](int h, int c) { MO::template bwd<true, false, true, 0, true>(d, h, c, h * nchunk + c); });
+    } else {
+      return NO_KERNEL;
+    }
+  }
   return pick([&](auto mp, auto half, auto fastk, auto zm) -> int {
     constexpr bool MP = decltype(mp)::value, HALF = decltype(half)::value, FASTK = decltype(fastk)::value, ZM = decltype(zm)::value;
     if constexpr (!GEO::OUTER) {
@@ -424,6 +471,29 @@
 };
 template <class GEO, int DT> struct UpwGet { static int run(int* out) { *out = GEO::UPW; return 0; } };
 
+template <int DT>
+static void sim_outer_inv_half(const HostPlan& p, const uint16_t* e_in, uint16_t* e_out) {
+  using GEO = Geo<32, 32, 32>;
+  using BD = Body<SimB, GEO, DT>;
+  run_wg(8, GEO::LDS_BYTES, [&]() {
+    BD::setup_tables(p.blob.data(), p.tabs);
+    typename BD::Unit un;
+    un.eb = 0; un.wq = g_wave;
+    if (g_wave == 0)
+      for (int pl = 0; pl < 2; pl++)
+        for (int row = 0; row < 32; row++)
+          for (int m = 0; m < 1024; m++)
+            memcpy(SimB::L() + pl * GEO::PLANE + e_off<GEO, int>(row, m), &e_in[(pl * 32 + row) * 1024 + m], 2);
+    SimB::barrier();
+    BD::template outer_inv_half<false>(un);
+    SimB::barrier();
+    if (g_wave == 0)
+      for (int pl = 0; pl < 2; pl++)
+        for (int row = 0; row < 16; row++)
+          for (int m = 0; m < 1024; m++)
+            memcpy(&e_out[(pl * 16 + row) * 1024 + m], SimB::L() + pl * GEO::PLANE + e_off<GEO, int>(row, m), 2);
+  });
+}
 }
 
 using namespace ffc;
@@ -459,6 +529,26 @@
   return 0;
 }
 
+int ffcsim_mfma16(int dtype, const uint32_t* a, const uint32_t* b, float* d) {
+  SimB::W4 wa, wb;
+  SimB::A4 acc;
+  for (int l = 0; l < 64; l++)
+    for (int i = 0; i < 4; i++) { wa[i].v[l] = a[l * 4 + i]; wb[i].v[l] = b[l * 4 + i]; acc[i].v[l] = d[l * 4 + i]; }
+  if (dtype == DT_BF16) SimB::mfma16<DT_BF16>(acc, wa, wb);
+  else SimB::mfma16<DT_F16>(acc, wa, wb);
+  for (int l = 0; l < 64; l++)
+    for (int i = 0; i < 4; i++) d[l * 4 + i] = acc[i].v[l];
+  return 0;
+}
+
+int ffcsim_outer_inv_half(int dtype, const uint16_t* e_in, uint16_t* e_out) {
+  HostPlan p;
+  if (!build_plan(32768, dtype, &p)) return -1;
+  if (dtype == DT_BF16) sim_outer_inv_half<DT_BF16>(p, e_in, e_out);
+  else sim_outer_inv_half<DT_F16>(p, e_in, e_out);
+  return 0;
+}
+
 int ffcsim_plan_info(int N, int dtype, int* nt, double* s_fwd, double* s_k, int32_t* kf_freq ) {
   HostPlan p;
   if (!build_plan(N, dtype, &p)) return -1;
@@ -472,6 +562,8 @@
 static void* g_z = nullptr; static void* g_yraw = nullptr; static int g_flags = 0;
 void ffcsim_set_z(void* z, void* yraw, int flags) { g_z = z; g_yraw = yraw; g_flags = flags; }
 long ffcsim_dma_count() { return g_dma_count.exchange(0); }
+long ffcsim_gs_count() { return g_gs_count.exchange(0); }
+void ffcsim_set_flags(int flags) { g_sim_flags = flags; }
 static float* g_dk_out = nullptr; static int g_dk_lk = 0;
 void ffcsim_set_fused_dk(float* dk, int Lk) { g_dk_out = dk; g_dk_lk = Lk; }
 static const float* g_kfuse_k = nullptr; static int g_kfuse_lk = 0;
@@ -495,6 +587,7 @@
   a.nchunk = 1; a.ppc = a.npair; a.conj_kf = conj_kf; a.s_inv = (float)p.s_inv; a.s_fwd = (float)p.s_fwd;
   a.fast = (L % 8 == 0) && !g_force_slow;
   a.R = p.R;
+  a.flags = g_sim_flags;
   a.sparse = g_sparse_rows;
   if (p.N1 > 1 && p.R == 1) { a.zsave = g_z; a.yraw = g_z ? g_yraw : nullptr; }
   if (p.N1 <= 1) { a.zsave = g_z; a.yraw = g_yraw; }
@@ -531,6 +624,7 @@
   a.nchunk = 1; a.ppc = a.npair; a.conj_kf = conj_kf; a.s_inv = (float)p.s_inv; a.s_fwd = (float)p.s_fwd;
   a.fast = (L % 8 == 0) && !((sb_u | sb_pre | sb_post | sb_y | sb_add) & 7) && !g_force_slow;
   a.R = p.R;
+  a.flags = g_sim_flags;
   a.zsave = zsave; a.yraw = y_raw;
   if (!addend) return dispatch<ConvRun>(N, dtype, a);
   return dispatch<ConvResRun>(N, dtype, a);
@@ -655,6 +749,27 @@
   return 0;
 }
 
+int ffcsim_launch_sink(int N, int dtype, int B, int H, int L, int flags, int* out) {
+  HostPlan p;
+  if (!build_plan(N, dtype, &p)) return -1;
+  static char buf[16];
+  DkfArgs d{};
+  ConvArgs& a = d.c;
+  a.B = B; a.H = H; a.L = L; a.npair = (B + 1) / 2; a.nchunk = 1; a.R = p.R; a.flags = flags & 0xffff;
+  a.zsave = (flags & (1 << 16)) ? buf : nullptr; a.yraw = (flags & (1 << 17)) ? buf : nullptr;
+  a.sparse = (flags & (1 << 18)) ? 2 : 0; a.fast = (flags & (1 << 19)) ? 1 : 0;
+  with_geo(N, [&](auto geo) {
+    using GEO = decltype(geo);
+    ConvArgs f = a;
+    f.postgate = (flags & (1 << 20)) ? buf : nullptr; f.addend = (flags & (1 << 21)) ? buf : nullptr;
+    out[0] = fwd_route<GEO>(f).gs;
+    a.pregate = (flags & (1 << 20)) ? buf : nullptr; d.dpre = (flags & (1 << 21)) ? buf : nullptr;
+    out[1] = bwd_route<GEO>(d, false).gs;
+    out[2] = bwd_route<GEO>(d, true).gs;
+  });
+  return 0;
+}
+
 int ffcsim_kernel_fft_c(int N, int dtype, const void* xpair, int H, void* kf, float scale) {
   HostPlan p;
   if (!build_plan(N, dtype, &p)) return -1;
@@ -718,7 +833,8 @@
   a.fast = (L % 8 == 0) && !g_force_slow;
   a.R = p.R;
   d.dout = dout; d.ws = ws; d.du = du; d.dpre = dpre; d.dpost = (p.N1 > 1 || g_yraw) ? dpost : nullptr;
-  if (p.N1 > 1 && p.R == 1 && g_z) { d.zin = g_z; d.yraw = g_yraw; a.flags = g_flags; a.stream = 1; }
+  a.flags = g_sim_flags;
+  if (p.N1 > 1 && p.R == 1 && g_z) { d.zin = g_z; d.yraw = g_yraw; a.flags = g_flags | g_sim_flags; a.stream = 1; }
   if (p.N1 <= 1) { d.zin = g_z; d.yraw = dpost ? g_yraw : nullptr; }
   HostPlan pbf;
   if (g_dk_pair && bwd_dk_form(p, a.nchunk, 128, true) != DK_SEPARATE) {
```

Measured after the change: 11.26 million seq/s (median of 6 runs). +6.5%, better.
